# haiciyang/LaDiffCodec

Measured on AMD Instinct MI355X. Metric: audio-sec decoded / wall-sec, 16kHz 3kbps 50-step DDPM, higher is better.
Workload: dtype bf16; 1 GPU; LaDiffCodec 3 kbps, diff_dims=256, enc_ratios 8 4, 50-step DDPM, batch=32x2.4 s utterances per GPU; global_batch=32, latent_len=1200, denoise_steps=50, rccl_ranks=1, batches_in_flight=1, parallelism=dp1 (utterance-sharded, no data-path collective)

## Files before the change

### include/ladiffcodec.h

```cpp
#ifndef LADIFFCODEC_H_
#define LADIFFCODEC_H_

#include <stdint.h>

#ifdef __cplusplus
extern "C" {
#endif

#define LDC_OK 0
#define LDC_E_INVALID -1
#define LDC_E_STATE -2
#define LDC_E_MISSING -3
#define LDC_E_HIP -4
#define LDC_E_NOMEM -5

#define LDC_F32 0
#define LDC_BF16 1
#define LDC_BF16_W8 2

#define LDC_MODEL_MAIN 0
#define LDC_MODEL_COND 1

#define LDC_MAX_RATIOS 8

// ... 120 lines not shown
                             float* eps_out, void* stream);
int ldc_denoise_windows(ldc_ctx* ctx, float* img_inout, const float* cond, const float* noise, int n_steps, int Ltot, int Ftot, int Lw,
                        int overlap, void* stream);
int ldc_ddim_sample_windows(ldc_ctx* ctx, float* img_inout, const float* cond, const float* noise, int t_start, int n_steps, float eta,
                            int Ltot, int Ftot, int Lw, int overlap, void* stream);
int ldc_decode_windows(ldc_ctx* ctx, const float* wav, int T, int n_steps, const float* noise, int Lw, int overlap, float* wav_out,
                       float* latents_out, float* cond_out, int64_t* codes_out, void* stream);
int ldc_decode_ddim_windows(ldc_ctx* ctx, const float* wav, int T, int t_start, int n_steps, float eta, const float* noise, int Lw,
                            int overlap, float* wav_out, float* latents_out, float* cond_out, int64_t* codes_out, void* stream);
int ldc_dpm_sample_windows(ldc_ctx* ctx, float* img_inout, const float* cond, int t_start, int n_steps, int Ltot, int Ftot, int Lw,
                           int overlap, void* stream);
int ldc_decode_dpm_windows(ldc_ctx* ctx, const float* wav, int T, int t_start, int n_steps, int Lw, int overlap, float* wav_out,
                           float* latents_out, float* cond_out, int64_t* codes_out, void* stream);
int ldc_decode_codes_windows(ldc_ctx* ctx, const int64_t* codes, const uint8_t* packed, int64_t packed_stride, int bits, int n_q, int Ftot,
                             int t_start, int n_steps, float eta, const float* noise, int Lw, int overlap, float* wav_out,
                             float* latents_out, float* cond_out, void* stream);
int ldc_decode_codes_dpm_windows(ldc_ctx* ctx, const int64_t* codes, const uint8_t* packed, int64_t packed_stride, int bits, int n_q,
                                 int Ftot, int t_start, int n_steps, int Lw, int overlap, float* wav_out, float* latents_out,
                                 float* cond_out, void* stream);
int ldc_window_group_layout(int R, const int* Ltot , int Lw, int overlap, int up, int* w0_out , int* starts_out ,
                            float* weights_out );
int ldc_unet_forward_windows_group(ldc_ctx* ctx, const float* x, int t, const float* cond, int R, const int* Ltot ,
                                   const int* Ftot , int Lw, int overlap, float* eps_out, void* stream);
int ldc_sample_windows_group(ldc_ctx* ctx, float* img_inout, const float* cond, int sampler, int t_start, int n_steps, float eta,
                             const float* noise, const uint64_t* seeds , int R, const int* Ltot ,
                             const int* Ftot , int Lw, int overlap, void* stream);
int ldc_decode_windows_group(ldc_ctx* ctx, const float* wav, int R, const int* T , int sampler, int t_start, int n_steps, float eta,
                             const float* noise, const uint64_t* seeds , int Lw, int overlap, float* wav_out,
                             float* latents_out, float* cond_out, int64_t* codes_out, void* stream);

int ldc_decode_codes(ldc_ctx* ctx, const int64_t* codes, const uint8_t* packed, int64_t packed_stride, int bits,
                     int n_q, int B, int F, int n_steps, const float* noise, int per_item,
                     float* wav_out, float* latents_out, float* cond_out, void* stream);
int ldc_decode_codes_ddim(ldc_ctx* ctx, const int64_t* codes, const uint8_t* packed, int64_t packed_stride, int bits,
                          int n_q, int B, int F, int t_start, int n_steps, float eta, const float* noise, int per_item,
                          float* wav_out, float* latents_out, float* cond_out, void* stream);
int ldc_decode_codes_ragged(ldc_ctx* ctx, const int64_t* codes, const uint8_t* packed, int64_t packed_stride, int bits, int n_q,
                            int B, int Fmax, const int32_t* frames_host, int t_start, int n_steps, float eta, const float* noise,
                            float* wav_out, float* latents_out, float* cond_out, void* stream);

int ldc_dpm_schedule(const float* sqrt_recip, const float* sqrt_recipm1, int timesteps, int t_start, int n_steps, int* t_out,
                     float* coef_out);
int ldc_dpm_sample(ldc_ctx* ctx, float* img_inout, const float* cond, int t_start, int n_steps, int B, int L, int F, void* stream);
int ldc_decode_dpm(ldc_ctx* ctx, const float* wav, int B, int T, int t_start, int n_steps, int per_item, float* wav_out,
                   float* latents_out, float* cond_out, int64_t* codes_out, void* stream);
int ldc_decode_codes_dpm(ldc_ctx* ctx, const int64_t* codes, const uint8_t* packed, int64_t packed_stride, int bits, int n_q, int B,
                         int F, int t_start, int n_steps, int per_item, float* wav_out, float* latents_out, float* cond_out,
                         void* stream);
int ldc_decode_ragged_dpm(ldc_ctx* ctx, const float* wav, const int32_t* lengths_host, int B, int Tmax, int t_start, int n_steps,
                          float* wav_out, float* latents_out, float* cond_out, int64_t* codes_out, void* stream);

int64_t ldc_packed_bytes(int n_q, int F, int bits);
int ldc_pack_codes(ldc_ctx* ctx, const int64_t* codes, int n_q, int B, int F, int bits, uint8_t* out, int64_t out_stride, void* stream);
int ldc_unpack_codes(ldc_ctx* ctx, const uint8_t* in, int64_t in_stride, int n_q, int B, int F, int bits, int64_t* codes_out,
                     void* stream);
int ldc_ac_build_cdf(ldc_ctx* ctx, const float* pdf, int rows, int card, int total_range_bits, float roundoff, int min_range,
                     int32_t* cdf_out, void* stream);
int ldc_ac_encode(ldc_ctx* ctx, const int32_t* symbols, const int32_t* cdf, int B, int S, int card, int n_static, int total_range_bits,
                  uint8_t* out, int64_t out_stride, int64_t* nbytes_out, void* stream);
int ldc_ac_decode(ldc_ctx* ctx, const uint8_t* in, int64_t in_stride, const int64_t* nbytes, const int32_t* cdf, int B, int S, int card,
                  int n_static, int total_range_bits, int32_t* symbols_out, int32_t* status_out, void* stream);
int ldc_ac_encode_ragged(ldc_ctx* ctx, const int32_t* symbols, const int32_t* n_sym, const int32_t* cdf, int B, int S, int card,
                         int n_static, int total_range_bits, uint8_t* out, int64_t out_stride, int64_t* nbytes_out, void* stream);
int ldc_ac_decode_ragged(ldc_ctx* ctx, const uint8_t* in, int64_t in_stride, const int64_t* nbytes, const int32_t* n_sym,
                         const int32_t* cdf, int B, int S, int card, int n_static, int total_range_bits, int32_t* symbols_out,
                         int32_t* status_out, void* stream);

int64_t ldc_resample_out_len(int64_t T, int orig_freq, int new_freq);
int ldc_resample(ldc_ctx* ctx, const float* wav, int C, int64_t T, int orig_freq, int new_freq, float* out, void* stream);

int ldc_train_q_sample(ldc_ctx* ctx, const float* x_start, const int64_t* t, const float* noise, int B, int C, int L, float* x_t,
                       void* stream);
int ldc_train_num_timesteps(ldc_ctx* ctx);
int ldc_train_predict_x_start(ldc_ctx* ctx, const float* x_t, const float* eps, const int64_t* t, int B, int C, int L, float* x0_out,
                              void* stream);
int ldc_train_neg_sdsdr(ldc_ctx* ctx, const float* est, const float* tgt, int B, int64_t n_per_item, float clip_min, float* per_item_out,
                        void* stream);

int ldc_train_l1_loss(ldc_ctx* ctx, const float* model_out, const float* target, const int64_t* t, int B, int C, int L, float* loss_out,
                      float* grad_out, void* stream);
int64_t ldc_train_block_ws_floats(int B, int Cin, int Cout, int L, int groups);
int ldc_train_block_forward(ldc_ctx* ctx, const float* x, const float* w, const float* bias, const float* gamma, const float* beta,
                            const float* scale_shift, int B, int Cin, int Cout, int L, int groups, float* y, float* ws, void* stream);
int ldc_train_block_backward(ldc_ctx* ctx, const float* dy, const float* x, const float* gamma, const float* beta,
                             const float* scale_shift, int B, int Cin, int Cout, int L, int groups, float* ws, float* dx, float* dw,
                             float* db, float* dgamma, float* dbeta, float* dscale_shift, void* stream);

int ldc_train_layernorm_forward(ldc_ctx* ctx, const float* x, const float* g, int B, int C, int L, float* y, float* stats, void* stream);
int ldc_train_layernorm_backward(ldc_ctx* ctx, const float* dy, const float* x, const float* g, const float* stats, int B, int C, int L,
                                 float* dx, float* dg, void* stream);

int ldc_train_pointwise_forward(ldc_ctx* ctx, const float* x, const float* w, const float* bias, int B, int Cin, int Cout, int L, int pre_silu,
                                float* y, void* stream);
int ldc_train_pointwise_backward(ldc_ctx* ctx, const float* dy, const float* x, const float* w, int B, int Cin, int Cout, int L, int pre_silu,
                                 float* dx, float* dw, float* db, void* stream);

int64_t ldc_train_linattn_ws_floats(int B, int heads, int dim_head, int N);
int ldc_train_linattn_forward(ldc_ctx* ctx, const float* qkv, int B, int heads, int dim_head, int N, float* out, float* ws, void* stream);
int ldc_train_linattn_backward(ldc_ctx* ctx, const float* dout, const float* qkv, int B, int heads, int dim_head, int N, float* ws, float* dqkv,
                               void* stream);

int ldc_train_conv_forward(ldc_ctx* ctx, const float* x, const float* w, const float* bias, int B, int Cin, int Cout, int Lin, int K, int stride,
                           int pad, float* y, void* stream);
int ldc_train_conv_backward(ldc_ctx* ctx, const float* dy, const float* x, const float* w, int B, int Cin, int Cout, int Lin, int K, int stride,
                            int pad, float* dx, float* dw, float* db, void* stream);
int ldc_train_join(ldc_ctx* ctx, void* stream);
int ldc_train_side_stream(ldc_ctx* ctx, void** stream_out);
int ldc_train_upsample2(ldc_ctx* ctx, const float* in, int64_t rows, int L, int backward, float* out, void* stream);
int ldc_train_activation(ldc_ctx* ctx, const float* x, const float* dy, int64_t n, int kind, float* out, void* stream);
int64_t ldc_train_attn_ws_floats(int B, int heads, int N);
int ldc_train_attn_forward(ldc_ctx* ctx, const float* qkv, int B, int heads, int dim_head, int N, float* out, float* ws, void* stream);
int ldc_train_attn_backward(ldc_ctx* ctx, const float* dout, const float* qkv, int B, int heads, int dim_head, int N, float* ws, float* dqkv,
                            void* stream);

int ldc_train_convtr_forward(ldc_ctx* ctx, const float* x, const float* w, const float* bias, int B, int Cin, int Cout, int L, int ratio, float* y,
                             void* stream);
int ldc_train_convtr_backward(ldc_ctx* ctx, const float* dy, const float* x, const float* w, int B, int Cin, int Cout, int L, int ratio, float* dx,
                              float* dw, float* db, void* stream);
int ldc_train_maxscale(ldc_ctx* ctx, const float* x, const float* dy, int B, int64_t n_per_item, float* out, void* stream);

int ldc_train_adam_step(ldc_ctx* ctx, float* param, const float* grad, float* exp_avg, float* exp_avg_sq, int64_t n, int step, float lr,
                        float beta1, float beta2, float eps, void* stream);
int ldc_train_adam_step_dev(ldc_ctx* ctx, float* param, const float* grad, float* exp_avg, float* exp_avg_sq, int64_t n, int32_t* step_dev,
                            float lr, float beta1, float beta2, float eps, void* stream);

int ldc_sconv1d(ldc_ctx* ctx, const float* x, int B, int Cin, int L, const float* w_host, const float* b_host,
                int Cout, int k, int stride, int dilation, int causal, int pre_elu, float* y, void* stream);
int ldc_sconvtr1d(ldc_ctx* ctx, const float* x, int B, int Cin, int L, const float* w_host, const float* b_host,
                  int Cout, int k, int stride, int causal, float* y, void* stream);
int ldc_slstm(ldc_ctx* ctx, const float* x, int B, int H, int T, const float* const* weights_host, int layers,
              float* y, void* stream);

int ldc_unet_debug_tap(ldc_ctx* ctx, const char* name, float* out, int64_t capacity_elems, void* stream);
int ldc_unet_step_cost(ldc_ctx* ctx, int B, int L, double* flops, double* bytes);
int ldc_profile_enable(ldc_ctx* ctx, int on);
int ldc_xcc_census(ldc_ctx* ctx, const uint32_t* mask, int n_words, int wgs, int* hist16);

int ldc_debug_attn_core(ldc_ctx* ctx, int kind, const float* qkv, int B, int L, const float* w_out, const float* b_out,
                        const float* gain, const float* resid, int C, float* out, void* stream);
int ldc_debug_attention_block(ldc_ctx* ctx, const char* name, const float* x, int B, int L, float* out, void* stream);
int ldc_debug_resnet_block(ldc_ctx* ctx, const char* name, const float* x1, const float* x2, int B, int L, int t, const int32_t* lens,
                           int shift, const int32_t* t_items, int with_attention, float* out, float* mid, float* stats, float* attn_out,
                           float* pre, int* info, void* stream);

int ldc_debug_sea_conv(ldc_ctx* ctx, const float* x, int B, int Cin, int L, const float* w_host, const float* b_host, int Cout, int k,
                       int stride, int dilation, int causal, int transposed, int pre_elu, const float* residual, float* y, int* route,
                       void* stream);
int ldc_debug_sea_op(ldc_ctx* ctx, int which, int decoder, int index, const float* x, int B, int L, float* out, int64_t capacity_elems,
                     int* info, void* stream);

int ldc_debug_raise_failure(ldc_ctx* ctx, int code);
long long ldc_debug_sync_count(void);
long long ldc_debug_lean_launches(int kind);

int ldc_host_stats(ldc_ctx* ctx, int reset, double* graph_launch_ms, double* lookahead_wait_ms, int64_t* graph_launches);
int ldc_graph_schedule(int n_steps, int parts, int strided, int graph_steps_option, int* K_out, int* n_big_out, int* n_single_out);
int ldc_stream_info(ldc_ctx* ctx, int* good, int* candidates, double* one_spin_ms, double* all_spin_ms, int* parts);
int ldc_clock_sample(ldc_ctx* ctx, uint64_t* out2, void* stream);

int ldc_timeline_enable(ldc_ctx* ctx, int on);
int ldc_timeline_read(ldc_ctx* ctx, int part, int n, uint64_t* ticks);
int ldc_kstamps_enable(ldc_ctx* ctx, int on);
int ldc_kstamps_reset(ldc_ctx* ctx);
int ldc_kstamps_read(ldc_ctx* ctx, int idx, int n_steps, int* n_ops, uint64_t* ticks, char* infos, int info_cap, int* classes);
int ldc_gn_microbench(ldc_ctx* ctx, int dtype, int B, int L, int C, int with_residual, int iters, double* ms_per_launch);
int ldc_conv_microbench(ldc_ctx* ctx, int dtype, int B, int L, int cin1, int cin2, int cout, int k, int stride, int ups,
                        int iters, double* ms_per_launch);
int ldc_conv_compare(ldc_ctx* ctx, int dtype, int B, int L, int cin1, int cin2, int cout, int k, int stride, int ups, int tile_cfg,
                     int with_gn, int with_colmax, int with_residual, double* max_abs_diff, double* max_abs_ref, double* max_rel_stat);
int ldc_ln_fold_compare(ldc_ctx* ctx, int dtype, int rows, int C, int n_out, double dc, double* max_abs_diff2, double* max_abs_ref);
int ldc_conv_compare_fp8(ldc_ctx* ctx, int B, int L, int cin1, int cin2, int cout, int k, int stride, int ups, int with_gn, int with_colmax,
                         double* max_abs_diff, double* max_abs_ref, double* max_rel_stat);
int ldc_profile_read(ldc_ctx* ctx, double* conv_ms_total, int64_t* conv_launches, double* conv_flops_total);
enum {
  LDC_CLASS_OTHER = 0,
  LDC_CLASS_CONV = 1,
  LDC_CLASS_GN_APPLY = 2,
  LDC_CLASS_LAYERNORM = 3,
  LDC_CLASS_LINATTN = 4,
  LDC_CLASS_ATTN_FULL = 5,
  LDC_CLASS_ELEMENTWISE = 6,
  LDC_N_CLASSES = 7
};
int ldc_profile_read_classes(ldc_ctx* ctx, int n, double* ms, int64_t* launches, double* flops, double* bytes);

#ifdef __cplusplus
}
#endif
#endif
```

### ladiffcodec_amd/csrc/ldc_api.cpp

```cpp
#include "ldc_internal.h"

long long g_device_syncs = 0;

static thread_local char g_err[1024] = "";
int fail(int code, const char* fmt, ...) {
  va_list ap;
  va_start(ap, fmt);
  vsnprintf(g_err, sizeof(g_err), fmt, ap);
  va_end(ap);
  return code;
}

extern "C" const char* ldc_last_error(void) { return g_err; }
extern "C" const char* ldc_version(void) { return "ladiffcodec-amd 0.1 (gfx950)"; }



static std::vector<float> fold_weight_norm(const HostTensor& g, const HostTensor& v) {
  const size_t n0 = (size_t)v.shape[0], inner = v.numel() / n0;
  std::vector<float> w(v.numel());
  for (size_t i = 0; i < n0; ++i) {
    double s = 0;
    for (size_t j = 0; j < inner; ++j) s += (double)v.data[i * inner + j] * v.data[i * inner + j];
    const float nrm = (float)sqrt(s);
// ... 499 lines not shown
    const int r = c->cfg.upsampling_ratios[i];
    const std::string p = P + ".upsampling_layers." + std::to_string(i) + ".convtr.convtr";
    HostTensor* w = wr.get(p + ".weight", {u.cond_channels, u.cond_channels, 2 * r});
    HostTensor* b = wr.get(p + ".bias", {u.cond_channels});
    u.up_ratios.push_back(r);
    if (!w || !b) continue;
    ConvLayer ly;
    const int padding_total = r, right = padding_total / 2, left = padding_total - right;
    LDCCHK(make_convtr(c, DT_F32, u.cond_channels, u.cond_channels, r, left, ACT_NONE, w->data.data(), b->data.data(), &ly));
    u.upsamplers.push_back(ly);
  }
  static const char* names[13] = {"betas", "alphas_cumprod", "alphas_cumprod_prev", "sqrt_alphas_cumprod",
                                  "sqrt_one_minus_alphas_cumprod", "log_one_minus_alphas_cumprod",
                                  "sqrt_recip_alphas_cumprod", "sqrt_recipm1_alphas_cumprod", "posterior_variance",
                                  "posterior_log_variance_clipped", "posterior_mean_coef1", "posterior_mean_coef2",
                                  "p2_loss_weight"};
  std::map<std::string, float*> dev;
  for (const char* n : names) {
    HostTensor* t = wr.get(std::string("diffusion.") + n, {u.timesteps});
    if (!t) continue;
    float* d = nullptr;
    LDCCHK(c->wmem.upload(&d, t->data));
    dev[n] = d;
    if (std::string(n) == "alphas_cumprod") c->alphas_cumprod = t->data;
    if (std::string(n) == "sqrt_recip_alphas_cumprod") c->sqrt_recip_ac = t->data;
    if (std::string(n) == "sqrt_recipm1_alphas_cumprod") c->sqrt_recipm1_ac = t->data;
  }
  c->sched.sqrt_recip_alphas_cumprod = dev["sqrt_recip_alphas_cumprod"];
  c->sched.sqrt_recipm1_alphas_cumprod = dev["sqrt_recipm1_alphas_cumprod"];
  c->sched.posterior_mean_coef1 = dev["posterior_mean_coef1"];
  c->sched.posterior_mean_coef2 = dev["posterior_mean_coef2"];
  c->sched.posterior_log_variance_clipped = dev["posterior_log_variance_clipped"];
  c->sqrt_alphas_cumprod = dev["sqrt_alphas_cumprod"];
  c->sqrt_one_minus_alphas_cumprod = dev["sqrt_one_minus_alphas_cumprod"];
  c->p2_loss_weight = dev["p2_loss_weight"];
  if (wr.missing.empty()) LDCCHK(build_time_table(c, wr));
  *missing += wr.missing;
  return LDC_OK;
}

static int build_time_table(ldc_ctx* c, WeightReader& wr) {
  UnetW& u = c->unet;
  const int T = u.timesteps, dim = u.dim, td = u.time_dim;
  const std::string P = "diff_model";
  HostTensor* w1 = wr.get(P + ".time_mlp.1.weight", {td, dim});
  HostTensor* b1 = wr.get(P + ".time_mlp.1.bias", {td});
  HostTensor* w2 = wr.get(P + ".time_mlp.3.weight", {td, td});
  HostTensor* b2 = wr.get(P + ".time_mlp.3.bias", {td});
  if (!w1 || !b1 || !w2 || !b2) return LDC_OK;
  const int half = dim / 2;
  std::vector<float> emb((size_t)T * dim);
  const float lg = logf(10000.0f) / (float)(half - 1);
  for (int t = 0; t < T; ++t)
    for (int k = 0; k < half; ++k) {
      const float f = expf((float)k * -lg);
      const float a = (float)t * f;
      emb[(size_t)t * dim + k] = sinf(a);
      emb[(size_t)t * dim + half + k] = cosf(a);
    }
  DevMem tmp;
  float *d_emb = nullptr, *d_h1 = nullptr, *d_h2 = nullptr;
  LDCCHK(tmp.upload(&d_emb, emb));
  void* p = nullptr;
  LDCCHK(tmp.alloc(&p, (size_t)T * td * 4)); d_h1 = (float*)p;
  LDCCHK(tmp.alloc(&p, (size_t)T * td * 4)); d_h2 = (float*)p;
  LDCCHK(c->wmem.alloc(&p, (size_t)T * u.ss_stride * 4));
  u.ss_table = (float*)p;
  LDCCHK(c->wmem.alloc(&p, (size_t)u.ss_stride * 4));
  u.cur_ss = (float*)p;
  hipStream_t s = c->own_stream;
  ConvLayer l1, l2;
  ConvSpec sp;
  sp.dt = DT_F32; sp.cin1 = dim; sp.cout = td; sp.k = 1; sp.post_act = ACT_GELU;
  LDCCHK(make_conv(c, sp, w1->data.data(), b1->data.data(), &l1));
  sp.cin1 = td; sp.post_act = ACT_SILU;
  LDCCHK(make_conv(c, sp, w2->data.data(), b2->data.data(), &l2));
  ConvCall cc;
  cc.B = 1; cc.L_in = T; cc.L_rows = T;
  cc.x1 = d_emb; cc.y = d_h1; cc.y_ld = td;
  HIPCHK(launch_conv(l1, cc, s));
  cc.x1 = d_h1; cc.y = d_h2;
  HIPCHK(launch_conv(l2, cc, s));
  std::vector<ResnetW*> blocks;
  for (auto& lv : u.downs) { blocks.push_back(&lv.b1); blocks.push_back(&lv.b2); }
  blocks.push_back(&u.mid1); blocks.push_back(&u.mid2);
  for (auto& lv : u.ups) { blocks.push_back(&lv.b1); blocks.push_back(&lv.b2); }
  blocks.push_back(&u.fin);
  std::vector<std::string> prefixes;
  for (size_t i = 0; i < u.downs.size(); ++i) { prefixes.push_back(P + ".downs." + std::to_string(i) + ".0"); prefixes.push_back(P + ".downs." + std::to_string(i) + ".1"); }
  prefixes.push_back(P + ".mid_block1"); prefixes.push_back(P + ".mid_block2");
  for (size_t i = 0; i < u.ups.size(); ++i) { prefixes.push_back(P + ".ups." + std::to_string(i) + ".0"); prefixes.push_back(P + ".ups." + std::to_string(i) + ".1"); }
  prefixes.push_back(P + ".final_res_block");
  for (size_t i = 0; i < blocks.size(); ++i) {
    ResnetW* r = blocks[i];
    HostTensor* wm = wr.get(prefixes[i] + ".mlp.1.weight", {2 * r->cout, td});
    HostTensor* bm = wr.get(prefixes[i] + ".mlp.1.bias", {2 * r->cout});
    if (!wm || !bm) continue;
    ConvLayer lm;
    ConvSpec sm;
    sm.dt = DT_F32; sm.cin1 = td; sm.cout = 2 * r->cout; sm.k = 1;
    LDCCHK(make_conv(c, sm, wm->data.data(), bm->data.data(), &lm));
    ConvCall cm;
    cm.B = 1; cm.L_in = T; cm.L_rows = T; cm.x1 = d_h2; cm.y = u.ss_table + r->ss_off; cm.y_ld = u.ss_stride;
    HIPCHK(launch_conv(lm, cm, s));
    u.weight_elems += (double)wm->numel();
  }
  HIPCHK(hipStreamSynchronize(s));
  return LDC_OK;
}

extern "C" int ldc_create(const ldc_config* cfg, int device, ldc_ctx** out) {
  if (!cfg || !out) return fail(LDC_E_INVALID, "null argument");
  if (cfg->compute_dtype != LDC_F32 && cfg->compute_dtype != LDC_BF16 && cfg->compute_dtype != LDC_BF16_W8)
    return fail(LDC_E_INVALID, "compute_dtype must be LDC_F32, LDC_BF16 or LDC_BF16_W8");
  if (cfg->n_enc_ratios < 1 || cfg->n_enc_ratios > LDC_MAX_RATIOS || cfg->n_upsampling_ratios < 0 ||
      cfg->n_upsampling_ratios > LDC_MAX_RATIOS)
    return fail(LDC_E_INVALID, "bad ratio counts");
  if (cfg->rep_dims != 128) return fail(LDC_E_INVALID, "rep_dims must be 128 (RVQ / UNet channel width of the reference checkpoints)");
  if (cfg->diff_dims % 32 || cfg->diff_dims <= 0) return fail(LDC_E_INVALID, "diff_dims must be a positive multiple of 32");
  if (cfg->n_filters % 32) return fail(LDC_E_INVALID, "n_filters must be a multiple of 32");
  int ndev = 0;
  HIPCHK(hipGetDeviceCount(&ndev));
  if (device < 0 || device >= ndev) return fail(LDC_E_INVALID, "device %d out of range (%d visible)", device, ndev);
  HIPCHK(hipSetDevice(device));
  hipDeviceProp_t prop;
  HIPCHK(hipGetDeviceProperties(&prop, device));
  if (strncmp(prop.gcnArchName, "gfx950", 6) != 0)
    return fail(LDC_E_INVALID, "this library is built for gfx950 (MI355X) only; device %d is %s", device, prop.gcnArchName);
  std::unique_ptr<ldc_ctx> c(new ldc_ctx());
  c->cfg = *cfg;
  c->device = device;
  c->num_cus = prop.multiProcessorCount;
  c->dt = cfg->compute_dtype == LDC_F32 ? DT_F32 : DT_BF16;
  c->w8 = cfg->compute_dtype == LDC_BF16_W8;
  HIPCHK(hipStreamCreateWithFlags(&c->own_stream, hipStreamNonBlocking));
  for (int k = 0; k < kMaxParts; ++k)
    for (int e = 0; e <= ldc_ctx::kLstmChunks; ++e) HIPCHK(hipEventCreateWithFlags(&c->lstm_ev[k][e], hipEventDisableTiming));
  if (const char* ex = getenv("LDC_TEST_EXTRA_STREAMS")) {
    for (int i = 0; i < atoi(ex); ++i) { hipStream_t dummy = nullptr; HIPCHK(hipStreamCreateWithFlags(&dummy, hipStreamNonBlocking)); }
  }
  HIPCHK(hipEventCreateWithFlags(&c->ev_fork, hipEventDisableTiming));
  for (auto& e : c->flow_ev) HIPCHK(hipEventCreateWithFlags(&e, hipEventDisableTiming));
  for (int k = 1; k < kMaxParts; ++k) {
    HIPCHK(hipStreamCreateWithFlags(&c->aux_stream[k], hipStreamNonBlocking));
    HIPCHK(hipEventCreateWithFlags(&c->ev_join[k], hipEventDisableTiming));
  }
  for (int k = 0; k < kMaxParts; ++k) {
    HIPCHK(hipStreamCreateWithFlags(&c->side_stream[k], hipStreamNonBlocking));
    HIPCHK(hipEventCreateWithFlags(&c->ev_side_fork[k], hipEventDisableTiming));
    HIPCHK(hipEventCreateWithFlags(&c->ev_side_join[k], hipEventDisableTiming));
  }
  c->xcd_resident[0] = lstm_xcd_resident(256);
  c->xcd_resident[1] = lstm_xcd_resident(512);
  c->coop_resident[0] = lstm_coop_resident(256) ? 1 : 0;
  c->coop_resident[1] = lstm_coop_resident(512) ? 1 : 0;
  c->plan_bytes_cap = (size_t)48 << 30;
  c->plan_count_cap = 24;
  if (const char* mp = getenv("LDC_AUX_FROM_SIDE")) {
    c->calib = 0;
    for (int k = 1; k < kMaxParts && mp[k - 1]; ++k)
      if (mp[k - 1] >= '0' && mp[k - 1] < '0' + kMaxParts) std::swap(c->aux_stream[k], c->side_stream[mp[k - 1] - '0']);
  }
  if (const char* ov = getenv("LDC_OPTIONS")) {
    std::string all(ov);
    size_t pos = 0;
    while (pos < all.size()) {
      size_t end = all.find_first_of(",; ", pos);
      if (end == std::string::npos) end = all.size();
      const std::string kv = all.substr(pos, end - pos);
      pos = end + 1;
      if (kv.empty()) continue;
      const size_t eq = kv.find('=');
      const std::string name = kv.substr(0, eq);
      const int value = eq == std::string::npos ? 1 : atoi(kv.c_str() + eq + 1);
      std::unique_ptr<ldc_ctx>& cc = c;
      const int rc = ldc_set_option(cc.get(), name.c_str(), value);
      if (rc != LDC_OK) return fail(LDC_E_INVALID, "LDC_OPTIONS: %s", ldc_last_error());
    }
  }
  switch (cfg->final_activation) {
    case LDC_ACT_NONE: c->enc_final_act = ACT_NONE; break;
    case LDC_ACT_TANH: c->enc_final_act = ACT_TANH; break;
    case LDC_ACT_SIGMOID: c->enc_final_act = ACT_SIGMOID; break;
    case LDC_ACT_ELU: c->enc_final_act = ACT_ELU; break;
    case LDC_ACT_SILU: c->enc_final_act = ACT_SILU; break;
    case LDC_ACT_GELU: c->enc_final_act = ACT_GELU; break;
    case LDC_ACT_RELU: c->enc_final_act = ACT_RELU; break;
    default: return fail(LDC_E_INVALID, "final_activation code %d is not one of LDC_ACT_*", cfg->final_activation);
  }
  {
    void* hp = nullptr;
    HIPCHK(hipHostMalloc(&hp, 64, hipHostMallocMapped));
    memset(hp, 0, 64);
    c->dev_flag_host = (unsigned*)hp;
    void* dp = nullptr;
    HIPCHK(hipHostGetDevicePointer(&dp, hp, 0));
    c->dev_flag_dev = (unsigned*)dp;
  }
  void* p = nullptr;
  HIPCHK(hipMalloc(&p, 4 * sizeof(int)));
  c->step_state = (int*)p;
  *out = c.release();
  return LDC_OK;
}

void free_plan_resources(Plan* pl) {
  for (hipEvent_t e : pl->marker_events) (void)hipEventDestroy(e);
  if (pl->arena_base) (void)hipFree(pl->arena_base);
  if (pl->x0_prev) (void)hipFree(pl->x0_prev);
  if (pl->item_keys) (void)hipFree(pl->item_keys);
  if (pl->win_base) (void)hipFree(pl->win_base);
}

void release_plan(ldc_ctx* c, size_t idx) {
  Plan* pl = c->plans[idx].get();
  for (int k = 0; k < c->last_halves.n; ++k)
    if (c->last_halves.p[k] == pl) c->last_halves = Halves();
  free_plan_resources(pl);
  c->plan_bytes -= pl->arena_bytes;
  c->plans.erase(c->plans.begin() + idx);
}

void drop_plans(ldc_ctx* c) {
  (void)counted_device_sync();
  drop_step_graphs(c, [](const StepGraph&) { return true; });
  for (auto& pl : c->plans) free_plan_resources(pl.get());
  c->plans.clear();
  c->plan_bytes = 0;
  c->last_halves = Halves();
}

extern "C" int ldc_destroy(ldc_ctx* c) {
  if (!c) return LDC_OK;
  (void)hipSetDevice(c->device);
  (void)counted_device_sync();
  drop_plans(c);
  if (c->scratch) (void)hipFree(c->scratch);
  if (c->outnorm_ws) (void)hipFree(c->outnorm_ws);
  if (c->state_buf) (void)hipFree(c->state_buf);
  if (c->ddim_table) (void)hipFree(c->ddim_table);
  if (c->dpm_table) (void)hipFree(c->dpm_table);
  if (c->step_state) (void)hipFree(c->step_state);
  if (c->dev_flag_host) (void)hipHostFree(c->dev_flag_host);
  if (c->tl_buf) (void)hipFree(c->tl_buf);
  for (auto& e : c->prof_events) { (void)hipEventDestroy(e.first); (void)hipEventDestroy(e.second); }
  if (c->ev_fork) (void)hipEventDestroy(c->ev_fork);
  for (int k = 0; k < kMaxParts; ++k) {
    for (int e = 0; e <= ldc_ctx::kLstmChunks; ++e)
      if (c->lstm_ev[k][e]) (void)hipEventDestroy(c->lstm_ev[k][e]);
  }
  for (auto& e : c->flow_ev) if (e) (void)hipEventDestroy(e);
  for (int k = 1; k < kMaxParts; ++k) {
    if (c->ev_join[k]) (void)hipEventDestroy(c->ev_join[k]);
    if (c->aux_stream[k]) (void)hipStreamDestroy(c->aux_stream[k]);
  }
  for (int k = 0; k < kMaxParts; ++k) {
    if (c->ev_side_fork[k]) (void)hipEventDestroy(c->ev_side_fork[k]);
    if (c->ev_side_join[k]) (void)hipEventDestroy(c->ev_side_join[k]);
    if (c->side_stream[k]) (void)hipStreamDestroy(c->side_stream[k]);
  }
  if (c->own_stream) (void)hipStreamDestroy(c->own_stream);
  delete c;
  return LDC_OK;
}

extern "C" void ldc_quantize_e4m3(const float* in, int64_t n, uint8_t* out_codes, float* out_values) {
  for (int64_t i = 0; i < n; ++i) {
    const uint8_t q = host_f32_to_e4m3(in[i]);
    if (out_codes) out_codes[i] = q;
    if (out_values) out_values[i] = host_e4m3_to_f32(q);
  }
}

struct OptRef { int* p; bool replan; int lo, hi; };
static bool find_option(ldc_ctx* c, const std::string& n, OptRef* r) {
#define LDC_OPT(NAME, FIELD, REPLAN, LO, HI) if (n == NAME) { r->p = &(FIELD); r->replan = REPLAN; r->lo = LO; r->hi = HI; return true; }
  LDC_OPT("split", c->split_batch, true, 1, kMaxParts)
  LDC_OPT("part_graphs", c->part_graphs, false, 0, 2)
  LDC_OPT("graph_steps", c->graph_steps, false, 0, 1000)
  LDC_OPT("flow_depth", c->flow_depth, false, 0, (int)ldc_ctx::kFlowRing - 1)
  LDC_OPT("split_ends", c->split_ends, false, 0, 1)
  LDC_OPT("ends_join", c->ends_join, false, 0, 1)
  LDC_OPT("split_init", c->split_init, true, 0, 1)
  LDC_OPT("side_streams", c->side_streams, true, 0, 1)
  LDC_OPT("serial_parts", c->serial_parts, false, 0, 1)
  LDC_OPT("stream_calib", c->calib, false, 0, 1)
  LDC_OPT("merge_advance", c->merge_advance, true, 0, 1)
  LDC_OPT("fuse_gn_stats", c->fuse_gn_stats, true, 0, 1)
  LDC_OPT("fuse_gn_epi", c->fuse_gn_epi, true, 0, 1)
  LDC_OPT("gn_epi_min_l", c->gn_epi_min_l, true, 0, 1 << 30)
  LDC_OPT("gn_epi_max_tiles", c->gn_epi_max_tiles, true, 0, 1 << 30)
  LDC_OPT("fold_res", c->fold_res, true, 0, 1)
  LDC_OPT("fold_ln", c->fold_ln, true, 0, 1)
  LDC_OPT("fuse_kmax", c->fuse_kmax, true, 0, 1)
  LDC_OPT("fuse_ln", c->fuse_ln, true, 0, 1)
  LDC_OPT("fuse_attn_tail", c->fuse_attn_tail, true, 0, 1)
  LDC_OPT("fold_ctx", c->fold_ctx, true, 0, 1)
  LDC_OPT("conv_lean", c->tune.lean, true, 0, 1)
  LDC_OPT("lean_all", c->tune.lean_all, true, 0, 1)
  LDC_OPT("ring3_tiles", c->tune.ring3_tiles, true, 0, 1 << 30)
  LDC_OPT("ring3_wgs", c->tune.ring3_wgs, true, 1, 3)
  LDC_OPT("ring3_window", c->tune.ring3_window, true, 0, 1)
  LDC_OPT("ring3_window_tiles", c->tune.ring3_window_tiles, true, 0, 1 << 30)
  LDC_OPT("conv_generic", c->tune.force_generic, true, 0, 1)
  LDC_OPT("conv_small_tiles", c->tune.small_max, true, 0, 1 << 30)
  LDC_OPT("conv_splitk", c->tune.splitk, true, 0, 4)
  LDC_OPT("sk_tiles", c->tune.sk_tiles, true, 0, 1 << 30)
  LDC_OPT("sk_u2", c->tune.sk_u2, true, 0, 1 << 30)
  LDC_OPT("sk_u3", c->tune.sk_u3, true, 0, 1 << 30)
  LDC_OPT("conv_mfast", c->tune.m_fastest, true, 0, 2)
  LDC_OPT("conv_debug", c->tune.debug, true, 0, 255)
  LDC_OPT("conv_tile", c->tune.force_tile, true, -1, 1)
  LDC_OPT("conv_xcd_order", c->tune.xcd_order, true, 0, 8)
  LDC_OPT("gn_nap", c->tune.gn_nap, true, 0, 4096)
  LDC_OPT("gn_nap0", c->tune.gn_nap0, true, 0, 4096)
  LDC_OPT("lstm_stream", c->lstm_stream_only, false, 0, 1)
  LDC_OPT("lstm_xcd", c->lstm_xcd, false, 0, 1)
  LDC_OPT("lstm_pipe", c->lstm_pipe, false, 0, 1)
  LDC_OPT("coop_launch", c->coop_launch, false, 0, 1)
  LDC_OPT("sea_splitk", c->sea_splitk, false, 0, 1)
  LDC_OPT("rvq_tiled", c->rvq_tiled, false, 0, 1)
  LDC_OPT("train_bf16", g_train_bf16, false, 0, 1)
  LDC_OPT("train_fp32_mfma", g_train_fp32_mfma, false, 0, 1)
  LDC_OPT("train_valu", g_train_valu, false, 0, 1)
  LDC_OPT("train_dw_side", g_train_dw_side, false, 0, 1)
#undef LDC_OPT
  return false;
}

extern "C" int ldc_set_option(ldc_ctx* c, const char* name, int value) {
  if (!c || !name) return fail(LDC_E_INVALID, "null context or option name");
  const std::string n(name);
  if (n == "fp8_act") {
    if (c->finalized) return fail(LDC_E_STATE, "fp8_act must be set before ldc_finalize_weights");
    c->fp8_act = value ? 1 : 0;
    return LDC_OK;
  }
  if (n == "plan_cache_gb") { c->plan_bytes_cap = (size_t)std::max(1, value) << 30; return LDC_OK; }
  if (n == "plan_cache_n") { c->plan_count_cap = std::max(2 * kMaxParts, value); return LDC_OK; }
  OptRef r;
  if (!find_option(c, n, &r)) return fail(LDC_E_INVALID, "unknown option '%s' (tools/README.md lists the options)", name);
  if (value < r.lo || value > r.hi) return fail(LDC_E_INVALID, "option %s must be in %d..%d", name, r.lo, r.hi);
  if (n == "side_streams" && value && c->split_batch != 1) return fail(LDC_E_INVALID, "side streams need a single chain (split 1)");
  if (value == *r.p) return LDC_OK;
  if (r.replan && c->live_pools > 0)
    return fail(LDC_E_STATE, "option %s rebuilds every plan, and %d decode pool(s) keep their items' state in theirs: destroy the pools first", name, c->live_pools);
  if (r.replan && !c->plans.empty()) { HIPCHK(hipSetDevice(c->device)); drop_plans(c); }
  *r.p = value;
  if (n == "split" && value != 1) c->side_streams = 0;
  return LDC_OK;
}

extern "C" long long ldc_debug_sync_count(void) { return g_device_syncs; }

extern "C" int ldc_debug_raise_failure(ldc_ctx* c, int code) {
  if (!c || !c->dev_flag_host || (code != 1 && code != 2 && code != (int)kDevFailCtxRange)) return fail(LDC_E_INVALID, "bad arguments");
  *reinterpret_cast<volatile unsigned*>(c->dev_flag_host) = (unsigned)code;
  return LDC_OK;
}

extern "C" int ldc_reseed(ldc_ctx* c, uint64_t seed) {
  if (!c) return fail(LDC_E_INVALID, "null ctx");
  c->cfg.noise_seed = seed;
  c->noise_epoch = 0;
  return LDC_OK;
}

extern "C" int ldc_set_weight(ldc_ctx* c, int which, const char* key, const float* data, const int64_t* shape, int ndim) {
  if (!c || !key || !data || (ndim > 0 && !shape)) return fail(LDC_E_INVALID, "null argument");
  if (which != LDC_MODEL_MAIN && which != LDC_MODEL_COND) return fail(LDC_E_INVALID, "which must be LDC_MODEL_MAIN or LDC_MODEL_COND");
  if (c->finalized) return fail(LDC_E_STATE, "weights already finalized");
  HostTensor t;
  t.shape.assign(shape, shape + ndim);
  t.data.assign(data, data + t.numel());
  c->raw[which][key] = std::move(t);
  return LDC_OK;
}

extern "C" int ldc_finalize_weights(ldc_ctx* c, int strict) {
  if (!c) return fail(LDC_E_INVALID, "null ctx");
  if (c->finalized) return fail(LDC_E_STATE, "already finalized");
  HIPCHK(hipSetDevice(c->device));
  std::string missing;
  std::vector<int> main_ratios(c->cfg.enc_ratios, c->cfg.enc_ratios + c->cfg.n_enc_ratios);
  LDCCHK(build_codec(c, LDC_MODEL_MAIN, main_ratios, 0, &missing));
  LDCCHK(build_unet(c, &missing));
  if (c->cfg.has_cond_model) {
    const int frame_rate_ceil = 50;
    const int n_q = (int)floor(1000.0 * c->cfg.cond_bandwidth / (frame_rate_ceil * 10));
    LDCCHK(build_codec(c, LDC_MODEL_COND, {8, 5, 4, 2}, n_q, &missing));
  }
  if (!missing.empty()) return fail(LDC_E_MISSING, "missing or mis-shaped keys in state_dict: %s", missing.c_str());
  if (strict) {
    std::string unexpected;
    for (int w = 0; w < 2; ++w)
      for (auto& kv : c->raw[w])
        if (!kv.second.used) {
          const std::string& k = kv.first;
          std::string alias;
          if (k.rfind("diffusion.model.", 0) == 0) alias = "diff_model." + k.substr(16);
          else if (k.rfind("diff_model.", 0) == 0) alias = "diffusion.model." + k.substr(11);
          auto it = alias.empty() ? c->raw[w].end() : c->raw[w].find(alias);
          if (it != c->raw[w].end() && it->second.used && it->second.shape == kv.second.shape) continue;
          if (unexpected.size() < 600) unexpected += k + " ";
        }
    if (!unexpected.empty()) return fail(LDC_E_MISSING, "unexpected keys in state_dict: %s", unexpected.c_str());
  }
  c->raw[0].clear();
  c->raw[1].clear();
  c->finalized = true;
  return LDC_OK;
}

int ensure_scratch(ldc_ctx* c, size_t bytes, hipStream_t s) {
  if (bytes <= c->scratch_cap) return LDC_OK;
  HIPCHK(hipStreamSynchronize(s));
  HIPCHK(counted_device_sync());
  if (c->scratch) HIPCHK(hipFree(c->scratch));
  c->scratch = nullptr;
  c->scratch_cap = 0;
  void* p = nullptr;
  const size_t want = bytes + bytes / 4;
  hipError_t e = hipMalloc(&p, want);
  if (e != hipSuccess) return fail(LDC_E_NOMEM, "hipMalloc(%zu) for scratch failed: %s", want, hipGetErrorString(e));
  c->scratch = (char*)p;
  c->scratch_cap = want;
  return LDC_OK;
}

int conv_out_len(const ConvLayer& ly, int L) {
  const int eff_k = (ly.taps - 1) * ly.dil + 1;
  const int padding_total = eff_k - ly.stride;
  const double n_frames = (double)(L - eff_k + padding_total) / ly.stride + 1.0;
  return (int)ceil(n_frames);
}


static int stream_conv_state(SeaRun& R, int rows, int ch, StreamConvState** out) {
  *out = nullptr;
  if (!R.st || rows <= 0) return LDC_OK;
  if (R.st->conv_at >= R.st->convs.size() || R.st->convs[R.st->conv_at].rows != rows || R.st->convs[R.st->conv_at].ch != ch)
    return fail(LDC_E_STATE, "stream state does not match the layer table (conv %zu: %d rows x %d channels)", R.st->conv_at, rows, ch);
  *out = &R.st->convs[R.st->conv_at++];
  return LDC_OK;
}

static int sea_conv_stream(SeaRun& R, const ConvLayer& ly, StreamConvState& cs, const void* x, const void* residual, int L_in, void** y, int* L_out, int cout) {
  if (!ly.tr_stride && L_in % ly.stride) return fail(LDC_E_INVALID, "stream chunk of %d rows is not a multiple of the layer's stride %d", L_in, ly.stride);
  ConvLayer lv = ly;
  lv.pad_left = 0;
  ConvCall cc;
  cc.B = R.B; cc.L_in = L_in + cs.rows; cc.x1 = x; cc.residual = residual; cc.tune = &R.c->tune; cc.route_out = R.route;
  cc.ctx = cs.buf[R.st->parity]; cc.ctx_fresh = R.st->fresh_dev; cc.ctx_rows = cs.rows; cc.ctx_zero = ly.tr_stride ? 1 : 0;
  if (ly.tr_stride) {
    cc.L_rows = L_in;
    cc.L_final = L_in * ly.tr_stride;
    *L_out = cc.L_final;
    cc.y_ld = ly.tr_cout;
  } else {
    cc.L_rows = L_in / ly.stride;
    *L_out = cc.L_rows;
    cc.y_ld = cout;
  }
  *y = R.ar->alloc((size_t)R.B * (*L_out) * cc.y_ld * 4);
  cc.y = *y;
  if (R.c->sea_splitk) {
    const long long fl = conv_generic_splitk_floats(lv, cc);
    if (fl > 0) {
      cc.sk_part = (float*)R.ar->alloc((size_t)fl * 4);
      cc.sk_part_cap = fl;
      cc.generic_split = 1;
    }
  }
  if (R.dry) {
    ConvCall chk = cc;
    chk.check_only = 1; chk.route_out = nullptr;
    if (launch_conv(lv, chk, R.s) != hipSuccess)
      return fail(LDC_E_INVALID, "stream chunk of %d rows x B = %d items: the LDS window of a layer (%d context rows per item, stride %d) does not fit; "
                                 "use longer chunks or fewer items per session", L_in, R.B, cs.rows, ly.stride);
  } else {
    HIPCHK(launch_conv(lv, cc, R.s));
    HIPCHK(launch_stream_ctx_update((const float*)x, cs.buf[R.st->parity], cs.buf[R.st->parity ^ 1], R.st->fresh_dev, R.B, L_in, cs.rows, cs.ch, cc.ctx_zero, R.s));
  }
  return LDC_OK;
}

int sea_conv(SeaRun& R, const ConvLayer& ly, const void* x, const void* residual, int L_in, void** y, int* L_out, int cout) {
  StreamConvState* cs = nullptr;
  LDCCHK(stream_conv_state(R, ly.tr_stride ? 1 : ly.pad_left, ly.cin1, &cs));
  if (cs) return sea_conv_stream(R, ly, *cs, x, residual, L_in, y, L_out, cout);
  ConvCall cc;
  cc.B = R.B; cc.L_in = L_in; cc.x1 = x; cc.residual = residual; cc.tune = &R.c->tune; cc.route_out = R.route;
  if (ly.tr_stride) {
    cc.L_rows = L_in + 1;
    cc.L_final = L_in * ly.tr_stride;
    *L_out = cc.L_final;
    cc.y_ld = ly.tr_cout;
  } else {
    cc.L_rows = conv_out_len(ly, L_in);
    *L_out = cc.L_rows;
    cc.y_ld = cout;
  }
  *y = R.ar->alloc((size_t)R.B * (*L_out) * cc.y_ld * 4);
  cc.y = *y;
  if (R.c->sea_splitk) {
    const long long fl = conv_generic_splitk_floats(ly, cc);
    if (fl > 0) {
      cc.sk_part = (float*)R.ar->alloc((size_t)fl * 4);
      cc.sk_part_cap = fl;
      cc.generic_split = 1;
    }
  }
  if (!R.dry) HIPCHK(launch_conv(ly, cc, R.s));
  return LDC_OK;
}

int run_seanet(SeaRun& R, const std::vector<SeaOp>& ops, const void* x_in, int L, void** out, int* L_out, int* C_out) {
  const void* x = x_in;
  int C = 0;
  for (const SeaOp& op : ops) {
    void* y = nullptr;
    int Ln = L;
    switch (op.kind) {
      case SeaOp::CONV_CIN1: {
        if (L <= op.k - 1) return fail(LDC_E_INVALID, "input no longer than the first conv's reflect padding is not supported (L=%d pad=%d)", L, op.k - 1);
        y = R.ar->alloc((size_t)R.B * L * op.cout * 4);
        StreamConvState* cs = nullptr;
        LDCCHK(stream_conv_state(R, op.k - 1, 1, &cs));
        if (!R.dry && cs) {
          HIPCHK(launch_conv_cin1(DT_F32, (const float*)x, y, op.w1, op.b1, R.B, L, op.cout, op.k, R.s, nullptr, cs->buf[R.st->parity], R.st->fresh_dev));
          HIPCHK(launch_stream_ctx_update((const float*)x, cs->buf[R.st->parity], cs->buf[R.st->parity ^ 1], R.st->fresh_dev, R.B, L, cs->rows, 1, 0, R.s));
        } else if (!R.dry) HIPCHK(launch_conv_cin1(DT_F32, (const float*)x, y, op.w1, op.b1, R.B, L, op.cout, op.k, R.s));
        C = op.cout;
        break;
      }
      case SeaOp::CONV:
      case SeaOp::CONVTR:
        LDCCHK(sea_conv(R, op.conv, x, nullptr, L, &y, &Ln, op.cout));
        C = op.cout;
        break;
      case SeaOp::RES: {
        void *sc = nullptr, *h = nullptr;
        int l1 = L, l2 = L, l3 = L;
        LDCCHK(sea_conv(R, op.shortcut, x, nullptr, L, &sc, &l1, op.cout));
        LDCCHK(sea_conv(R, op.conv, x, nullptr, L, &h, &l2, op.hidden));
        LDCCHK(sea_conv(R, op.conv2, h, sc, l2, &y, &l3, op.cout));
        Ln = l3;
        C = op.cout;
        break;
      }
      case SeaOp::LSTM: {
        const int H = op.cout;
        const void* in = x;
        const bool pipe = !R.st && R.c->lstm_pipe && R.side >= 0 && R.side < 2 && R.c->aux_stream[2 + R.side] && op.lstm.size() == 2 && lstm_seq_supported(H) && !op.lstm[0].w_rm && !op.lstm[1].w_rm &&
                          L >= 64 * ldc_ctx::kLstmChunks;
        if (pipe) {
          constexpr int NCH = ldc_ctx::kLstmChunks;
          void* pre0 = R.ar->alloc((size_t)R.B * L * 4 * H * 4);
          void* o0 = R.ar->alloc((size_t)R.B * L * H * 4);
          void* pre1 = R.ar->alloc((size_t)R.B * L * 4 * H * 4);
          void* o1 = R.ar->alloc((size_t)R.B * L * H * 4);
          float* st0 = (float*)R.ar->alloc((size_t)R.B * 2 * H * 4);
          float* st1 = (float*)R.ar->alloc((size_t)R.B * 2 * H * 4);
          if (!R.dry) {
            hipStream_t s2 = R.c->aux_stream[2 + R.side];
            hipEvent_t* ev = R.c->lstm_ev[R.side];
            ConvCall cc;
            cc.B = R.B; cc.L_in = L; cc.L_rows = L; cc.x1 = in; cc.y = pre0; cc.y_ld = 4 * H; cc.tune = &R.c->tune;
            HIPCHK(launch_conv(op.lstm[0].in_proj, cc, R.s));
            for (int k = 0; k < NCH; ++k) {
              const int t0 = (int)((long long)L * k / NCH), t1 = (int)((long long)L * (k + 1) / NCH);
              LstmSeq q0;
              q0.t0 = t0; q0.t1 = t1; q0.pre_bs = L; q0.pre_ts = 1; q0.out_bs = 1; q0.out_ts = R.B; q0.state = st0;
              HIPCHK(launch_lstm_seq(DT_F32, pre0, op.lstm[0].w_hh, o0, nullptr, R.B, H, q0, R.s));
              HIPCHK(hipEventRecord(ev[k], R.s));
              HIPCHK(hipStreamWaitEvent(s2, ev[k], 0));
              ConvCall c1;
              c1.B = 1; c1.L_in = (t1 - t0) * R.B; c1.L_rows = c1.L_in; c1.tune = &R.c->tune; c1.y_ld = 4 * H;
              c1.x1 = (const char*)o0 + (size_t)t0 * R.B * H * 4;
              c1.y = (char*)pre1 + (size_t)t0 * R.B * 4 * H * 4;
              HIPCHK(launch_conv(op.lstm[1].in_proj, c1, s2));
              LstmSeq q1;
              q1.t0 = t0; q1.t1 = t1; q1.pre_bs = 1; q1.pre_ts = R.B; q1.out_bs = L; q1.out_ts = 1; q1.skip_bs = L; q1.skip_ts = 1; q1.state = st1;
              HIPCHK(launch_lstm_seq(DT_F32, pre1, op.lstm[1].w_hh, o1, x, R.B, H, q1, s2));
            }
            HIPCHK(hipEventRecord(ev[NCH], s2));
            HIPCHK(hipStreamWaitEvent(R.s, ev[NCH], 0));
          }
          y = o1;
          C = H;
          break;
        }
        for (size_t n = 0; n < op.lstm.size(); ++n) {
          void* pre = R.ar->alloc((size_t)R.B * L * 4 * H * 4);
          void* o = R.ar->alloc((size_t)R.B * L * H * 4);
          const bool coop = op.lstm[n].w_rm && !R.c->lstm_stream_only && R.c->coop_resident[H == 512 ? 1 : 0];
          void* lws = coop ? R.ar->alloc(lstm_coop_ws_bytes(H)) : nullptr;
          LstmCarry carry;
          if (R.st) {
            if (R.st->lstm_at >= R.st->lstm.size()) return fail(LDC_E_STATE, "stream state does not match the layer table (LSTM layer %zu)", R.st->lstm_at);
            carry.state = R.st->lstm[R.st->lstm_at++];
            carry.fresh = R.st->fresh_dev;
          }
          if (!R.dry) {
            ConvCall cc;
            cc.B = R.B; cc.L_in = L; cc.L_rows = L; cc.x1 = in; cc.y = pre; cc.y_ld = 4 * H; cc.tune = &R.c->tune;
            HIPCHK(launch_conv(op.lstm[n].in_proj, cc, R.s));
            const bool lastl = n + 1 == op.lstm.size();
            hipError_t le = hipErrorCooperativeLaunchTooLarge;
            if (coop) le = launch_lstm_coop(DT_F32, pre, op.lstm[n].w_rm, o, lastl ? x : nullptr, R.B, L, H, lws, R.c->dev_flag_dev, (R.c->lstm_xcd && R.c->xcd_resident[H == 512 ? 1 : 0] >= 2 * R.teams) ? 2 : R.c->coop_launch, R.s, carry);
            if (le == hipErrorCooperativeLaunchTooLarge) {
              (void)hipGetLastError();
              le = launch_lstm_layer(DT_F32, pre, op.lstm[n].w_hh, o, lastl ? x : nullptr, R.B, L, H, R.s, carry);
            }
            HIPCHK(le);
          }
          in = o;
          y = o;
        }
        C = H;
        break;
      }
    }
    x = y;
    L = Ln;
  }
  *out = const_cast<void*>(x);
  *L_out = L;
  *C_out = C;
  return LDC_OK;
}


int check_ready(ldc_ctx* c, int which, bool need_cond_codec) {
  if (!c) return fail(LDC_E_INVALID, "null ctx");
  if (!c->finalized) return fail(LDC_E_STATE, "ldc_finalize_weights has not been called");
  if (which != LDC_MODEL_MAIN && which != LDC_MODEL_COND) return fail(LDC_E_INVALID, "bad model selector");
  if ((which == LDC_MODEL_COND || need_cond_codec) && !c->codec[LDC_MODEL_COND].present)
    return fail(LDC_E_STATE, "no cond model configured (has_cond_model = 0)");
  hipError_t e = hipSetDevice(c->device);
  if (e != hipSuccess) return fail(LDC_E_HIP, "hipSetDevice failed: %s", hipGetErrorString(e));
  return check_dev_flag(c);
}

extern "C" int ldc_seanet_encode(ldc_ctx* c, int which, const float* wav, int B, int T, float* z_out, void* stream) {
  LDCCHK(check_ready(c, which));
  if (!wav || !z_out || B <= 0 || T <= 0) return fail(LDC_E_INVALID, "bad arguments");
  hipStream_t s = pick_stream(c, stream);
  const Codec& cd = c->codec[which];
  LDCCHK(with_scratch(c, s, [&](Arena& ar, bool dry) -> int {
    SeaRun R{c, &ar, s, dry, B};
    void* z = nullptr;
    int L = 0, C = 0;
    LDCCHK(run_seanet(R, cd.enc, wav, T, &z, &L, &C));
    if (!dry) HIPCHK(launch_from_cl(DT_F32, z, z_out, B, C, L, nullptr, 0, 0.f, s));
    return LDC_OK;
  }));
  return finish_stream(c, stream);
}

extern "C" int ldc_seanet_decode(ldc_ctx* c, int which, const float* z, int B, int L, float* wav_out, void* stream) {
  LDCCHK(check_ready(c, which));
  if (!z || !wav_out || B <= 0 || L <= 0) return fail(LDC_E_INVALID, "bad arguments");
  hipStream_t s = pick_stream(c, stream);
  const Codec& cd = c->codec[which];
  const int D = c->cfg.rep_dims;
  LDCCHK(with_scratch(c, s, [&](Arena& ar, bool dry) -> int {
    SeaRun R{c, &ar, s, dry, B};
    R.side = 0;
    void* zc = ar.alloc((size_t)B * L * D * 4);
    if (!dry) HIPCHK(launch_to_cl(DT_F32, z, zc, B, D, L, nullptr, 0, 0.f, s));
    void* y = nullptr;
    int Lo = 0, C = 0;
    LDCCHK(run_seanet(R, cd.dec, zc, L, &y, &Lo, &C));
    if (!dry) HIPCHK(hipMemcpyAsync(wav_out, y, (size_t)B * Lo * 4, hipMemcpyDeviceToDevice, s));
    return LDC_OK;
  }));
  return finish_stream(c, stream);
}

int rvq_rows(ldc_ctx* c, const float* z_rows, int rows, int n_q, int64_t* codes, float* q_rows, Arena& ar, bool dry,
                    hipStream_t s) {
  const Codec& cd = c->codec[LDC_MODEL_COND];
  int64_t* cw = codes;
  if (!cw) cw = (int64_t*)ar.alloc((size_t)n_q * rows * sizeof(int64_t));
  if (!dry) HIPCHK(launch_rvq(z_rows, rows, c->cfg.rep_dims, cd.codebooks, cd.cb_sqnorm, cd.bins, n_q, cw, q_rows, s, c->rvq_tiled));
  return LDC_OK;
}

int n_q_for_bandwidth(ldc_ctx* c, float bandwidth) {
  const Codec& cd = c->codec[LDC_MODEL_COND];
  const double bw = bandwidth > 0 ? bandwidth : c->cfg.cond_bandwidth;
  const double bw_per_q = log2((double)cd.bins) * (16000.0 / cd.hop) / 1000.0;
  int n_q = cd.n_q_layers;
  if (bw > 0) n_q = (int)std::max(1.0, floor(bw / bw_per_q));
  return std::min(n_q, cd.n_q_layers);
}

extern "C" int ldc_rvq_encode(ldc_ctx* c, const float* z, int B, int F, int n_q, int64_t* codes_out, float* quantized_out,
                              void* stream) {
  LDCCHK(check_ready(c, LDC_MODEL_COND));
  const Codec& cd = c->codec[LDC_MODEL_COND];
  if (!z || !quantized_out || B <= 0 || F <= 0 || n_q < 1 || n_q > cd.n_q_layers)
    return fail(LDC_E_INVALID, "bad arguments (n_q must be in [1,%d])", cd.n_q_layers);
  hipStream_t s = pick_stream(c, stream);
  const int D = c->cfg.rep_dims;
  LDCCHK(with_scratch(c, s, [&](Arena& ar, bool dry) -> int {
    float* zr = (float*)ar.alloc((size_t)B * F * D * 4);
    float* qr = (float*)ar.alloc((size_t)B * F * D * 4);
    if (!dry) HIPCHK(launch_to_cl(DT_F32, z, zr, B, D, F, nullptr, 0, 0.f, s));
    LDCCHK(rvq_rows(c, zr, B * F, n_q, codes_out, qr, ar, dry, s));
    if (!dry) HIPCHK(launch_from_cl(DT_F32, qr, quantized_out, B, D, F, nullptr, 0, 0.f, s));
    return LDC_OK;
  }));
  return finish_stream(c, stream);
}

extern "C" int ldc_rvq_decode(ldc_ctx* c, const int64_t* codes, int B, int F, int n_q, float* quantized_out, void* stream) {
  LDCCHK(check_ready(c, LDC_MODEL_COND));
  const Codec& cd = c->codec[LDC_MODEL_COND];
  if (!codes || !quantized_out || B <= 0 || F <= 0 || n_q < 1 || n_q > cd.n_q_layers) return fail(LDC_E_INVALID, "bad arguments");
  hipStream_t s = pick_stream(c, stream);
  const int D = c->cfg.rep_dims;
  LDCCHK(with_scratch(c, s, [&](Arena& ar, bool dry) -> int {
    float* qr = (float*)ar.alloc((size_t)B * F * D * 4);
    if (!dry) {
      HIPCHK(launch_rvq_dequant(codes, nullptr, 0, 0, n_q, B, 0, B, F, cd.codebooks, cd.bins, D, qr, c->dev_flag_dev, s));
      HIPCHK(launch_from_cl(DT_F32, qr, quantized_out, B, D, F, nullptr, 0, 0.f, s));
    }
    return LDC_OK;
  }));
  return finish_stream(c, stream);
}

static int get_cond_rows(ldc_ctx* c, const float* wav, int B, int T, float bandwidth, Arena& ar, bool dry, hipStream_t s,
                         float** q_rows, int* F_out, int64_t* codes_out, int teams = 1) {
  const Codec& cd = c->codec[LDC_MODEL_COND];
  SeaRun R{c, &ar, s, dry, B};
  R.teams = teams;
  void* z = nullptr;
  int F = 0, C = 0;
  LDCCHK(run_seanet(R, cd.enc, wav, T, &z, &F, &C));
  float* qr = (float*)ar.alloc((size_t)B * F * C * 4);
  LDCCHK(rvq_rows(c, (const float*)z, B * F, n_q_for_bandwidth(c, bandwidth), codes_out, qr, ar, dry, s));
  *q_rows = qr;
  *F_out = F;
  return LDC_OK;
}

extern "C" int ldc_get_cond(ldc_ctx* c, const float* wav, int B, int T, float bandwidth, float* cond_out, int64_t* codes_out,
                            void* stream) {
  LDCCHK(check_ready(c, LDC_MODEL_COND));
  if (!wav || !cond_out || B <= 0 || T <= 0) return fail(LDC_E_INVALID, "bad arguments");
  hipStream_t s = pick_stream(c, stream);
  LDCCHK(with_scratch(c, s, [&](Arena& ar, bool dry) -> int {
    float* qr = nullptr;
    int F = 0;
    LDCCHK(get_cond_rows(c, wav, B, T, bandwidth, ar, dry, s, &qr, &F, codes_out));
    if (!dry) HIPCHK(launch_from_cl(DT_F32, qr, cond_out, B, c->cfg.rep_dims, F, nullptr, 0, 0.f, s));
    return LDC_OK;
  }));
  return finish_stream(c, stream);
}

static int upsample_rows(ldc_ctx* c, const void* rows_in, int B, int F, Arena& ar, bool dry, hipStream_t s, void** out,
                         int* L_out, const int* flens = nullptr) {
  const UnetW& u = c->unet;
  const void* x = rows_in;
  int L = F;
  for (const ConvLayer& ly : u.upsamplers) {
    ConvCall cc;
    cc.B = B; cc.L_in = L; cc.L_rows = L + 1; cc.L_final = L * ly.tr_stride; cc.y_ld = ly.tr_cout; cc.x1 = x; cc.tune = &c->tune;
    void* y = ar.alloc((size_t)B * cc.L_final * ly.tr_cout * 4);
    cc.y = y;
    if (!dry) HIPCHK(launch_conv(ly, cc, s));
    if (!dry && flens) HIPCHK(launch_mask_rows(DT_F32, y, B, F, cc.L_final / F * ly.tr_cout, flens, 0, s));
    x = y;
    L = cc.L_final;
  }
  *out = const_cast<void*>(x);
  *L_out = L;
  return LDC_OK;
}

int upsample_factor(const ldc_ctx* c) {
  int f = 1;
  for (int r : c->unet.up_ratios) f *= r;
  return f;
}

extern "C" int ldc_cond_upsample(ldc_ctx* c, const float* cond, int B, int F, int normalise, float* img_out, void* stream) {
  LDCCHK(check_ready(c, LDC_MODEL_MAIN));
  if (!cond || !img_out || B <= 0 || F <= 0 || normalise < 0 || normalise > 2) return fail(LDC_E_INVALID, "bad arguments");
  hipStream_t s = pick_stream(c, stream);
  const int C = c->unet.cond_channels;
  LDCCHK(with_scratch(c, s, [&](Arena& ar, bool dry) -> int {
    void* rows = ar.alloc((size_t)B * F * C * 4);
    float* mx = (float*)ar.alloc((size_t)B * 4);
    if (!dry) HIPCHK(launch_to_cl(DT_F32, cond, rows, B, C, F, nullptr, 0, 0.f, s));
    void* up = nullptr;
    int L = 0;
    LDCCHK(upsample_rows(c, rows, B, F, ar, dry, s, &up, &L));
    if (!dry) {
      if (normalise) {
        HIPCHK(hipMemsetAsync(mx, 0, (size_t)B * 4, s));
        HIPCHK(launch_maxabs(DT_F32, up, B, (int64_t)L * C, normalise == 2, mx, s));
        HIPCHK(launch_from_cl(DT_F32, up, img_out, B, C, L, mx, normalise == 2, 1e-8f, s));
      } else {
        HIPCHK(launch_from_cl(DT_F32, up, img_out, B, C, L, nullptr, 0, 0.f, s));
      }
    }
    return LDC_OK;
  }));
  return finish_stream(c, stream);
}

int calibrate_part_streams(ldc_ctx* c, hipStream_t s) {
  if (!c->calib || (c->calibrated && c->calib_stream == s)) return LDC_OK;
  hipStreamCaptureStatus cs = hipStreamCaptureStatusNone;
  if (hipStreamIsCapturing(s, &cs) != hipSuccess || cs != hipStreamCaptureStatusNone) { (void)hipGetLastError(); return LDC_OK; }
  std::vector<hipStream_t*> cand;
  for (int k = 1; k < kMaxParts; ++k) cand.push_back(&c->aux_stream[k]);
  for (int k = 0; k < kMaxParts; ++k) cand.push_back(&c->side_stream[k]);
  for (const auto& e : c->calib_cache)
    if (e.s == s && e.order.size() == cand.size()) {
      for (size_t i = 0; i < cand.size(); ++i) *cand[i] = e.order[i];
      c->calib_good = e.good; c->calib_cand = e.cand; c->calib_one_ms = e.one_ms; c->calib_all_ms = e.all_ms;
      c->calib_stream = s; c->calibrated = true;
      return LDC_OK;
    }
  std::vector<hipStream_t> chosen{s};
  auto timed = [&](const std::vector<hipStream_t>& set, double* ms) -> int {
    double best = 1e30;
    for (int rep = 0; rep < 4; ++rep) {
      for (hipStream_t q : set) HIPCHK(hipStreamSynchronize(q));
      const auto t0 = std::chrono::steady_clock::now();
      for (hipStream_t q : set) HIPCHK(launch_spin_us(150, q));
      for (hipStream_t q : set) HIPCHK(hipStreamSynchronize(q));
      best = std::min(best, std::chrono::duration<double, std::milli>(std::chrono::steady_clock::now() - t0).count());
    }
    *ms = best;
    return LDC_OK;
  };
  double base = 0;
  LDCCHK(timed(chosen, &base));
  LDCCHK(timed(chosen, &base));
  std::vector<hipStream_t> good, rest;
  for (hipStream_t* p : cand) {
    if ((int)good.size() >= kMaxParts - 1) { rest.push_back(*p); continue; }
    std::vector<hipStream_t> set = chosen;
    set.push_back(*p);
    double ms = 0;
    LDCCHK(timed(set, &ms));
    if (ms < base + 0.09) { good.push_back(*p); chosen.push_back(*p); }
    else rest.push_back(*p);
  }
  if (getenv("LDC_VERBOSE")) fprintf(stderr, "[ldc] part streams: %zu of %zu candidates overlap with the caller's stream and each other (one spin: %.3f ms)\n", good.size(), cand.size(), base);
  std::vector<hipStream_t> order = good;
  order.insert(order.end(), rest.begin(), rest.end());
  for (size_t i = 0; i < cand.size(); ++i) *cand[i] = order[i];
  double all_ms = base;
  if (!good.empty()) LDCCHK(timed(chosen, &all_ms));
  c->calib_good = (int)good.size(); c->calib_cand = (int)cand.size(); c->calib_one_ms = base; c->calib_all_ms = all_ms;
  if (c->calib_cache.size() >= 8) c->calib_cache.erase(c->calib_cache.begin());
  c->calib_cache.push_back({s, order, c->calib_good, c->calib_cand, base, all_ms});
  c->calib_stream = s;
  c->calibrated = true;
  return LDC_OK;
}

int get_halves(ldc_ctx* c, int B, int L, int F, hipStream_t s, Halves* h, bool ragged, bool items, int pool_id) {
  *h = Halves();
  c->call_tick = c->use_tick;
  h->n = std::max(1, std::min(c->split_batch, B));
  if (h->n >= 2) LDCCHK(calibrate_part_streams(c, s));
  for (int k = 0; k < h->n; ++k) {
    const int lo = (int)((long long)B * k / h->n), hi = (int)((long long)B * (k + 1) / h->n);
    h->b0[k] = lo;
    LDCCHK(get_plan(c, hi - lo, L, F, k, s, &h->p[k], ragged, items, pool_id));
  }
  c->last_halves = *h;
  return LDC_OK;
}

int load_cond(ldc_ctx* c, const Halves& h, const float* cond, hipStream_t s) {
  for (int k = 0; k < h.n; ++k) {
    Plan* pl = h.p[k];
    const float* src = cond + (size_t)h.b0[k] * c->unet.cond_channels * pl->F;
    HIPCHK(launch_to_cl(DT_F32, src, pl->cond_in_cl, pl->B, c->unet.cond_channels, pl->F, nullptr, 0, 0.f, s));
    LDCCHK(run_ops(c, pl, false, s));
  }
  return LDC_OK;
}

int load_x(ldc_ctx* c, const Halves& h, const float* x, hipStream_t s) {
  for (int k = 0; k < h.n; ++k) {
    Plan* pl = h.p[k];
    HIPCHK(launch_to_cl(c->dt, x + (size_t)h.b0[k] * c->unet.channels * pl->L, pl->x_cl, pl->B, c->unet.channels, pl->L, nullptr,
                        0, 0.f, s));
  }
  return LDC_OK;
}

int check_unet_args(ldc_ctx* c, int B, int L, int F) {
  if (B <= 0 || L <= 0 || F <= 0) return fail(LDC_E_INVALID, "bad sizes");
  if (F * upsample_factor(c) != L) return fail(LDC_E_INVALID, "L (%d) must equal F (%d) x prod(upsampling_ratios) (%d)", L, F, upsample_factor(c));
  return LDC_OK;
}

extern "C" int ldc_unet_forward(ldc_ctx* c, const float* x, int t, const float* cond, int B, int L, int F, float* eps_out,
                                void* stream) {
// ... 43 lines not shown
    std::vector<int> fr(pl->B);
    for (int b = 0; b < pl->B; ++b) fr[b] = lat[h.b0[k] + b] / up;
    HIPCHK(launch_lens_write(pl->lens, lat.data() + h.b0[k], pl->B, s));
    HIPCHK(launch_lens_write(pl->flens, fr.data(), pl->B, s));
  }
  return LDC_OK;
}

extern "C" int ldc_unet_forward_ragged(ldc_ctx* c, const float* x, int t, const float* cond, const int32_t* latent_lens_host, int B, int Lmax,
                                       int Fmax, float* eps_out, void* stream) {
  LDCCHK(check_ready(c, LDC_MODEL_MAIN));
  if (!x || !cond || !eps_out) return fail(LDC_E_INVALID, "null tensor");
  if (t < 0 || t >= c->unet.timesteps) return fail(LDC_E_INVALID, "t out of range");
  LDCCHK(check_unet_args(c, B, Lmax, Fmax));
  LDCCHK(check_ragged_lengths(latent_lens_host, B, Lmax, ragged_latent_quantum(c), "latent frames"));
  if (c->w8) return fail(LDC_E_INVALID, "ragged batches are not available on the fp8 engine (its fused forms have no length-aware variant): use dtype bf16 or f32");
  hipStream_t s = pick_stream(c, stream);
  Halves h;
  LDCCHK(get_halves(c, B, Lmax, Fmax, s, &h, true));
  LDCCHK(write_plan_lens(c, h, std::vector<int>(latent_lens_host, latent_lens_host + B), s));
  LDCCHK(load_cond(c, h, cond, s));
  LDCCHK(load_x(c, h, x, s));
  for (int k = 0; k < h.n; ++k) {
    Plan* pl = h.p[k];
    HIPCHK(launch_mask_rows(c->dt, pl->x_cl, pl->B, Lmax, c->unet.channels, pl->lens, 0, s));
    HIPCHK(launch_step_set(pl->step_state, t, 0, c->cur_key, s));
    HIPCHK(launch_step_begin(c->unet.ss_table, c->unet.ss_stride, pl->step_state, pl->cur_ss, nullptr, s, pl->zero_ptr, pl->zero_bytes));
    LDCCHK(run_ops(c, pl, true, s));
    HIPCHK(launch_mask_rows(c->dt, pl->eps_cl, pl->B, Lmax, c->unet.channels, pl->lens, 0, s));
    HIPCHK(launch_from_cl(c->dt, pl->eps_cl, eps_out + (size_t)h.b0[k] * c->unet.channels * Lmax, pl->B, c->unet.channels, Lmax, nullptr,
                          0, 0.f, s));
  }
  return finish_stream(c, stream);
}

static int ensure_outnorm(ldc_ctx* c, int B) {
  const size_t need = output_normalise_ws_bytes(B);
  if (need <= c->outnorm_ws_bytes) return LDC_OK;
  HIPCHK(counted_device_sync());
  if (c->outnorm_ws) HIPCHK(hipFree(c->outnorm_ws));
  c->outnorm_ws = nullptr;
  HIPCHK(hipMalloc(&c->outnorm_ws, need * 2));
  c->outnorm_ws_bytes = need * 2;
  return LDC_OK;
}

extern "C" int ldc_output_normalise(ldc_ctx* c, float* wav, int B, int T, int per_item, void* stream) {
  if (!c) return fail(LDC_E_INVALID, "null ctx");
  if (!wav || B <= 0 || T <= 0) return fail(LDC_E_INVALID, "bad arguments");
  HIPCHK(hipSetDevice(c->device));
  LDCCHK(ensure_outnorm(c, B));
  hipStream_t s = pick_stream(c, stream);
  HIPCHK(launch_output_normalise(wav, B, T, per_item ? 1 : 0, c->outnorm_ws, s));
  return finish_stream(c, stream);
}

struct FrontSrc {
  const float* wav = nullptr;
  const int64_t* codes = nullptr;
  const uint8_t* packed = nullptr;
  int64_t packed_stride = 0;
  int bits = 0, n_q = 0;
};

static int ragged_cond_rows(ldc_ctx* c, const float* wav, int B, int b0, int Bk, int T, const int32_t* lens, const int* flens_dev,
                            float bandwidth, Arena& ar, bool dry, hipStream_t sk, float** q_rows, int* F_out, int64_t* codes_out,
                            int teams) {
  const Codec& cc = c->codec[LDC_MODEL_COND];
  const int F = T / cc.hop, D = c->cfg.rep_dims, n_q = n_q_for_bandwidth(c, bandwidth);
  if (codes_out && (b0 != 0 || Bk != B)) return fail(LDC_E_INVALID, "internal: the codes of a ragged batch are written for the whole batch");
  float* qr = nullptr;
  int Fq = 0;
  LDCCHK(get_cond_rows(c, wav + (size_t)b0 * T, Bk, T, bandwidth, ar, dry, sk, &qr, &Fq, codes_out, teams));
  if (!dry && Fq != F) return fail(LDC_E_INVALID, "internal: encoder produced %d frames, expected %d", Fq, F);
  const int short_max = cc.enc.empty() ? 0 : cc.enc.back().k - 1;
  for (int b = b0; b < b0 + Bk; ++b) {
    const int Fb = lens[b] / cc.hop;
    if (Fb > short_max) continue;
    float* q1 = nullptr;
    int F1 = 0;
    int64_t* codes1 = codes_out ? (int64_t*)ar.alloc((size_t)n_q * Fb * 8) : nullptr;
    LDCCHK(get_cond_rows(c, wav + (size_t)b * T, 1, lens[b], bandwidth, ar, dry, sk, &q1, &F1, codes1, teams));
    if (dry) continue;
    HIPCHK(hipMemcpyAsync(qr + (size_t)(b - b0) * F * D, q1, (size_t)F1 * D * 4, hipMemcpyDeviceToDevice, sk));
    if (codes_out)
      HIPCHK(hipMemcpy2DAsync(codes_out + (size_t)b * F, (size_t)B * F * 8, codes1, (size_t)F1 * 8, (size_t)F1 * 8, n_q, hipMemcpyDeviceToDevice, sk));
  }
  if (!dry) {
    if (codes_out) HIPCHK(launch_mask_codes(codes_out, n_q, Bk, F, flens_dev + b0, sk));
    HIPCHK(launch_mask_rows(DT_F32, qr, Bk, F, D, flens_dev + b0, 0, sk));
  }
  *q_rows = qr;
  *F_out = F;
  return LDC_OK;
}

static int decode_body(ldc_ctx* c, const FrontSrc& src, int B, int T, int n_steps, int sampler, bool draws, const float* noise, int per_item,
                       float* wav_out, float* latents_out, float* cond_out, int64_t* codes_out, void* stream, const int32_t* rag = nullptr,
                       const uint64_t* seeds = nullptr) {
  const Codec& cc = c->codec[LDC_MODEL_COND];
  const Codec& mc = c->codec[LDC_MODEL_MAIN];
  if (T % cc.hop || T % mc.hop) return fail(LDC_E_INVALID, "T must be a multiple of %d and %d (sample.py:87 trims to 640)", cc.hop, mc.hop);
  const int F = T / cc.hop, L = T / mc.hop, D = c->cfg.rep_dims;
  LDCCHK(check_unet_args(c, B, L, F));
  LDCCHK(ensure_outnorm(c, B));
  hipStream_t s = pick_stream(c, stream);
  if (sampler == SAMPLER_DDIM) LDCCHK(ddim_upload(c, s));
  if (sampler == SAMPLER_DPM) LDCCHK(dpm_upload(c, s));
  Halves h;
  LDCCHK(get_halves(c, B, L, F, s, &h, rag != nullptr));
  if (sampler == SAMPLER_DPM) LDCCHK(ensure_history(c, h));
  std::vector<int> rag_lat, rag_fr;
  if (rag) {
    for (int b = 0; b < B; ++b) { rag_lat.push_back(rag[b] / mc.hop); rag_fr.push_back(rag[b] / cc.hop); }
    LDCCHK(write_plan_lens(c, h, rag_lat, s));
  }
  if (seeds) LDCCHK(write_item_keys(c, h, seeds, s));
  const bool split_ends = c->split_ends && per_item && !codes_out && h.n >= 2 && parts_parallel(c, h);
  LDCCHK(with_scratch(c, s, [&](Arena& ar, bool dry) -> int {
    float* x = latents_out ? latents_out : (float*)ar.alloc((size_t)B * D * L * 4);
    float* mx = (float*)ar.alloc((size_t)B * 4);
    int *lens_all = nullptr, *flens_all = nullptr;
    const float* wav_in = src.wav;
    if (rag) {
      lens_all = (int*)ar.alloc((size_t)B * 4);
      flens_all = (int*)ar.alloc((size_t)B * 4);
      float* wm = src.wav ? (float*)ar.alloc((size_t)B * T * 4) : nullptr;
      if (!dry) {
        HIPCHK(launch_lens_write(lens_all, rag_lat.data(), B, s));
        HIPCHK(launch_lens_write(flens_all, rag_fr.data(), B, s));
        if (wm) {
          HIPCHK(hipMemcpyAsync(wm, src.wav, (size_t)B * T * 4, hipMemcpyDeviceToDevice, s));
          HIPCHK(launch_mask_rows(DT_F32, wm, B, L, mc.hop, lens_all, 0, s));
        }
      }
      wav_in = wm;
    }
    if (!dry && split_ends) LDCCHK(fork_parts(c, h, s));
    const int n_front = split_ends ? h.n : 1;
    bool parts_open = !dry && split_ends;
    auto bail = [&](int rc) -> int {
      if (parts_open) (void)join_parts(c, h, s);
      parts_open = false;
      return rc;
    };
    auto front_end = [&]() -> int {
    for (int k = 0; k < n_front; ++k) {
      hipStream_t sk = (split_ends && k > 0) ? c->aux_stream[k] : s;
      const int b0 = split_ends ? h.b0[k] : 0, Bk = split_ends ? h.p[k]->B : B;
      float* qr = nullptr;
      int Fq = 0;
      if (src.wav) {
        if (rag) LDCCHK(ragged_cond_rows(c, wav_in, B, b0, Bk, T, rag, flens_all, 0.f, ar, dry, sk, &qr, &Fq, codes_out, n_front));
        else LDCCHK(get_cond_rows(c, wav_in + (size_t)b0 * T, Bk, T, 0.f, ar, dry, sk, &qr, &Fq, codes_out, n_front));
      } else {
        qr = (float*)ar.alloc((size_t)Bk * F * D * 4);
        Fq = F;
        if (!dry)
          HIPCHK(launch_rvq_dequant(src.codes, src.packed, src.packed_stride, src.bits, src.n_q, B, b0, Bk, F, cc.codebooks, cc.bins, D, qr,
                                    c->dev_flag_dev, sk, rag ? flens_all + b0 : nullptr));
      }
      if (!dry && Fq != F) return fail(LDC_E_INVALID, "internal: encoder produced %d frames, expected %d", Fq, F);
      void* up = nullptr;
      int Lu = 0;
      LDCCHK(upsample_rows(c, qr, Bk, F, ar, dry, sk, &up, &Lu, rag ? flens_all + b0 : nullptr));
      if (dry) continue;
      if (cond_out) HIPCHK(launch_from_cl(DT_F32, qr, cond_out + (size_t)b0 * D * F, Bk, D, F, nullptr, 0, 0.f, sk));
      HIPCHK(hipMemsetAsync(mx + b0, 0, (size_t)Bk * 4, sk));
      HIPCHK(launch_maxabs(DT_F32, up, Bk, (int64_t)L * D, per_item ? 1 : 0, mx + b0, sk));
      HIPCHK(launch_from_cl(DT_F32, up, x + (size_t)b0 * D * L, Bk, D, L, mx + b0, per_item ? 1 : 0, 1e-8f, sk));
      for (int kk = 0; kk < h.n; ++kk) {
        if (split_ends && kk != k) continue;
        Plan* pl = h.p[kk];
        HIPCHK(hipMemcpyAsync(pl->cond_in_cl, qr + (size_t)(h.b0[kk] - b0) * F * D, (size_t)pl->B * F * D * 4, hipMemcpyDeviceToDevice, sk));
        LDCCHK(run_ops(c, pl, false, sk));
        HIPCHK(launch_to_cl(c->dt, x + (size_t)h.b0[kk] * c->unet.channels * pl->L, pl->x_cl, pl->B, c->unet.channels, pl->L, nullptr, 0, 0.f, sk));
      }
    }
    return LDC_OK;
    };
    { const int fr = front_end(); if (fr != LDC_OK) return bail(fr); }
    if (!dry) {
      if (split_ends && c->ends_join) { parts_open = false; LDCCHK(join_parts(c, h, s)); }
      if (!seeds) next_noise_key(c, noise == nullptr && draws);
      bool forked = false;
      StepSampler sm;
      sm.kind = sampler;
      sm.item_seeds = seeds != nullptr;
      sm.ddim = sampler == SAMPLER_DDIM ? c->ddim_table : nullptr;
      sm.dpm = sampler == SAMPLER_DPM ? c->dpm_table : nullptr;
      const int dr = denoise_loop(c, h, B, x, noise, n_steps, s, (split_ends && !c->ends_join) ? &forked : nullptr, sm);
      if (dr != LDC_OK) return bail(dr);
      if (split_ends && !forked) { parts_open = false; LDCCHK(fork_parts(c, h, s)); }
      parts_open = split_ends;
    }
    int Lo_all = T;
    auto back_end = [&]() -> int {
    for (int k = 0; k < n_front; ++k) {
      hipStream_t sk = (split_ends && k > 0) ? c->aux_stream[k] : s;
      const int b0 = split_ends ? h.b0[k] : 0, Bk = split_ends ? h.p[k]->B : B;
      SeaRun R{c, &ar, sk, dry, Bk};
      R.side = h.n <= 2 ? k : -1;
      R.teams = h.n;
      void* zc = ar.alloc((size_t)Bk * L * D * 4);
      if (!dry) HIPCHK(launch_to_cl(DT_F32, x + (size_t)b0 * D * L, zc, Bk, D, L, nullptr, 0, 0.f, sk));
      void* y = nullptr;
      int Lo = 0, Cd = 0;
      LDCCHK(run_seanet(R, mc.dec, zc, L, &y, &Lo, &Cd));
      if (!dry) HIPCHK(hipMemcpyAsync(wav_out + (size_t)b0 * Lo, y, (size_t)Bk * Lo * 4, hipMemcpyDeviceToDevice, sk));
      Lo_all = Lo;
    }
    return LDC_OK;
    };
    { const int br = back_end(); if (br != LDC_OK) return bail(br); }
    if (!dry) {
      if (split_ends) { parts_open = false; LDCCHK(join_parts(c, h, s)); }
      if (rag && Lo_all != T) return fail(LDC_E_INVALID, "internal: decoder produced %d samples, expected %d", Lo_all, T);
      HIPCHK(launch_output_normalise(wav_out, B, Lo_all, per_item ? 1 : 0, c->outnorm_ws, s, lens_all, mc.hop));
    }
    return LDC_OK;
  }));
  return finish_stream(c, stream);
}

extern "C" int ldc_decode(ldc_ctx* c, const float* wav, int B, int T, int n_steps, const float* noise, int per_item,
                          float* wav_out, float* latents_out, float* cond_out, int64_t* codes_out, void* stream) {
  LDCCHK(check_ready(c, LDC_MODEL_MAIN, true));
  if (!wav || !wav_out || B <= 0 || T <= 0) return fail(LDC_E_INVALID, "bad arguments");
  if (n_steps < 1 || n_steps > c->unet.timesteps) return fail(LDC_E_INVALID, "n_steps must be in [1,%d]", c->unet.timesteps);
  FrontSrc src;
  src.wav = wav;
  return decode_body(c, src, B, T, n_steps, SAMPLER_DDPM, true, noise, per_item, wav_out, latents_out, cond_out, codes_out, stream);
}

extern "C" int ldc_decode_ddim(ldc_ctx* c, const float* wav, int B, int T, int t_start, int n_steps, float eta, const float* noise,
                               int per_item, float* wav_out, float* latents_out, float* cond_out, int64_t* codes_out, void* stream) {
  LDCCHK(check_ready(c, LDC_MODEL_MAIN, true));
  if (!wav || !wav_out || B <= 0 || T <= 0) return fail(LDC_E_INVALID, "bad arguments");
  bool draws = false;
  LDCCHK(ddim_schedule(c, t_start, n_steps, eta, &draws));
  FrontSrc src;
  src.wav = wav;
  return decode_body(c, src, B, T, n_steps, SAMPLER_DDIM, draws, noise, per_item, wav_out, latents_out, cond_out, codes_out, stream);
}

static int decode_ragged_impl(ldc_ctx* c, const float* wav, const int32_t* lengths_host, int B, int Tmax, int t_start, int n_steps, float eta,
                              const float* noise, const uint64_t* seeds, float* wav_out, float* latents_out, float* cond_out, int64_t* codes_out,
                              void* stream) {
  LDCCHK(check_ready(c, LDC_MODEL_MAIN, true));
  if (!wav || !wav_out || B <= 0 || Tmax <= 0) return fail(LDC_E_INVALID, "bad arguments");
  if (t_start < 0) return fail(LDC_E_INVALID, "t_start must be >= 0 (0: DDPM halfway sampling)");
  const long long quantum = lcm_ll(c->codec[LDC_MODEL_COND].hop, (long long)c->codec[LDC_MODEL_MAIN].hop << unet_halvings(c));
  LDCCHK(check_ragged_lengths(lengths_host, B, Tmax, quantum, "samples"));
  if (c->w8) return fail(LDC_E_INVALID, "ragged batches are not available on the fp8 engine (its fused forms have no length-aware variant): use dtype bf16 or f32");
  bool draws = true;
  if (t_start > 0) LDCCHK(ddim_schedule(c, t_start, n_steps, eta, &draws));
  else if (n_steps < 1 || n_steps > c->unet.timesteps) return fail(LDC_E_INVALID, "n_steps must be in [1,%d]", c->unet.timesteps);
  FrontSrc src;
  src.wav = wav;
  return decode_body(c, src, B, Tmax, n_steps, t_start > 0 ? SAMPLER_DDIM : SAMPLER_DDPM, draws, noise, 1, wav_out, latents_out, cond_out, codes_out,
                     stream, lengths_host, seeds);
}
extern "C" int ldc_decode_ragged(ldc_ctx* c, const float* wav, const int32_t* lengths_host, int B, int Tmax, int t_start, int n_steps, float eta,
                                 const float* noise, float* wav_out, float* latents_out, float* cond_out, int64_t* codes_out, void* stream) {
  return decode_ragged_impl(c, wav, lengths_host, B, Tmax, t_start, n_steps, eta, noise, nullptr, wav_out, latents_out, cond_out, codes_out, stream);
}

extern "C" int ldc_get_cond_ragged(ldc_ctx* c, const float* wav, const int32_t* lengths_host, int B, int Tmax, float bandwidth, float* cond_out,
                                   int64_t* codes_out, void* stream) {
  LDCCHK(check_ready(c, LDC_MODEL_COND));
  if (!wav || !cond_out || B <= 0 || Tmax <= 0) return fail(LDC_E_INVALID, "bad arguments");
  const Codec& cc = c->codec[LDC_MODEL_COND];
  LDCCHK(check_ragged_lengths(lengths_host, B, Tmax, cc.hop, "samples"));
  hipStream_t s = pick_stream(c, stream);
  const int F = Tmax / cc.hop, D = c->cfg.rep_dims;
  std::vector<int> fr(B);
  for (int b = 0; b < B; ++b) fr[b] = lengths_host[b] / cc.hop;
  LDCCHK(with_scratch(c, s, [&](Arena& ar, bool dry) -> int {
    int* flens = (int*)ar.alloc((size_t)B * 4);
    float* wm = (float*)ar.alloc((size_t)B * Tmax * 4);
    if (!dry) {
      HIPCHK(launch_lens_write(flens, fr.data(), B, s));
      HIPCHK(hipMemcpyAsync(wm, wav, (size_t)B * Tmax * 4, hipMemcpyDeviceToDevice, s));
      HIPCHK(launch_mask_rows(DT_F32, wm, B, F, cc.hop, flens, 0, s));
    }
    float* qr = nullptr;
    int Fq = 0;
    LDCCHK(ragged_cond_rows(c, wm, B, 0, B, Tmax, lengths_host, flens, bandwidth, ar, dry, s, &qr, &Fq, codes_out, 1));
    if (!dry) HIPCHK(launch_from_cl(DT_F32, qr, cond_out, B, D, F, nullptr, 0, 0.f, s));
    return LDC_OK;
  }));
  return finish_stream(c, stream);
}

static int codes_args(const int64_t* codes, const uint8_t* packed, int64_t packed_stride, int bits, int n_q, int B, int F,
                      const float* wav_out) {
  if ((codes == nullptr) == (packed == nullptr)) return fail(LDC_E_INVALID, "exactly one of codes / packed must be given");
  if (!wav_out || B <= 0 || F <= 0) return fail(LDC_E_INVALID, "bad arguments");
  if (n_q < 1) return fail(LDC_E_INVALID, "n_q must be >= 1");
  if (packed && (bits < 1 || bits > 16)) return fail(LDC_E_INVALID, "bits must be in [1,16]");
  if (packed && packed_stride < ldc_packed_bytes(n_q, F, bits))
    return fail(LDC_E_INVALID, "packed_stride %lld < %lld packed bytes per item", (long long)packed_stride, (long long)ldc_packed_bytes(n_q, F, bits));
  return LDC_OK;
}

static int codes_src(ldc_ctx* c, const int64_t* codes, const uint8_t* packed, int64_t packed_stride, int bits, int n_q, int F, FrontSrc* src,
                     int* T) {
// ... 593 lines not shown
```

### ladiffcodec_amd/csrc/ldc_internal.h

```cpp
#pragma once
#include "../../include/ladiffcodec.h"

#include <hip/hip_runtime.h>
#include <math.h>
#include <stdarg.h>
#include <stdio.h>
#include <string.h>

#include <algorithm>
#include <chrono>
#include <functional>
#include <map>
#include <memory>
#include <set>
#include <string>
#include <vector>

#include "ldc_kernels.h"
#include "ldc_windows.h"
#include "plan_passes.h"
static_assert(kGnSumFloats == ldc::kGnPad, "plan_passes.h sizes the GroupNorm sums by the kernels' padding");

extern long long g_device_syncs;
inline hipError_t counted_device_sync() {
// ... 72 lines not shown
struct Codec {
  std::vector<int> ratios;
  int hop = 1;
  std::vector<SeaOp> enc, dec;
  int n_q_layers = 0, bins = 1024;
  float* codebooks = nullptr;
  float* cb_sqnorm = nullptr;
  bool present = false;
};

struct ResnetW {
  ConvLayer c1r;
  ConvLayer c1, c2, res;
  ConvLayer c2_f8;
  bool has_res = false;
  float *g1 = nullptr, *b1 = nullptr, *g2 = nullptr, *b2 = nullptr;
  int cin1 = 0, cin2 = 0, cout = 0;
  int ss_off = 0;
};
struct LinAttnW {
  float* norm_g = nullptr;
  ConvLayer qkv, out;
  ConvLayer qkv_f8;
  ConvLayer qkv_ln;
  ConvLayer qkv_ctx;
  float* out_g = nullptr;
  int dim = 0;
};
struct LevelW {
  ResnetW b1, b2;
  LinAttnW attn;
  ConvLayer resample;
  int kind = 0;
  int cin = 0, cout = 0;
};
struct UnetW {
  int dim = 0, time_dim = 0, groups = 8, heads = 4, dim_head = 32, channels = 128, cond_channels = 128;
  std::vector<int> dims;
  ConvLayer init, final_conv;
  ConvLayer init_c, init_x;
  ConvLayer final_conv_f8;
  std::vector<LevelW> downs, ups;
  ResnetW mid1, mid2, fin;
  LinAttnW mid_attn;
  std::vector<ConvLayer> upsamplers;
  std::vector<int> up_ratios;
  float* ss_table = nullptr;
  float* cur_ss = nullptr;
  int ss_stride = 0;
  int timesteps = 1000;
  double weight_elems = 0;
};

struct Plan {
  int B = 0, L = 0, F = 0, slot = 0;
  bool ragged = false;
  int* lens = nullptr;
  int* flens = nullptr;
  bool items = false;
  ItemState* item_state = nullptr;
  int pool_id = 0;
  void* init_pc = nullptr;
  uint64_t last_use = 0;
  long long sk_floats = 0;
  long long sk_need_max = 0;
  unsigned long long* kst = nullptr;
  size_t part_bytes = 0;
  size_t part_need = 0;
  void* arena_base = nullptr;
  size_t arena_bytes = 0;
  void* zero_ptr = nullptr;
  size_t zero_bytes = 0;
  void* x_cl = nullptr;
  void* cond_in_cl = nullptr;
  void* cond_cl = nullptr;
  void* eps_cl = nullptr;
  float* maxabs = nullptr;
  int* step_state = nullptr;
  float* cur_ss = nullptr;
  float* x0_prev = nullptr;
  uint64_t* item_keys = nullptr;
  int win_Ltot = 0, win_O = 0, win_id = 0;
  void* win_base = nullptr;
  float* win_x = nullptr;
  WinGroup win_group;
  WinGroupTables wg{};
  WinGroupRec* wg_rec = nullptr;
  std::vector<std::function<hipError_t(hipStream_t)>> cond_ops;
  struct StepOp {
    std::function<hipError_t(hipStream_t)> fn;
    int where;
    int cls;
    double flops, bytes;
    std::string info;
  };
  std::vector<StepOp> step;
  std::vector<hipEvent_t> marker_events;
  struct Tap { void* p; int C; int L; };
  std::map<std::string, Tap> taps;
  double flops = 0, act_bytes = 0, conv_bytes = 0;
  std::vector<std::pair<void*, size_t>> zero_once;
  void reset_build() {
    cond_ops.clear(); step.clear(); taps.clear(); zero_once.clear();
    flops = 0; act_bytes = 0; conv_bytes = 0; sk_need_max = 0; part_need = 0;
  }
};

static constexpr int kMaxParts = 4;
static_assert(kMaxParts == kWinMaxParts, "ldc_windows.h sizes the windows cap by the number of batch parts");
struct Halves {
  int n = 0;
  Plan* p[kMaxParts] = {nullptr, nullptr, nullptr, nullptr};
  int b0[kMaxParts] = {0, 0, 0, 0};
};

static constexpr int kKstOps = 256;

enum { SAMPLER_DDPM = 0, SAMPLER_DDIM = 1, SAMPLER_DPM = 2 };
struct StepSampler {
  int kind = SAMPLER_DDPM;
  const DdimStep* ddim = nullptr;
  bool item_seeds = false;
  const DpmStep* dpm = nullptr;
};

#include "step_graphs.h"

struct ldc_ctx {
  ldc_config cfg;
  int device = 0;
  int dt = DT_F32;
  bool w8 = false;
  bool finalized = false;
  std::map<std::string, HostTensor> raw[2];
  DevMem wmem;
  Codec codec[2];
  UnetW unet;
  StepTables sched{};
  const float* sqrt_alphas_cumprod = nullptr;
  const float* sqrt_one_minus_alphas_cumprod = nullptr;
  const float* p2_loss_weight = nullptr;
  std::vector<float> alphas_cumprod;
  DdimStep* ddim_table = nullptr;
  std::vector<DdimStep> ddim_host;
  std::vector<float> sqrt_recip_ac, sqrt_recipm1_ac;
  DpmStep* dpm_table = nullptr;
  std::vector<DpmStep> dpm_host;
  int* step_state = nullptr;
  std::vector<std::unique_ptr<Plan>> plans;
  std::vector<StepGraph> graphs;
  Halves last_halves;
  hipStream_t aux_stream[kMaxParts] = {nullptr, nullptr, nullptr, nullptr};
  hipEvent_t ev_fork = nullptr, ev_join[kMaxParts] = {nullptr, nullptr, nullptr, nullptr};
  static constexpr int kLstmChunks = 4;
  hipEvent_t lstm_ev[kMaxParts][kLstmChunks + 1] = {};
  hipStream_t calib_stream = nullptr; bool calibrated = false;
  int calib_good = -1, calib_cand = 0; double calib_one_ms = 0, calib_all_ms = 0;
  struct CalibOrder { hipStream_t s; std::vector<hipStream_t> order; int good, cand; double one_ms, all_ms; };
  std::vector<CalibOrder> calib_cache;
  int calib = 1;
  int ends_join = 0;
  int lstm_pipe = 0;
  int split_batch = 2;
  int merge_advance = 1;
  int rvq_tiled = 1;
  int sea_splitk = 1;
  int split_init = 1;
  int split_ends = 1;
  int fp8_act = 1;
  int part_graphs = 1;
  double host_graph_ms = 0, host_wait_ms = 0;
  long long host_graph_launches = 0;
  hipStream_t side_stream[kMaxParts] = {nullptr, nullptr, nullptr, nullptr};
  hipEvent_t ev_side_fork[kMaxParts] = {nullptr, nullptr, nullptr, nullptr}, ev_side_join[kMaxParts] = {nullptr, nullptr, nullptr, nullptr};
  int side_streams = 0;
  int fuse_kmax = 1;
  int fuse_ln = 1;
  int coop_launch = 0;
  int lstm_xcd = 1;
  int num_cus = 256;
  int xcd_resident[2] = {0, 0};
  int coop_resident[2] = {0, 0};
  int fuse_attn_tail = 1;
  int fold_ctx = 1;
  static constexpr int kFlowRing = 32;
  hipEvent_t flow_ev[kFlowRing] = {};
  unsigned long long flow_n = 0;
  int flow_depth = 8;
  int fuse_gn_stats = 1;
  int gn_epi_max_tiles = 1300;
  int gn_epi_min_l = 0;
  int fold_ln = 1;
  int fold_res = 1;
  int fuse_gn_epi = 1;
  ConvTune tune;
  int lstm_stream_only = 0;
  int serial_parts = 0;
  int graph_steps = 0;
  uint64_t use_tick = 0, call_tick = 0;
  size_t plan_bytes = 0, plan_bytes_cap = (size_t)48 << 30;
  int plan_count_cap = 24;
  int live_pools = 0, next_pool_id = 1;
  int next_win_id = 1;
  uint64_t noise_epoch = 0, cur_key = 0;
  unsigned* dev_flag_host = nullptr;
  unsigned* dev_flag_dev = nullptr;
  int enc_final_act = ACT_NONE;
  unsigned long long* tl_buf = nullptr;
  bool timeline = false;
  bool kstamps = false;
  char* scratch = nullptr;
  size_t scratch_cap = 0;
  void* outnorm_ws = nullptr;
  size_t outnorm_ws_bytes = 0;
  float* state_buf = nullptr;
  size_t state_bytes = 0;
  hipStream_t own_stream = nullptr;
  bool profile = false;
  double prof_ms = 0, prof_flops = 0;
  int64_t prof_launches = 0;
  std::vector<std::pair<hipEvent_t, hipEvent_t>> prof_events;
  std::vector<double> prof_event_flops;
  std::vector<int> prof_event_class;
  std::vector<double> prof_event_bytes;
  std::vector<std::string> prof_event_info;
  double cls_ms[LDC_N_CLASSES] = {}, cls_flops[LDC_N_CLASSES] = {}, cls_bytes[LDC_N_CLASSES] = {};
  int64_t cls_launches[LDC_N_CLASSES] = {};
};

inline hipStream_t pick_stream(ldc_ctx* c, void* s) { return s ? reinterpret_cast<hipStream_t>(s) : c->own_stream; }
inline int check_dev_flag(ldc_ctx* c) {
  const unsigned v = c->dev_flag_host ? *reinterpret_cast<volatile unsigned*>(c->dev_flag_host) : 0u;
  if (v) {
    *reinterpret_cast<volatile unsigned*>(c->dev_flag_host) = 0u;
    if (v == LDC_DEV_BAD_CODE) {
      const uint64_t w = *reinterpret_cast<volatile uint64_t*>(c->dev_flag_host + 2);
      return fail(LDC_E_INVALID, "[bad_code] an RVQ code is outside [0, %d) (e.g. codebook %d, item %d, frame %d); the rows of such "
                                 "codes are NaN", c->codec[LDC_MODEL_COND].bins, (int)(w >> 56), (int)((w >> 32) & 0xffffff), (int)(uint32_t)w);
    }
    if (v == 2)
      return fail(LDC_E_HIP, "device-side failure [gn_wait]: the in-launch GroupNorm exchange of a fused conv timed out (its tiles were "
                             "not all resident in time: is the GPU shared with another process?); the outputs of that call are NaN; "
                             "ldc_set_option(ctx, \"fuse_gn_epi\", 0) restores the separate conv + gn_apply launches");
    if (v == kDevFailCtxRange)
      return fail(LDC_E_HIP, "device-side failure [ctx_range]: the LinearAttention context folded into to_qkv met k values outside the range "
                             "its unshifted exponentials are valid for (a column whose sum of exp(k) is below 2^-100 or reaches 1e26: a k of 60 or more); the "
                             "outputs of that call are wrong; ldc_set_option(ctx, \"fold_ctx\", 0) restores the column maximum and the "
                             "context launch, which shift by it");
    c->lstm_xcd = 0;
    return fail(LDC_E_HIP, "device-side failure [coop_lstm]: cooperative LSTM: the hidden-state exchange timed out (its workgroups were "
                           "not co-resident: is the GPU shared with another process?); the outputs of that call are NaN; "
                           "ldc_set_option(ctx, \"lstm_stream\", 1) selects the streamed LSTM kernel");
  }
  return LDC_OK;
}
inline int finish_stream(ldc_ctx* c, void* s) {
  if (!s) {
    HIPCHK(hipStreamSynchronize(c->own_stream));
    return check_dev_flag(c);
  }
  return LDC_OK;
}
inline uint64_t next_noise_key(ldc_ctx* c, bool draws) {
  c->cur_key = c->cfg.noise_seed ^ (c->noise_epoch * 0x9E3779B97F4A7C15ull);
  if (draws) ++c->noise_epoch;
  return c->cur_key;
}

struct WeightReader {
  ldc_ctx* c;
  int which;
  std::string missing;
  HostTensor* get(const std::string& key, std::initializer_list<int64_t> shape) {
    auto& m = c->raw[which];
    auto it = m.find(key);
    if (it == m.end() && key.rfind("diff_model.", 0) == 0) it = m.find("diffusion.model." + key.substr(11));
    if (it == m.end()) {
      if (missing.size() < 600) missing += key + " ";
      return nullptr;
    }
    HostTensor& t = it->second;
    if (t.shape != std::vector<int64_t>(shape)) {
      if (missing.size() < 600) missing += key + "(shape) ";
      return nullptr;
    }
    t.used = true;
    return &t;
  }
};

struct ConvSpec {
  int dt = DT_F32;
  int cin1 = 0, cin2 = 0, cout = 0, k = 1, stride = 1, dil = 1, pad_left = 0, ups = 0, pad_mode = PAD_ZERO;
  int pre_act = ACT_NONE, post_act = ACT_NONE;
  int no_w8 = 0;
  int act8 = 0;
};

struct StreamConvState { int rows = 0, ch = 0; float* buf[2] = {nullptr, nullptr}; };
struct ldc_stream {
  ldc_ctx* ctx = nullptr;
  int which = 0, side = 0, B = 0, hop = 1, min_first = 0;
  std::vector<StreamConvState> convs;
  std::vector<float*> lstm;
  int* fresh_dev = nullptr;
  std::vector<int> fresh_host;
  int parity = 0;
  size_t conv_at = 0, lstm_at = 0;
  hipStream_t last_stream = nullptr;
  bool touched = false;
  bool poisoned = false;
  DevMem mem;
};

// ... 75 lines not shown
```

### ladiffcodec_amd/csrc/ldc_kernels.h

```cpp
#pragma once
#include <hip/hip_runtime.h>
#include <stdint.h>

#include "ldc_windows.h"

namespace ldc {

enum { DT_F32 = 0, DT_BF16 = 1, DT_FP8 = 2 };
enum { ACT_NONE = 0, ACT_SILU = 1, ACT_ELU = 2, ACT_TANH = 3, ACT_GELU = 4, ACT_SIGMOID = 5, ACT_RELU = 6 };
enum { PAD_ZERO = 0, PAD_REFLECT = 1 };
static constexpr int kGnPad = 16;

inline size_t dt_size(int dt) { return dt == DT_F32 ? 4 : (dt == DT_FP8 ? 1 : 2); }

struct ConvLayer {
  int dt = DT_F32;
  int cin1 = 0, cin2 = 0;
  int n = 0;
  int n_pad = 0;
  int bn = 128;
  int taps = 1, stride = 1, dil = 1, pad_left = 0, ups = 0, pad_mode = PAD_ZERO;
  int pre_act = ACT_NONE, post_act = ACT_NONE;
  int tr_stride = 0, tr_cout = 0, tr_trim_left = 0;
  void* w = nullptr;
// ... 79 lines not shown
uint8_t host_f32_to_e4m3(float f);
float host_e4m3_to_f32(uint8_t v);
void pack_convtr_weights(const ConvLayer& ly, const float* w_iok, int cin, int cout, int stride, void* dst_host);
int conv_pick_bn(int n);

hipError_t launch_gn_stats(int dt, const void* x, int B, int L, int C, int groups, float* stats, hipStream_t s, const int* lens = nullptr,
                           int shift = 0);
hipError_t launch_gn_apply(int dt, const void* x, void* y, const void* residual, int B, int L, int C, int groups,
                           const float* stats, const float* gamma, const float* beta, const float* ss_table,
                           int ss_stride, const int* t_ptr, int act, hipStream_t s, void* y_ln = nullptr, const float* ln_g = nullptr, int out8 = 0,
                           const int* lens = nullptr, int shift = 0,
                           int t_stride = 0, int t_rows = 0);
bool gn_apply_ln_fusable(int C);
hipError_t launch_ln_rows(int dt, const void* x, void* y, const void* residual, const float* g, int rows, int C,
                          hipStream_t s, int out8 = 0, const int* lens = nullptr, int shift = 0, int L = 0);
hipError_t launch_mask_rows(int dt, void* x, int B, int L, int C, const int* lens, int shift, hipStream_t s);
hipError_t launch_act(int dt, const void* x, void* y, int64_t n, int act, hipStream_t s, int out8 = 0);

hipError_t launch_linattn(int dt, const void* qkv, void* out, float* ctx_ws, int B, int L, int heads, int dim_head,
                          bool kmax_fused, hipStream_t s, const int* lens = nullptr, int shift = 0, bool ws_zeroed = false);
size_t linattn_ws_floats_per_item(int heads, int dim_head);
bool linattn_tail_supported(int dt, int heads, int dim_head, int C);
hipError_t launch_linattn_ctx(int dt, const void* qkv, float* ctx_ws, int B, int L, int heads, int dim_head, hipStream_t s);
hipError_t launch_linattn_tail(int dt, const void* qkv, const float* ctx_ws, const void* wo_packed, int n_pad, const float* bias, const float* gain,
                               const void* resid, void* out, int B, int L, int heads, int dim_head, int C, unsigned* fail_flag, hipStream_t s);
hipError_t launch_linattn_kmax(int dt, const void* qkv, float* ctx_ws, int B, int L, int heads, int dim_head, hipStream_t s,
                               const int* lens = nullptr, int shift = 0);
constexpr float kLinattnKClamp = 60.0f;
constexpr float kLinattnKsumMin = 7.888609052210118e-31f;
constexpr float kLinattnKsumMax = 1.0e26f;
constexpr unsigned kDevFailCtxRange = 4u;
hipError_t launch_attn_full(int dt, const void* qkv, void* out, int B, int L, int heads, int dim_head, hipStream_t s, const int* lens = nullptr,
                            int shift = 0);

hipError_t launch_to_cl(int dt, const float* x_bcl, void* y_blc, int B, int C, int L, const float* maxabs,
                        int maxabs_per_item, float eps, hipStream_t s);
hipError_t launch_from_cl(int dt, const void* x_blc, float* y_bcl, int B, int C, int L, const float* maxabs,
                          int maxabs_per_item, float eps, hipStream_t s);
hipError_t launch_maxabs(int dt, const void* x, int B, int64_t n_per_item, int per_item, float* maxabs,
                         hipStream_t s);
struct StepTables {
  const float* sqrt_recip_alphas_cumprod;
  const float* sqrt_recipm1_alphas_cumprod;
  const float* posterior_mean_coef1;
  const float* posterior_mean_coef2;
  const float* posterior_log_variance_clipped;
};
hipError_t launch_random_fill(float* x, int64_t n, int uniform, uint64_t seed, unsigned step, hipStream_t s);
hipError_t launch_axpby(float* x, const float* y, float a, float b, int64_t n, hipStream_t s);
hipError_t launch_p_sample_update(int dt, float* x, const void* eps_cl, const float* noise, int64_t noise_step_stride,
                                  void* x_cl, int B, int C, int L, StepTables tb, const int* st,
                                  uint64_t elem_base, hipStream_t s, const int* lens = nullptr,
                                  const uint64_t* item_keys = nullptr);
hipError_t launch_item_keys_write(uint64_t* dst, const uint64_t* keys_host, int n, hipStream_t s);
struct DdimStep;
struct ItemState {
  int t;
  int j;
  unsigned key_lo, key_hi;
  int remaining;
  int len;
  int active;
  int pad_;
  const float* noise;
  const DdimStep* sched;
};
constexpr int kItemStateInts = (int)(sizeof(ItemState) / sizeof(int));
hipError_t launch_items_write(ItemState* dst, const ItemState* src_host, int n, int* lens, int* flens, int up, hipStream_t s);
hipError_t launch_step_begin_items(ItemState* items, int B, int* st, void* zero, size_t zero_bytes, int advance, hipStream_t s);
hipError_t launch_p_sample_update_items(int dt, float* x, int64_t x_item_stride, const void* eps_cl, void* x_cl, int B, int C, int Lmax,
                                        StepTables tb, const ItemState* items, int T, hipStream_t s);
struct DdimStep {
  int t;
  int last;
  float sqrt_an;
  float c;
  float sigma;
  float pad_[3];
};
hipError_t launch_ddim_table_write(DdimStep* dst, const DdimStep* src_host, int n, hipStream_t s);
hipError_t launch_ddim_update(int dt, float* x, const void* eps_cl, const float* noise, int64_t noise_step_stride,
                              void* x_cl, int B, int C, int L, StepTables tb, const DdimStep* sched, const int* st,
                              uint64_t elem_base, hipStream_t s, const int* lens = nullptr, const uint64_t* item_keys = nullptr);
struct DpmStep {
  int t;
  int last;
  int has_prev;
  float a;
  float b0;
  float b1;
  float pad_[2];
};
hipError_t launch_dpm_table_write(DpmStep* dst, const DpmStep* src_host, int n, hipStream_t s);
hipError_t launch_dpm_update(int dt, float* x, const void* eps_cl, float* x0_prev, void* x_cl, int B, int C, int L, StepTables tb,
                             const DpmStep* sched, const int* st, hipStream_t s, const int* lens = nullptr);
struct WinGroupTables {
  const WinGroupTile* tile;
  const WinGroupRec* rec;
  const int* cover;
  const float* weight;
  const int* start;
  const int* wrec;
  int n_tiles, R, Lw;
};
enum { WIN_BLEND = 0, WIN_DDPM = 1, WIN_DDIM = 2, WIN_DPM = 3 };
hipError_t launch_windows_group_update(int dt, int kind, float* x, const void* eps_cl, const float* noise, int64_t noise_step_stride, void* x_cl,
                                       float* ebar, int C, WinGroupTables gt, StepTables tb, const DdimStep* sched, const int* st, hipStream_t s);
hipError_t launch_windows_group_dpm_update(int dt, float* x, const void* eps_cl, float* x0_prev, void* x_cl, int C, WinGroupTables gt, StepTables tb,
                                           const DpmStep* sched, const int* st, hipStream_t s);
hipError_t launch_windows_group_gather(int dt, const float* x, void* y, int W, int C, int Lw, WinGroupTables gt, int div, hipStream_t s);
hipError_t launch_windows_group_keys(WinGroupRec* rec, const uint64_t* keys_host, int R, hipStream_t s);
hipError_t launch_scale_by_maxabs(int dt, void* x, int B, int64_t n_per_item, const float* maxabs, int per_item,
                                  float eps, hipStream_t s);
hipError_t launch_resample(const float* wav, int C, int64_t T, const float* bank, int orig, int nnew, int width, int64_t target, float* out,
                           hipStream_t s);
hipError_t launch_scale_copy(int dt, const void* x, void* y, int B, int64_t n_per_item, const float* maxabs, float eps,
                             hipStream_t s);
hipError_t launch_step_advance(int* st, unsigned long long* tl, hipStream_t s);
hipError_t launch_step_begin(const float* table, int stride, int* st, float* cur, unsigned long long* tl, hipStream_t s,
                             void* zero = nullptr, size_t zero_bytes = 0, int advance = 0, const DdimStep* ddim = nullptr);
hipError_t launch_step_begin_sched(const float* table, int stride, int* st, float* cur, unsigned long long* tl, hipStream_t s, void* zero,
                                   size_t zero_bytes, int advance, const int* t_words, int t_stride_ints);
hipError_t launch_step_set(int* st, int t, int j, uint64_t noise_key, hipStream_t s);
hipError_t launch_clock_sample(unsigned long long* out2, hipStream_t s);
hipError_t launch_spin_us(unsigned us, hipStream_t s);
hipError_t launch_output_normalise(float* x, int B, int64_t n_per_item, int per_item, void* ws, hipStream_t s, const int* lens = nullptr,
                                   int lens_unit = 1);
hipError_t launch_lens_write(int* dst, const int* src_host, int n, hipStream_t s);
hipError_t launch_mask_codes(int64_t* codes, int n_q, int B, int F, const int* flens, hipStream_t s);
size_t output_normalise_ws_bytes(int B);

hipError_t launch_conv_cin1(int dt, const float* x, void* y, const float* w, const float* bias, int B, int L, int Cout,
                            int k, hipStream_t s, int* route_out = nullptr,
                            const float* ctx = nullptr, const int* fresh = nullptr);
hipError_t launch_stream_ctx_update(const float* x, const float* cur, float* nxt, const int* fresh, int B, int L, int P, int C, int zero_pad,
                                    hipStream_t s);
struct LstmSeq {
  int t0 = 0, t1 = 0;
  long long pre_bs = 0, pre_ts = 1, out_bs = 0, out_ts = 1, skip_bs = 0, skip_ts = 1;
  float* state = nullptr;
  const int* fresh = nullptr;
};
struct LstmCarry {
  float* state = nullptr;
  const int* fresh = nullptr;
};
bool lstm_seq_supported(int H);
hipError_t launch_lstm_seq(int dt, const void* pre, const float* w_hh, void* out, const void* skip, int B, int H, const LstmSeq& q,
                           hipStream_t s);
hipError_t launch_lstm_layer(int dt, const void* pre, const float* w_hh, void* out, const void* skip, int B, int T,
                             int H, hipStream_t s, LstmCarry carry = LstmCarry());
bool lstm_coop_eligible(int H);
size_t lstm_coop_ws_bytes(int H);
bool lstm_coop_resident(int H);
int conv_fused_gn_wgs_per_cu(int dt, bool w8);
int lstm_xcd_resident(int H);
hipError_t launch_lstm_coop(int dt, const void* pre, const float* w_rm, void* out, const void* skip, int B, int T, int H,
                            void* ws, unsigned* host_flag, int coop_launch, hipStream_t s, LstmCarry carry = LstmCarry());

hipError_t launch_rvq(const float* z_rows, int rows, int D, const float* codebooks, const float* cb_sqnorm, int bins,
                      int n_q, int64_t* codes, float* quantized_rows, hipStream_t s, int variant = 1);
constexpr unsigned LDC_DEV_BAD_CODE = 3u;
hipError_t launch_rvq_dequant(const int64_t* codes, const uint8_t* packed, int64_t packed_stride, int bits, int n_q, int B_total, int b0,
                              int Bk, int F, const float* codebooks, int bins, int D, float* quantized_rows, unsigned* flag, hipStream_t s,
                              const int* flens = nullptr);
hipError_t launch_sqnorm_rows(const float* x, int rows, int D, float* out, hipStream_t s);

hipError_t launch_q_sample(const float* x0, const float* noise, const int64_t* t, const float* sqrt_ac, const float* sqrt_1mac, int B,
                           int64_t n_per_item, float* out, int T, hipStream_t s);
hipError_t launch_predict_x_start(const float* x_t, const float* eps, const int64_t* t, const float* sqrt_recip_ac, const float* sqrt_recipm1_ac,
                                  int B, int64_t n_per_item, float* out, int T, hipStream_t s);
hipError_t launch_neg_sdsdr(const float* est, const float* tgt, int B, int64_t n_per_item, float clip_min, float* per_item, hipStream_t s);
size_t l1_loss_ws_bytes(int B);
hipError_t launch_l1_loss(const float* pred, const float* target, const int64_t* t, const float* p2w, int B, int64_t n_per_item,
                          float* loss, float* grad, void* ws, int T, hipStream_t s);
size_t train_block_ws_floats(int B, int Cin, int Cout, int L, int groups);
hipError_t launch_train_pw_forward(const float* x, const float* w, const float* bias, int B, int Cin, int Cout, int L, int pre_silu, float* y,
                                   hipStream_t s);
hipError_t launch_train_pw_backward(const float* dy, const float* x, const float* w, int B, int Cin, int Cout, int L, int pre_silu, float* dx,
                                    float* dw, float* db, hipStream_t s);
size_t train_linattn_ws_floats(int B, int H, int D, int N);
hipError_t launch_train_linattn_forward(const float* qkv, int B, int H, int D, int N, float* o, float* ws, hipStream_t s);
hipError_t launch_train_linattn_backward(const float* d_o, const float* qkv, int B, int H, int D, int N, float* ws, float* dqkv, hipStream_t s);
hipError_t launch_train_conv_forward(const float* x, const float* w, const float* bias, int B, int Cin, int Cout, int Lin, int K, int S, int P,
                                     float* y, hipStream_t s);
hipError_t launch_train_conv_backward(const float* dy, const float* x, const float* w, int B, int Cin, int Cout, int Lin, int K, int S, int P,
                                      float* dx, float* dw, float* db, hipStream_t s);
hipError_t launch_train_upsample2(const float* in, int64_t rows, int L, int backward, float* out, hipStream_t s);
hipError_t launch_train_act(const float* x, const float* dy, int64_t n, int kind, float* out, hipStream_t s);
size_t train_attn_ws_floats(int B, int H, int N);
hipError_t launch_train_attn_forward(const float* qkv, int B, int H, int D, int N, float* out, float* ws, hipStream_t s);
hipError_t launch_train_attn_backward(const float* d_o, const float* qkv, int B, int H, int D, int N, float* ws, float* dqkv, hipStream_t s);
hipError_t launch_train_convtr_forward(const float* x, const float* w, const float* bias, int B, int Cin, int Cout, int L, int r, float* y,
                                       hipStream_t s);
hipError_t launch_train_convtr_backward(const float* dy, const float* x, const float* w, int B, int Cin, int Cout, int L, int r, float* dx,
                                        float* dw, float* db, hipStream_t s);
hipError_t launch_train_maxscale(const float* x, const float* dy, int B, int64_t n_per_item, float* out, hipStream_t s);
extern int g_train_bf16;
extern int g_train_fp32_mfma;
hipError_t launch_mm3_forward(const float* x, const float* w, const float* bias, int B, int Cin, int Cout, int Lin, int Lout, int K, int S, int P,
                              float* y, hipStream_t s);
hipError_t launch_mm3_dx(const float* dy, const float* w, int B, int Cin, int Cout, int Lin, int Lout, int K, int S, int P, float* dx, hipStream_t s,
                         const float* bias = nullptr);
hipError_t launch_mm3_dw(const float* dy, const float* x, int B, int Cin, int Cout, int Lin, int Lout, int K, int S, int P, float* dw, hipStream_t s,
                         float* db = nullptr);
extern hipStream_t g_train_side_stream;
extern int g_train_dw_side;
hipStream_t train_side_stream();
hipError_t launch_train_join(hipStream_t s);
extern int g_train_valu;
hipError_t launch_adam(float* p, const float* g, float* m, float* v, int64_t n, int step, float lr, float b1, float b2, float eps, hipStream_t s);
hipError_t launch_adam_dev(float* p, const float* g, float* m, float* v, int64_t n, int* step_dev, float lr, float b1, float b2, float eps, hipStream_t s);
hipError_t launch_train_ln_forward(const float* x, const float* g, int B, int C, int L, float* y, float* stats, hipStream_t s);
hipError_t launch_train_ln_backward(const float* dy, const float* x, const float* g, const float* stats, int B, int C, int L, float* dx,
                                    float* dg, hipStream_t s);
hipError_t launch_train_block_forward(const float* x, const float* w, const float* bias, const float* gamma, const float* beta,
                                      const float* ss, int B, int Cin, int Cout, int L, int groups, float* y, float* ws, hipStream_t s);
hipError_t launch_train_block_backward(const float* dy, const float* x, const float* gamma, const float* beta, const float* ss, int B,
                                       int Cin, int Cout, int L, int groups, float* ws, float* dx, float* dw, float* db, float* dgamma,
                                       float* dbeta, float* dss, hipStream_t s);

hipError_t launch_pack_codes(const int64_t* codes, int n_q, int B, int F, int bits, uint8_t* out, int64_t out_stride, hipStream_t s);
hipError_t launch_unpack_codes(const uint8_t* in, int64_t in_stride, int n_q, int B, int F, int bits, int64_t* codes, hipStream_t s);
hipError_t launch_build_cdf(const float* pdf, int rows, int card, int total_range_bits, float roundoff, int min_range, int* cdf,
                            hipStream_t s);
hipError_t launch_ac_encode(const int* symbols, const int* cdf, int B, int S, int card, int mode, int period, int total_range_bits,
                            uint8_t* out, int64_t out_stride, int64_t cap, int64_t* nbytes, hipStream_t s, const int* n_sym = nullptr);
hipError_t launch_ac_decode(const uint8_t* in, int64_t in_stride, const int64_t* nbytes, const int* cdf, int B, int S, int card, int mode,
                            int period, int total_range_bits, int* symbols, int* status, hipStream_t s, const int* n_sym = nullptr);

}
```

### ladiffcodec_amd/csrc/seanet.hip

```cpp
#include <type_traits>
#include "ldc_kernels.h"
#include "ldc_math.h"

namespace ldc {

__device__ __forceinline__ float sbf2f(unsigned short h) { return __uint_as_float(((unsigned)h) << 16); }
__device__ __forceinline__ unsigned short sf2bf(float f) { return hw_bf16(f); }
template <typename T>
__device__ __forceinline__ float sld(const void* p, size_t i);
template <>
__device__ __forceinline__ float sld<float>(const void* p, size_t i) { return reinterpret_cast<const float*>(p)[i]; }
template <>
__device__ __forceinline__ float sld<__bf16>(const void* p, size_t i) {
  return sbf2f(reinterpret_cast<const unsigned short*>(p)[i]);
}
template <typename T>
__device__ __forceinline__ void sst(void* p, size_t i, float v);
template <>
__device__ __forceinline__ void sst<float>(void* p, size_t i, float v) { reinterpret_cast<float*>(p)[i] = v; }
template <>
__device__ __forceinline__ void sst<__bf16>(void* p, size_t i, float v) {
  reinterpret_cast<unsigned short*>(p)[i] = sf2bf(v);
}

// ... 106 lines not shown
hipError_t launch_stream_ctx_update(const float* x, const float* cur, float* nxt, const int* fresh, int B, int L, int P, int C, int zero_pad,
                                    hipStream_t s) {
  if (B <= 0 || L <= 0 || P <= 0 || C <= 0 || !fresh || cur == nxt) return hipErrorInvalidValue;
  const int V = C % 4 == 0 ? 4 : 1;
  const long n = (long)B * P * (C / V);
  const dim3 grid((unsigned)((n + 255) / 256));
  if (V == 4) hipLaunchKernelGGL(stream_ctx_update_kernel<4>, grid, dim3(256), 0, s, x, cur, nxt, fresh, B, L, P, C, zero_pad);
  else hipLaunchKernelGGL(stream_ctx_update_kernel<1>, grid, dim3(256), 0, s, x, cur, nxt, fresh, B, L, P, C, zero_pad);
  return hipGetLastError();
}

__device__ __forceinline__ float sigmoid_acc(float v) { return 1.0f / (1.0f + expf(-v)); }

template <typename T, int H>
__global__ __launch_bounds__(4 * H) void lstm_reg_kernel(const void* pre, const float* w_hh, void* out, const void* skip,
                                                         const LstmSeq q) {
  constexpr int KS = H / 4;
  constexpr int KP = KS + 4;
  __shared__ __attribute__((aligned(16))) float sh[4 * KP];
  __shared__ float sg[4 * H];
  const int b = blockIdx.x, tid = threadIdx.x;
  const int rg = tid >> 2, g = tid & 3;
  float w[4][KS];
#pragma unroll
  for (int q = 0; q < 4; ++q)
#pragma unroll
    for (int k = 0; k < KS; k += 4) {
      const float4 v = *reinterpret_cast<const float4*>(w_hh + (size_t)(rg * 4 + q) * H + g * KS + k);
      w[q][k] = v.x; w[q][k + 1] = v.y; w[q][k + 2] = v.z; w[q][k + 3] = v.w;
    }
  const int row = tid;
  const bool resume = q.state && (q.fresh ? !q.fresh[b] : q.t0 > 0);
  float c = (resume && row < H) ? q.state[(size_t)b * 2 * H + H + row] : 0.f;
  float h_last = (resume && row < H) ? q.state[(size_t)b * 2 * H + row] : 0.f;
  if (row < H) sh[row + 4 * (row / KS)] = h_last;
  float p_next[4] = {0.f, 0.f, 0.f, 0.f};
  const size_t pre0 = (size_t)b * q.pre_bs, out0 = (size_t)b * q.out_bs, skip0 = (size_t)b * q.skip_bs;
  if (row < H) {
#pragma unroll
    for (int gq = 0; gq < 4; ++gq) p_next[gq] = sld<T>(pre, (pre0 + (size_t)q.t0 * q.pre_ts) * (4 * H) + gq * H + row);
  }
  float sk_next = (skip && row < H) ? sld<T>(skip, (skip0 + (size_t)q.t0 * q.skip_ts) * H + row) : 0.f;
  __syncthreads();
  for (int t = q.t0; t < q.t1; ++t) {
    const float p_cur[4] = {p_next[0], p_next[1], p_next[2], p_next[3]};
    const float sk = sk_next;
    if (t + 1 < q.t1 && row < H) {
#pragma unroll
      for (int gq = 0; gq < 4; ++gq) p_next[gq] = sld<T>(pre, (pre0 + (size_t)(t + 1) * q.pre_ts) * (4 * H) + gq * H + row);
      if (skip) sk_next = sld<T>(skip, (skip0 + (size_t)(t + 1) * q.skip_ts) * H + row);
    }
    typedef float f32x2 __attribute__((ext_vector_type(2)));
    f32x2 a01[4], a23[4];
#pragma unroll
    for (int q = 0; q < 4; ++q) { a01[q] = f32x2{0.f, 0.f}; a23[q] = f32x2{0.f, 0.f}; }
#pragma unroll
    for (int k = 0; k < KS; k += 4) {
      const float4 hv = *reinterpret_cast<const float4*>(&sh[g * KP + k]);
      const f32x2 h01 = {hv.x, hv.y}, h23 = {hv.z, hv.w};
#pragma unroll
      for (int q = 0; q < 4; ++q) {
        const f32x2 w01 = {w[q][k], w[q][k + 1]}, w23 = {w[q][k + 2], w[q][k + 3]};
        a01[q] = __builtin_elementwise_fma(w01, h01, a01[q]);
        a23[q] = __builtin_elementwise_fma(w23, h23, a23[q]);
      }
    }
#pragma unroll
    for (int q = 0; q < 4; ++q) {
      float v = (a01[q][0] + a01[q][1]) + (a23[q][0] + a23[q][1]);
      v += __int_as_float(__builtin_amdgcn_update_dpp(0, __float_as_int(v), 0xB1, 0xf, 0xf, true));
      v += __int_as_float(__builtin_amdgcn_update_dpp(0, __float_as_int(v), 0x4E, 0xf, 0xf, true));
      if (g == q) sg[rg * 4 + q] = v;
    }
    __syncthreads();
    if (row < H) {
      const float ig = fast_sigmoid(sg[row] + p_cur[0]), fg = fast_sigmoid(sg[H + row] + p_cur[1]);
      const float gg = fast_tanh(sg[2 * H + row] + p_cur[2]), og = fast_sigmoid(sg[3 * H + row] + p_cur[3]);
      c = fg * c + ig * gg;
      const float h = og * fast_tanh(c);
      h_last = h;
      sh[row + 4 * (row / KS)] = h;
      const size_t o = (out0 + (size_t)t * q.out_ts) * H + row;
      sst<T>(out, o, h + sk);
    }
    __syncthreads();
  }
  if (q.state && row < H) {
    q.state[(size_t)b * 2 * H + row] = h_last;
    q.state[(size_t)b * 2 * H + H + row] = c;
  }
}

template <typename T>
__global__ __launch_bounds__(1024) void lstm_stream_kernel(const void* pre, const float* w_km, void* out, const void* skip,
                                                           int T_len, int H, const LstmCarry carry) {
  extern __shared__ __attribute__((aligned(16))) float sm[];
  float* sh = sm;
  float* sg = sm + H;
  const int b = blockIdx.x, tid = threadIdx.x;
  const int G = 4 * H;
  const float* st_in = (carry.state && !carry.fresh[b]) ? carry.state + (size_t)b * 2 * H : nullptr;
  for (int i = tid; i < H; i += 1024) sh[i] = st_in ? st_in[i] : 0.f;
  float c_state[4] = {0.f, 0.f, 0.f, 0.f};
  if (st_in) {
    int ci = 0;
    for (int j = tid; j < H; j += 1024, ++ci) c_state[ci] = st_in[H + j];
  }
  __syncthreads();
  for (int t = 0; t < T_len; ++t) {
    for (int row = tid; row < G; row += 1024) {
      float acc0 = 0.f, acc1 = 0.f;
      const float4* wp = reinterpret_cast<const float4*>(w_km) + row;
      for (int k4 = 0; k4 < H / 4; k4 += 2) {
        const float4 w0 = wp[(size_t)k4 * G];
        const float4 w1 = wp[(size_t)(k4 + 1) * G];
        const float4 h0 = *reinterpret_cast<const float4*>(&sh[4 * k4]);
        const float4 h1 = *reinterpret_cast<const float4*>(&sh[4 * k4 + 4]);
        acc0 += w0.x * h0.x + w0.y * h0.y + w0.z * h0.z + w0.w * h0.w;
        acc1 += w1.x * h1.x + w1.y * h1.y + w1.z * h1.z + w1.w * h1.w;
      }
      sg[row] = acc0 + acc1 + sld<T>(pre, ((size_t)b * T_len + t) * G + row);
    }
    __syncthreads();
    int ci = 0;
    for (int j = tid; j < H; j += 1024, ++ci) {
      const float ig = sigmoid_acc(sg[j]), fg = sigmoid_acc(sg[H + j]);
      const float gg = tanhf(sg[2 * H + j]), og = sigmoid_acc(sg[3 * H + j]);
      const float c = fg * c_state[ci] + ig * gg;
      c_state[ci] = c;
      const float h = og * tanhf(c);
      sh[j] = h;
      const size_t o = ((size_t)b * T_len + t) * H + j;
      sst<T>(out, o, skip ? h + sld<T>(skip, o) : h);
    }
    __syncthreads();
  }
  if (carry.state) {
    int ci = 0;
    for (int j = tid; j < H; j += 1024, ++ci) {
      carry.state[(size_t)b * 2 * H + j] = sh[j];
      carry.state[(size_t)b * 2 * H + H + j] = c_state[ci];
    }
  }
}

constexpr int LSTM_COOP_SHARDS = 8;
constexpr int LSTM_COOP_SHARD_STRIDE = 16;
size_t lstm_coop_ws_bytes(int H) { return (size_t)2 * 32 * H * sizeof(float) + 256 * sizeof(unsigned); }

using f32x4 = __attribute__((ext_vector_type(4))) float;

template <typename T, int H>
__global__ __launch_bounds__(256) void lstm_coop_kernel(const void* pre, const float* w_hh, void* out, const void* skip,
                                                        int B, int T_len, float* hbuf, unsigned* sync, unsigned* host_flag, const LstmCarry carry) {
  constexpr int KW = H / 4;
  constexpr int NI = KW / 16;
  __shared__ float part[4][2][16][16];
  __shared__ int s_dead;
  const int tid = threadIdx.x, lane = tid & 63, w = tid >> 6;
  const int j = blockIdx.x, nb = gridDim.x;
  const int n = lane & 15, q = lane >> 4;
  const int MT = (B + 15) / 16;
  f32x4 breg[NI];
  {
    const size_t row = (size_t)(n >> 2) * H + 4 * j + (n & 3);
#pragma unroll
    for (int jj = 0; jj < NI; ++jj) breg[jj] = *reinterpret_cast<const f32x4*>(w_hh + row * H + w * KW + 16 * jj + 4 * q);
  }
  if (tid == 0) s_dead = 0;
  const int ob = tid >> 2, ou = tid & 3;
  const bool owner = tid < 4 * B;
  float c_state = 0.f;
  float pnext[4] = {0.f, 0.f, 0.f, 0.f};
  float sknext = 0.f;
  if (owner) {
#pragma unroll
    for (int g = 0; g < 4; ++g) pnext[g] = sld<T>(pre, ((size_t)ob * T_len) * (4 * H) + g * H + 4 * j + ou);
    if (skip) sknext = sld<T>(skip, ((size_t)ob * T_len) * H + 4 * j + ou);
    if (carry.state && !carry.fresh[ob]) c_state = carry.state[(size_t)ob * 2 * H + H + 4 * j + ou];
  }
  float h_last = 0.f;
  __syncthreads();
  bool dead = false;
  int t = 0;
  for (; t < T_len; ++t) {
    f32x4 acc[2] = {{0.f, 0.f, 0.f, 0.f}, {0.f, 0.f, 0.f, 0.f}};
    if (t > 0) {
      if (w == 0) {
        const unsigned target = (unsigned)(t * (nb / LSTM_COOP_SHARDS));
        unsigned spins = 0;
        for (;;) {
          unsigned v = target;
          if (lane < LSTM_COOP_SHARDS) v = __hip_atomic_load(sync + lane * LSTM_COOP_SHARD_STRIDE, __ATOMIC_RELAXED, __HIP_MEMORY_SCOPE_AGENT);
          const unsigned flag = lane == 0 ? __hip_atomic_load(sync + 200, __ATOMIC_RELAXED, __HIP_MEMORY_SCOPE_AGENT) : 0u;
          if (__any(flag != 0u) || ++spins > 400000u) {
            if (lane == 0) { __hip_atomic_store(sync + 200, 1u, __ATOMIC_RELAXED, __HIP_MEMORY_SCOPE_AGENT); s_dead = 1; }
            break;
          }
          if (__all(v >= target)) break;
          __builtin_amdgcn_s_sleep(2);
        }
      }
      __syncthreads();
      if (s_dead) { dead = true; break; }
    }
    if (t > 0 || carry.state) {
      const float* hp = hbuf + (size_t)((t + 1) & 1) * 32 * H;
      f32x4 areg[2][NI];
#pragma unroll
      for (int mt = 0; mt < 2; ++mt) {
        if (mt < MT) {
          const int item = min(mt * 16 + n, B - 1);
#pragma unroll
          for (int jj = 0; jj < NI; ++jj) {
            const float* src = hp + (size_t)item * H + w * KW + 16 * jj + 4 * q;
            asm volatile("global_load_dwordx4 %0, %1, off sc0 sc1" : "=v"(areg[mt][jj]) : "v"(src) : "memory");
          }
        }
      }
      asm volatile("s_waitcnt vmcnt(0)" ::: "memory");
#pragma unroll
      for (int mt = 0; mt < 2; ++mt)
        if (mt < MT) {
#pragma unroll
          for (int jj = 0; jj < NI; ++jj) asm volatile("" : "+v"(areg[mt][jj]));
        }
#pragma unroll
      for (int jj = 0; jj < NI; ++jj) {
#pragma unroll
        for (int e = 0; e < 4; ++e) {
          acc[0] = __builtin_amdgcn_mfma_f32_16x16x4f32(areg[0][jj][e], breg[jj][e], acc[0], 0, 0, 0);
          if (MT > 1) acc[1] = __builtin_amdgcn_mfma_f32_16x16x4f32(areg[1][jj][e], breg[jj][e], acc[1], 0, 0, 0);
        }
      }
    }
#pragma unroll
    for (int mt = 0; mt < 2; ++mt)
#pragma unroll
      for (int r = 0; r < 4; ++r) part[w][mt][4 * q + r][n] = acc[mt][r];
    __syncthreads();
    if (owner) {
      float gates[4];
#pragma unroll
      for (int g = 0; g < 4; ++g) {
        const int col = g * 4 + ou;
        gates[g] = pnext[g] + ((part[0][ob >> 4][ob & 15][col] + part[1][ob >> 4][ob & 15][col]) +
                               (part[2][ob >> 4][ob & 15][col] + part[3][ob >> 4][ob & 15][col]));
      }
      const float ig = sigmoid_acc(gates[0]), fg = sigmoid_acc(gates[1]);
      const float gg = tanhf(gates[2]), og = sigmoid_acc(gates[3]);
      c_state = fg * c_state + ig * gg;
      const float h = og * tanhf(c_state);
      h_last = h;
      __hip_atomic_store(hbuf + (size_t)(t & 1) * 32 * H + (size_t)ob * H + 4 * j + ou, h, __ATOMIC_RELAXED, __HIP_MEMORY_SCOPE_AGENT);
      asm volatile("s_waitcnt vmcnt(0)" ::: "memory");
      const size_t o = ((size_t)ob * T_len + t) * H + 4 * j + ou;
      sst<T>(out, o, h + sknext);
      if (t + 1 < T_len) {
#pragma unroll
        for (int g = 0; g < 4; ++g) pnext[g] = sld<T>(pre, ((size_t)ob * T_len + t + 1) * (4 * H) + g * H + 4 * j + ou);
        if (skip) sknext = sld<T>(skip, o + H);
      }
    }
    __syncthreads();
    if (tid == 0 && t + 1 < T_len)
      __hip_atomic_fetch_add(sync + (j % LSTM_COOP_SHARDS) * LSTM_COOP_SHARD_STRIDE, 1u, __ATOMIC_RELAXED, __HIP_MEMORY_SCOPE_AGENT);
  }
  if (dead && owner) {
    for (int tt = t; tt < T_len; ++tt) sst<T>(out, ((size_t)ob * T_len + tt) * H + 4 * j + ou, __builtin_nanf(""));
  }
  if (carry.state && owner) {
    carry.state[(size_t)ob * 2 * H + 4 * j + ou] = dead ? __builtin_nanf("") : h_last;
    carry.state[(size_t)ob * 2 * H + H + 4 * j + ou] = dead ? __builtin_nanf("") : c_state;
  }
  if (dead && tid == 0 && host_flag) __hip_atomic_store(host_flag, 1u, __ATOMIC_RELAXED, __HIP_MEMORY_SCOPE_SYSTEM);
}

template <int G>
__device__ __forceinline__ float dpp_sum_group(float v) {
  auto dpp = [](float x, auto ctrl) {
    return __int_as_float(__builtin_amdgcn_update_dpp(0, __float_as_int(x), decltype(ctrl)::value, 0xf, 0xf, true));
  };
  v += dpp(v, std::integral_constant<int, 0xB1>());
  v += dpp(v, std::integral_constant<int, 0x4E>());
  v += dpp(v, std::integral_constant<int, 0x141>());
  if (G >= 16) v += dpp(v, std::integral_constant<int, 0x140>());
  if (G >= 32) v += __shfl_xor(v, 16);
  if (G >= 64) v += __shfl_xor(v, 32);
  return v;
}

template <typename T, int H>
__global__ __launch_bounds__(1024) void lstm_xcd_kernel(const void* pre, const float* w_hh, void* out, const void* skip,
                                                        int B, int T_len, float* hbuf, unsigned* sync, unsigned* host_flag, unsigned long long* dbg = nullptr,
                                                        const LstmCarry carry = LstmCarry()) {
  constexpr int NB = 16;
  constexpr int U = H / NB;
  constexpr int ROWS = 4 * U;
  constexpr int RPT = 2;
  constexpr int KSEG = 1024 / (ROWS / RPT);
  constexpr int KS = H / KSEG;
  constexpr int NV = KS / 4;
  constexpr int KPAD = KS >= 8 ? 4 : 0;
  __shared__ float sgate[2][ROWS];
  __shared__ __attribute__((aligned(16))) float sh[2][H + KPAD * KSEG];
  __shared__ int s_dead, s_rank;
  const int tid = threadIdx.x, lane = tid & 63, w = tid >> 6;
  const unsigned xcc = __builtin_amdgcn_s_getreg((20 << 0) | (0 << 6) | ((4 - 1) << 11)) & 7u;
  if (xcc != 0u) return;
  if (tid == 0) {
    s_rank = (int)__hip_atomic_fetch_add(sync + 202, 1u, __ATOMIC_RELAXED, __HIP_MEMORY_SCOPE_AGENT);
    s_dead = 0;
  }
  __syncthreads();
  const int j = s_rank;
  if (j >= NB) return;
  unsigned* flags = sync;
  const int rg = tid / KSEG, g = tid % KSEG;
  f32x4 wreg[RPT][NV];
#pragma unroll
  for (int q = 0; q < RPT; ++q) {
    const int r = rg * RPT + q;
    const size_t row = (size_t)(r / U) * H + (size_t)j * U + (r % U);
#pragma unroll
    for (int v = 0; v < NV; ++v) wreg[q][v] = *reinterpret_cast<const f32x4*>(w_hh + row * H + g * KS + 4 * v);
  }
  const int ob = tid / U, ou = tid % U;
  const bool owner = tid < U * B;
  float c_state = 0.f;
  float pnext[4] = {0.f, 0.f, 0.f, 0.f};
  float sknext = 0.f;
  if (owner) {
#pragma unroll
    for (int gg = 0; gg < 4; ++gg) pnext[gg] = sld<T>(pre, ((size_t)ob * T_len) * (4 * H) + gg * H + j * U + ou);
    if (skip) sknext = sld<T>(skip, ((size_t)ob * T_len) * H + j * U + ou);
    if (carry.state && !carry.fresh[ob]) c_state = carry.state[(size_t)ob * 2 * H + H + j * U + ou];
  }
  float h_last = 0.f;
  bool dead = false;
  int t = 0;
  for (; t < T_len; ++t) {
    float dot[2][RPT];
#pragma unroll
    for (int q = 0; q < RPT; ++q) dot[0][q] = dot[1][q] = 0.f;
    unsigned long long st0 = 0, st1 = 0, st2 = 0, st3 = 0, st4 = 0, st5 = 0;
    const bool rec = dbg && j == 3 && tid == 0 && t >= 16 && t < 48;
    if (rec) st0 = __builtin_amdgcn_s_memtime();
    if (t > 0 || carry.state) {
      if (t > 0 && w == 0) {
        const unsigned long long t0 = wall_clock64();
        for (unsigned spins = 0;; ++spins) {
          const bool ok = lane >= NB || __hip_atomic_load(flags + lane, __ATOMIC_RELAXED, __HIP_MEMORY_SCOPE_AGENT) >= (unsigned)t;
          if (__all(ok)) break;
          if ((spins & 255u) == 255u) {
            const unsigned flag = lane == 0 ? __hip_atomic_load(sync + 200, __ATOMIC_RELAXED, __HIP_MEMORY_SCOPE_AGENT) : 0u;
            if (__any(flag != 0u) || wall_clock64() - t0 > 20000000ull) {
              if (lane == 0) { __hip_atomic_store(sync + 200, 1u, __ATOMIC_RELAXED, __HIP_MEMORY_SCOPE_AGENT); s_dead = 1; }
              break;
            }
          }
        }
      }
      __syncthreads();
      if (rec) st1 = __builtin_amdgcn_s_memtime();
      if (s_dead) { dead = true; break; }
      const float* hp = hbuf + (size_t)((t + 1) & 1) * 32 * H;
      if (tid < B * (H / 4)) {
        const int b = tid / (H / 4), v = tid % (H / 4);
        f32x4 hv;
        asm volatile("global_load_dwordx4 %0, %1, off sc1\n\ts_waitcnt vmcnt(0)" : "=&v"(hv) : "v"(hp + (size_t)b * H + 4 * v) : "memory");
        *reinterpret_cast<f32x4*>(&sh[b][4 * v + KPAD * ((4 * v) / KS)]) = hv;
      }
      __syncthreads();
      if (rec) st2 = __builtin_amdgcn_s_memtime();
#pragma unroll
      for (int b = 0; b < 2; ++b)
        if (b < B) {
#pragma unroll
          for (int v = 0; v < NV; ++v) {
            const f32x4 hv = *reinterpret_cast<const f32x4*>(&sh[b][g * (KS + KPAD) + 4 * v]);
#pragma unroll
            for (int q = 0; q < RPT; ++q)
#pragma unroll
              for (int e = 0; e < 4; ++e) dot[b][q] = fmaf(hv[e], wreg[q][v][e], dot[b][q]);
          }
        }
#pragma unroll
      for (int b = 0; b < 2; ++b)
        if (b < B) {
#pragma unroll
          for (int q = 0; q < RPT; ++q) dot[b][q] = dpp_sum_group<KSEG>(dot[b][q]);
        }
    }
    if (g == 0) {
#pragma unroll
      for (int q = 0; q < RPT; ++q) {
        sgate[0][rg * RPT + q] = dot[0][q];
        sgate[1][rg * RPT + q] = dot[1][q];
      }
    }
    __syncthreads();
    if (rec) st3 = __builtin_amdgcn_s_memtime();
    if (owner) {
      float gates[4];
#pragma unroll
      for (int gg = 0; gg < 4; ++gg) gates[gg] = pnext[gg] + sgate[ob][gg * U + ou];
      const float ig = sigmoid_acc(gates[0]), fg = sigmoid_acc(gates[1]);
      const float gv = tanhf(gates[2]), og = sigmoid_acc(gates[3]);
      c_state = fg * c_state + ig * gv;
      const float h = og * tanhf(c_state);
      h_last = h;
      asm volatile("global_store_dword %0, %1, off" ::"v"(hbuf + (size_t)(t & 1) * 32 * H + (size_t)ob * H + j * U + ou), "v"(h) : "memory");
      asm volatile("s_waitcnt vmcnt(0)" ::: "memory");
      if (rec) st4 = __builtin_amdgcn_s_memtime();
      const size_t o = ((size_t)ob * T_len + t) * H + j * U + ou;
      sst<T>(out, o, h + sknext);
      if (t + 1 < T_len) {
#pragma unroll
        for (int gg = 0; gg < 4; ++gg) pnext[gg] = sld<T>(pre, ((size_t)ob * T_len + t + 1) * (4 * H) + gg * H + j * U + ou);
        if (skip) sknext = sld<T>(skip, o + H);
      }
    }
    __syncthreads();
    if (tid == 0 && t + 1 < T_len) {
      asm volatile("global_store_dword %0, %1, off" ::"v"(flags + j), "v"((unsigned)(t + 1)) : "memory");
    }
    if (rec) { st5 = __builtin_amdgcn_s_memtime(); unsigned long long* o = dbg + (size_t)(t - 16) * 6; o[0] = st0; o[1] = st1; o[2] = st2; o[3] = st3; o[4] = st4; o[5] = st5; }
  }
  if (dead && owner) {
    for (int tt = t; tt < T_len; ++tt) sst<T>(out, ((size_t)ob * T_len + tt) * H + j * U + ou, __builtin_nanf(""));
  }
  if (carry.state && owner) {
    carry.state[(size_t)ob * 2 * H + j * U + ou] = dead ? __builtin_nanf("") : h_last;
    carry.state[(size_t)ob * 2 * H + H + j * U + ou] = dead ? __builtin_nanf("") : c_state;
  }
  if (dead && tid == 0 && host_flag) __hip_atomic_store(host_flag, 1u, __ATOMIC_RELAXED, __HIP_MEMORY_SCOPE_SYSTEM);
}

__global__ __launch_bounds__(256) void lstm_state_publish_kernel(const LstmCarry carry, float* hdst, int nb, int H) {
  const int idx = blockIdx.x * 256 + threadIdx.x;
  if (idx >= nb * H) return;
  const int b = idx / H, u = idx - b * H;
  hdst[(size_t)b * H + u] = carry.fresh[b] ? 0.f : carry.state[(size_t)b * 2 * H + u];
}

template <typename T>
static hipError_t lstm_coop_launch(const void* pre, const float* w_rm, void* out, const void* skip, int B, int T_len, int H,
                                   void* ws, unsigned* host_flag, int coop_launch, hipStream_t s, const LstmCarry carry_all) {
  float* hbuf = reinterpret_cast<float*>(ws);
  unsigned* sync = reinterpret_cast<unsigned*>(hbuf + (size_t)2 * 32 * H);
  const size_t esz = sizeof(T);
  for (int b0 = 0; b0 < B; b0 += 32) {
    const int nb = std::min(32, B - b0);
    hipError_t e = hipMemsetAsync(sync, 0, 256 * sizeof(unsigned), s);
    if (e != hipSuccess) return e;
    const char* p = reinterpret_cast<const char*>(pre) + (size_t)b0 * T_len * 4 * H * esz;
    char* o = reinterpret_cast<char*>(out) + (size_t)b0 * T_len * H * esz;
    const char* k = skip ? reinterpret_cast<const char*>(skip) + (size_t)b0 * T_len * H * esz : nullptr;
    const void* pp = p; void* oo = o; const void* kk = k; int nbv = nb, tl = T_len;
    LstmCarry carry;
    if (carry_all.state) {
      carry.state = carry_all.state + (size_t)b0 * 2 * H;
      carry.fresh = carry_all.fresh + b0;
      hipLaunchKernelGGL(lstm_state_publish_kernel, dim3((nb * H + 255) / 256), dim3(256), 0, s, carry, hbuf + (size_t)32 * H, nb, H);
      if ((e = hipGetLastError()) != hipSuccess) return e;
    }
    void* args[] = {&pp, &w_rm, &oo, &kk, &nbv, &tl, &hbuf, &sync, &host_flag, &carry};
    const void* fn = H == 512 ? reinterpret_cast<const void*>(lstm_coop_kernel<T, 512>) : reinterpret_cast<const void*>(lstm_coop_kernel<T, 256>);
    if (coop_launch == 2 && nb <= 2) {
      const void* fx = H == 512 ? reinterpret_cast<const void*>(lstm_xcd_kernel<T, 512>) : reinterpret_cast<const void*>(lstm_xcd_kernel<T, 256>);
      static unsigned long long* dbg = nullptr;
      static int dbg_n = 0;
      if (getenv("LDC_LSTM_STAMPS") && !dbg) (void)hipMalloc((void**)&dbg, 32 * 6 * 8);
      void* args2[] = {&pp, &w_rm, &oo, &kk, &nbv, &tl, &hbuf, &sync, &host_flag, &dbg, &carry};
      e = hipLaunchKernel(fx, dim3(8 * 16), dim3(1024), args2, 0, s);
      if (dbg && ++dbg_n == 20) {
        (void)hipStreamSynchronize(s);
        unsigned long long hb[32 * 6];
        (void)hipMemcpy(hb, dbg, sizeof(hb), hipMemcpyDeviceToHost);
        double acc[6] = {0};
        for (int i = 1; i < 32; ++i) {
          acc[0] += (double)(hb[i * 6 + 1] - hb[i * 6 + 0]); acc[1] += (double)(hb[i * 6 + 2] - hb[i * 6 + 1]); acc[2] += (double)(hb[i * 6 + 3] - hb[i * 6 + 2]);
          acc[3] += (double)(hb[i * 6 + 4] - hb[i * 6 + 3]); acc[4] += (double)(hb[i * 6 + 5] - hb[i * 6 + 4]); acc[5] += (double)(hb[i * 6 + 0] - hb[(i - 1) * 6 + 0]);
        }
        fprintf(stderr, "[lstm_xcd] cycles per step: poll %.0f | h load %.0f | dot+reduce %.0f | gates+h store %.0f | rest+flag %.0f | step %.0f\n", acc[0] / 31, acc[1] / 31,
                acc[2] / 31, acc[3] / 31, acc[4] / 31, acc[5] / 31);
      }
    } else if (coop_launch == 1) e = hipLaunchCooperativeKernel(fn, dim3(H / 4), dim3(256), args, 0, s);
    else e = hipLaunchKernel(fn, dim3(H / 4), dim3(256), args, 0, s);
    if (e != hipSuccess) return e;
  }
  return hipSuccess;
}

bool lstm_coop_eligible(int H) { return H == 256 || H == 512; }
int lstm_xcd_resident(int H) {
  if (!lstm_coop_eligible(H)) return 0;
  const void* fn = H == 512 ? reinterpret_cast<const void*>(lstm_xcd_kernel<float, 512>) : reinterpret_cast<const void*>(lstm_xcd_kernel<float, 256>);
  int per_cu = 0, cus = 0, dev = 0;
  if (hipGetDevice(&dev) != hipSuccess || hipDeviceGetAttribute(&cus, hipDeviceAttributeMultiprocessorCount, dev) != hipSuccess ||
      hipOccupancyMaxActiveBlocksPerMultiprocessor(&per_cu, fn, 1024, 0) != hipSuccess) {
    (void)hipGetLastError();
    return 0;
  }
  if (cus % 8 != 0 || per_cu < 1) return 0;
  return per_cu * (cus / 8) / 16;
}

bool lstm_coop_resident(int H) {
  if (!lstm_coop_eligible(H)) return false;
  const void* fn = H == 512 ? reinterpret_cast<const void*>(lstm_coop_kernel<float, 512>) : reinterpret_cast<const void*>(lstm_coop_kernel<float, 256>);
  int dev = 0, per_cu = 0, cus = 0;
  if (hipGetDevice(&dev) != hipSuccess || hipDeviceGetAttribute(&cus, hipDeviceAttributeMultiprocessorCount, dev) != hipSuccess ||
      hipOccupancyMaxActiveBlocksPerMultiprocessor(&per_cu, fn, 256, 0) != hipSuccess) {
    (void)hipGetLastError();
    return false;
  }
  return (long long)std::max(0, per_cu - 1) * cus >= H / 4 || (long long)per_cu * cus >= 2 * (H / 4);
}

hipError_t launch_lstm_coop(int dt, const void* pre, const float* w_rm, void* out, const void* skip, int B, int T, int H,
                            void* ws, unsigned* host_flag, int coop_launch, hipStream_t s, LstmCarry carry) {
  if (!lstm_coop_eligible(H) || (carry.state && !carry.fresh)) return hipErrorInvalidValue;
  return dt == DT_F32 ? lstm_coop_launch<float>(pre, w_rm, out, skip, B, T, H, ws, host_flag, coop_launch, s, carry)
                      : lstm_coop_launch<__bf16>(pre, w_rm, out, skip, B, T, H, ws, host_flag, coop_launch, s, carry);
}

bool lstm_seq_supported(int H) { return H == 64 || H == 128; }

hipError_t launch_lstm_seq(int dt, const void* pre, const float* w_hh, void* out, const void* skip, int B, int H, const LstmSeq& q,
                           hipStream_t s) {
  if (!lstm_seq_supported(H) || q.t1 <= q.t0) return hipErrorInvalidValue;
  if (H == 64) {
    if (dt == DT_F32) hipLaunchKernelGGL((lstm_reg_kernel<float, 64>), dim3(B), dim3(256), 0, s, pre, w_hh, out, skip, q);
    else hipLaunchKernelGGL((lstm_reg_kernel<__bf16, 64>), dim3(B), dim3(256), 0, s, pre, w_hh, out, skip, q);
  } else {
    if (dt == DT_F32) hipLaunchKernelGGL((lstm_reg_kernel<float, 128>), dim3(B), dim3(512), 0, s, pre, w_hh, out, skip, q);
    else hipLaunchKernelGGL((lstm_reg_kernel<__bf16, 128>), dim3(B), dim3(512), 0, s, pre, w_hh, out, skip, q);
  }
  return hipGetLastError();
}

hipError_t launch_lstm_layer(int dt, const void* pre, const float* w_hh, void* out, const void* skip, int B, int T,
                             int H, hipStream_t s, LstmCarry carry) {
  if (H % 8 || H > 4096 || (carry.state && !carry.fresh)) return hipErrorInvalidValue;
  if (H == 64 || H == 128) {
    LstmSeq q;
    q.t0 = 0; q.t1 = T; q.pre_bs = q.out_bs = q.skip_bs = T; q.pre_ts = q.out_ts = q.skip_ts = 1; q.state = carry.state; q.fresh = carry.fresh;
    return launch_lstm_seq(dt, pre, w_hh, out, skip, B, H, q, s);
  } else {
    const size_t lds = (size_t)5 * H * sizeof(float);
    if (dt == DT_F32) hipLaunchKernelGGL(lstm_stream_kernel<float>, dim3(B), dim3(1024), lds, s, pre, w_hh, out, skip, T, H, carry);
    else hipLaunchKernelGGL(lstm_stream_kernel<__bf16>, dim3(B), dim3(1024), lds, s, pre, w_hh, out, skip, T, H, carry);
  }
  return hipGetLastError();
}

}
```

### ladiffcodec_amd/lib.py

```python
from __future__ import annotations

import ctypes as C
import os
import subprocess
from typing import Optional

_HERE = os.path.dirname(os.path.abspath(__file__))
LIB_PATH = os.path.join(_HERE, "libladiffcodec.so")
CSRC = os.path.join(_HERE, "csrc")

LDC_F32, LDC_BF16, LDC_BF16_W8 = 0, 1, 2
DTYPES = {"f32": LDC_F32, "bf16": LDC_BF16, "fp8": LDC_BF16_W8}
MODEL_MAIN, MODEL_COND = 0, 1
MAX_RATIOS = 8
STREAM_ENCODER, STREAM_DECODER = 0, 1

EXPORTS = [
    "ldc_last_error", "ldc_version", "ldc_create", "ldc_destroy", "ldc_reseed", "ldc_set_option", "ldc_quantize_e4m3", "ldc_set_weight", "ldc_finalize_weights",
    "ldc_seanet_encode", "ldc_seanet_decode", "ldc_rvq_encode", "ldc_rvq_decode", "ldc_get_cond",
    "ldc_cond_upsample", "ldc_unet_forward", "ldc_p_sample", "ldc_denoise", "ldc_p_sample_loop", "ldc_infilling", "ldc_output_normalise", "ldc_decode", "ldc_ddim_times", "ldc_ddim_sample", "ldc_decode_ddim", "ldc_decode_codes", "ldc_decode_codes_ddim",
    "ldc_dpm_schedule", "ldc_dpm_sample", "ldc_decode_dpm", "ldc_decode_codes_dpm", "ldc_decode_ragged_dpm",
    "ldc_window_layout", "ldc_window_layout_n", "ldc_window_parts", "ldc_unet_forward_windows", "ldc_denoise_windows", "ldc_ddim_sample_windows", "ldc_decode_windows", "ldc_decode_ddim_windows",
    "ldc_dpm_sample_windows", "ldc_decode_dpm_windows", "ldc_decode_codes_windows", "ldc_decode_codes_dpm_windows",
    "ldc_window_group_layout", "ldc_unet_forward_windows_group", "ldc_sample_windows_group", "ldc_decode_windows_group",
    "ldc_decode_ragged", "ldc_unet_forward_ragged", "ldc_get_cond_ragged", "ldc_decode_codes_ragged", "ldc_ac_encode_ragged", "ldc_ac_decode_ragged",
    "ldc_sample_seeded", "ldc_decode_seeded", "ldc_decode_codes_seeded",
    "ldc_unet_forward_items", "ldc_pool_create", "ldc_pool_destroy", "ldc_pool_admit", "ldc_pool_admit_ddim", "ldc_pool_step", "ldc_pool_remaining", "ldc_pool_take", "ldc_pool_peek", "ldc_pool_evict",
    "ldc_stream_min_first", "ldc_stream_create", "ldc_stream_reset", "ldc_stream_destroy", "ldc_seanet_encode_stream", "ldc_seanet_decode_stream", "ldc_get_cond_stream",
    "ldc_sconv1d", "ldc_sconvtr1d", "ldc_slstm", "ldc_unet_debug_tap", "ldc_unet_step_cost", "ldc_profile_enable",
    "ldc_profile_read", "ldc_profile_read_classes", "ldc_conv_microbench", "ldc_conv_compare", "ldc_conv_compare_fp8", "ldc_ln_fold_compare", "ldc_gn_microbench", "ldc_host_stats", "ldc_graph_schedule", "ldc_stream_info", "ldc_clock_sample", "ldc_debug_raise_failure", "ldc_debug_attn_core", "ldc_debug_attention_block", "ldc_debug_resnet_block", "ldc_debug_sea_conv", "ldc_debug_sea_op", "ldc_debug_sync_count", "ldc_debug_lean_launches", "ldc_xcc_census", "ldc_timeline_enable", "ldc_timeline_read", "ldc_kstamps_enable", "ldc_kstamps_reset", "ldc_kstamps_read", "ldc_packed_bytes", "ldc_pack_codes", "ldc_unpack_codes",
    "ldc_ac_build_cdf", "ldc_ac_encode", "ldc_ac_decode", "ldc_train_q_sample", "ldc_train_num_timesteps", "ldc_train_predict_x_start", "ldc_train_neg_sdsdr", "ldc_train_l1_loss", "ldc_train_block_ws_floats",
    "ldc_train_block_forward", "ldc_train_block_backward", "ldc_train_layernorm_forward", "ldc_train_layernorm_backward", "ldc_train_adam_step", "ldc_train_adam_step_dev", "ldc_train_pointwise_forward", "ldc_train_pointwise_backward", "ldc_train_linattn_ws_floats", "ldc_train_linattn_forward", "ldc_train_linattn_backward", "ldc_train_conv_forward", "ldc_train_conv_backward", "ldc_train_join", "ldc_train_side_stream", "ldc_train_upsample2", "ldc_train_activation", "ldc_train_attn_ws_floats", "ldc_train_attn_forward", "ldc_train_attn_backward", "ldc_train_convtr_forward", "ldc_train_convtr_backward", "ldc_train_maxscale", "ldc_resample_out_len", "ldc_resample",
]


class LdcConfig(C.Structure):
    _fields_ = [
        ("compute_dtype", C.c_int32), ("rep_dims", C.c_int32), ("n_filters", C.c_int32),
        ("n_residual_layers", C.c_int32), ("lstm", C.c_int32), ("n_enc_ratios", C.c_int32),
        ("enc_ratios", C.c_int32 * MAX_RATIOS), ("diff_dims", C.c_int32), ("n_upsampling_ratios", C.c_int32),
        ("upsampling_ratios", C.c_int32 * MAX_RATIOS), ("unet_scale_cond", C.c_int32), ("unet_scale_x", C.c_int32),
        ("has_cond_model", C.c_int32), ("cond_bandwidth", C.c_float), ("max_batch", C.c_int32),
        ("max_latent_len", C.c_int32), ("noise_seed", C.c_uint64), ("final_activation", C.c_int32),
        ("reserved_", C.c_int32),
    ]


FINAL_ACTIVATIONS = {None: 0, "Identity": 0, "Tanh": 1, "Sigmoid": 2, "ELU": 3, "SiLU": 4, "GELU": 5, "ReLU": 6}


E_INVALID, E_STATE, E_MISSING, E_HIP, E_NOMEM = -1, -2, -3, -4, -5


class LdcError(RuntimeError):
    def __init__(self, code: int, msg: str):
        super().__init__(f"libladiffcodec error {code}: {msg}")
        self.code = code


_lib: Optional[C.CDLL] = None


def build(verbose: bool = False) -> str:
    r = subprocess.run(["make", "-C", CSRC, "-j8"], capture_output=True, text=True)
    if verbose or r.returncode != 0:
        print(r.stdout[-4000:])
        print(r.stderr[-8000:])
    if r.returncode != 0:
        raise RuntimeError("building libladiffcodec.so failed")
    return LIB_PATH


def load() -> C.CDLL:
    global _lib
    if _lib is not None:
        return _lib
    path = os.environ.get("LDC_LIB_PATH", LIB_PATH)
    if not os.path.exists(path):
        raise RuntimeError(f"{path} not found: run `python -c 'import __graft_entry__ as g; g.build()'` "
                           f"(or `make -C {CSRC}`). There is no CPU fallback.")
    lib = C.CDLL(path)
    vp, i32, i64p, fp = C.c_void_p, C.c_int, C.POINTER(C.c_int64), C.c_void_p
    lib.ldc_last_error.restype = C.c_char_p
    lib.ldc_version.restype = C.c_char_p
    lib.ldc_create.argtypes = [C.POINTER(LdcConfig), i32, C.POINTER(vp)]
    lib.ldc_destroy.argtypes = [vp]
    lib.ldc_reseed.argtypes = [vp, C.c_uint64]
    lib.ldc_quantize_e4m3.argtypes = [vp, C.c_int64, vp, vp]
    lib.ldc_set_weight.argtypes = [vp, i32, C.c_char_p, vp, i64p, i32]
    lib.ldc_finalize_weights.argtypes = [vp, i32]
    lib.ldc_seanet_encode.argtypes = [vp, i32, fp, i32, i32, fp, vp]
    lib.ldc_seanet_decode.argtypes = [vp, i32, fp, i32, i32, fp, vp]
    lib.ldc_rvq_encode.argtypes = [vp, fp, i32, i32, i32, vp, fp, vp]
    lib.ldc_rvq_decode.argtypes = [vp, vp, i32, i32, i32, fp, vp]
    lib.ldc_get_cond.argtypes = [vp, fp, i32, i32, C.c_float, fp, vp, vp]
    lib.ldc_cond_upsample.argtypes = [vp, fp, i32, i32, i32, fp, vp]
    lib.ldc_unet_forward.argtypes = [vp, fp, i32, fp, i32, i32, i32, fp, vp]
    lib.ldc_p_sample.argtypes = [vp, fp, i32, fp, fp, i32, i32, i32, vp]
    lib.ldc_denoise.argtypes = [vp, fp, fp, fp, i32, i32, i32, i32, vp]
    lib.ldc_p_sample_loop.argtypes = [vp, fp, fp, fp, i32, i32, i32, i32, vp]
    lib.ldc_infilling.argtypes = [vp, fp, fp, fp, i32, fp, C.c_float, i32, i32, i32, i32, vp]
    lib.ldc_output_normalise.argtypes = [vp, fp, i32, i32, i32, vp]
    lib.ldc_decode.argtypes = [vp, fp, i32, i32, i32, fp, i32, fp, fp, fp, vp, vp]
    lib.ldc_ddim_times.argtypes = [i32, i32, C.POINTER(C.c_int)]
    lib.ldc_graph_schedule.argtypes = [i32, i32, i32, i32, C.POINTER(C.c_int), C.POINTER(C.c_int), C.POINTER(C.c_int)]
    lib.ldc_ddim_sample.argtypes = [vp, fp, fp, fp, i32, i32, i32, C.c_float, i32, i32, i32, vp]
    lib.ldc_decode_ddim.argtypes = [vp, fp, i32, i32, i32, i32, C.c_float, fp, i32, fp, fp, fp, vp, vp]
    lib.ldc_decode_codes.argtypes = [vp, vp, vp, C.c_int64, i32, i32, i32, i32, i32, fp, i32, fp, fp, fp, vp]
    lib.ldc_decode_codes_ddim.argtypes = [vp, vp, vp, C.c_int64, i32, i32, i32, i32, i32, i32, C.c_float, fp, i32, fp, fp, fp, vp]
    lib.ldc_decode_ragged.argtypes = [vp, fp, C.POINTER(C.c_int32), i32, i32, i32, i32, C.c_float, fp, fp, fp, fp, vp, vp]
    lib.ldc_get_cond_ragged.argtypes = [vp, fp, C.POINTER(C.c_int32), i32, i32, C.c_float, fp, vp, vp]
    lib.ldc_decode_codes_ragged.argtypes = [vp, vp, vp, C.c_int64, i32, i32, i32, i32, C.POINTER(C.c_int32), i32, i32, C.c_float, fp, fp, fp, fp, vp]
    lib.ldc_dpm_schedule.argtypes = [fp, fp, i32, i32, i32, C.POINTER(C.c_int), C.POINTER(C.c_float)]
    lib.ldc_dpm_sample.argtypes = [vp, fp, fp, i32, i32, i32, i32, i32, vp]
    lib.ldc_decode_dpm.argtypes = [vp, fp, i32, i32, i32, i32, i32, fp, fp, fp, vp, vp]
    lib.ldc_decode_codes_dpm.argtypes = [vp, vp, vp, C.c_int64, i32, i32, i32, i32, i32, i32, i32, fp, fp, fp, vp]
    lib.ldc_decode_ragged_dpm.argtypes = [vp, fp, C.POINTER(C.c_int32), i32, i32, i32, i32, fp, fp, fp, vp, vp]
    lib.ldc_window_layout.argtypes = [i32, i32, i32, i32, C.POINTER(C.c_int), C.POINTER(C.c_float)]
    lib.ldc_window_layout_n.argtypes = [i32, i32, i32, i32, i32, C.POINTER(C.c_int), C.POINTER(C.c_float)]
    lib.ldc_window_parts.argtypes = [i32, i32, C.POINTER(C.c_int)]
    lib.ldc_unet_forward_windows.argtypes = [vp, fp, i32, fp, i32, i32, i32, i32, fp, vp]
    lib.ldc_denoise_windows.argtypes = [vp, fp, fp, fp, i32, i32, i32, i32, i32, vp]
    lib.ldc_ddim_sample_windows.argtypes = [vp, fp, fp, fp, i32, i32, C.c_float, i32, i32, i32, i32, vp]
    lib.ldc_decode_windows.argtypes = [vp, fp, i32, i32, fp, i32, i32, fp, fp, fp, vp, vp]
    lib.ldc_decode_ddim_windows.argtypes = [vp, fp, i32, i32, i32, C.c_float, fp, i32, i32, fp, fp, fp, vp, vp]
    lib.ldc_dpm_sample_windows.argtypes = [vp, fp, fp, i32, i32, i32, i32, i32, i32, vp]
    lib.ldc_decode_dpm_windows.argtypes = [vp, fp, i32, i32, i32, i32, i32, fp, fp, fp, vp, vp]
    lib.ldc_decode_codes_windows.argtypes = [vp, vp, vp, C.c_int64, i32, i32, i32, i32, i32, C.c_float, fp, i32, i32, fp, fp, fp, vp]
    lib.ldc_decode_codes_dpm_windows.argtypes = [vp, vp, vp, C.c_int64, i32, i32, i32, i32, i32, i32, i32, fp, fp, fp, vp]
    ip, u64p = C.POINTER(C.c_int), C.POINTER(C.c_uint64)
    lib.ldc_window_group_layout.argtypes = [i32, ip, i32, i32, i32, ip, ip, C.POINTER(C.c_float)]
    lib.ldc_unet_forward_windows_group.argtypes = [vp, fp, i32, fp, i32, ip, ip, i32, i32, fp, vp]
    lib.ldc_sample_windows_group.argtypes = [vp, fp, fp, i32, i32, i32, C.c_float, fp, u64p, i32, ip, ip, i32, i32, vp]
    lib.ldc_decode_windows_group.argtypes = [vp, fp, i32, ip, i32, i32, i32, C.c_float, fp, u64p, i32, i32, fp, fp, fp, vp, vp]
    lib.ldc_sample_seeded.argtypes = [vp, fp, fp, i32, i32, i32, C.c_float, u64p, i32, i32, i32, vp]
    lib.ldc_decode_seeded.argtypes = [vp, fp, C.POINTER(C.c_int32), i32, i32, i32, i32, i32, C.c_float, u64p, fp, fp, fp, vp, vp]
    lib.ldc_decode_codes_seeded.argtypes = [vp, vp, vp, C.c_int64, i32, i32, i32, i32, C.POINTER(C.c_int32), i32, i32, i32, C.c_float, u64p, fp, fp,
                                            fp, vp]
    lib.ldc_ac_encode_ragged.argtypes = [vp, vp, vp, vp, i32, i32, i32, i32, i32, vp, C.c_int64, vp, vp]
    lib.ldc_ac_decode_ragged.argtypes = [vp, vp, C.c_int64, vp, vp, vp, i32, i32, i32, i32, i32, vp, vp, vp]
    lib.ldc_unet_forward_ragged.argtypes = [vp, fp, i32, fp, C.POINTER(C.c_int32), i32, i32, i32, fp, vp]
    lib.ldc_unet_forward_items.argtypes = [vp, fp, C.POINTER(C.c_int32), fp, C.POINTER(C.c_int32), i32, i32, i32, fp, vp]
    lib.ldc_pool_create.argtypes = [vp, i32, i32, C.POINTER(vp)]
    lib.ldc_pool_destroy.argtypes = [vp]
    lib.ldc_pool_admit.argtypes = [vp, vp, i32, fp, fp, i32, i32, fp, C.c_uint64, vp]
    lib.ldc_pool_admit_ddim.argtypes = [vp, vp, i32, fp, fp, i32, i32, i32, C.c_float, fp, C.c_uint64, vp]
    lib.ldc_pool_step.argtypes = [vp, vp, i32, vp]
    lib.ldc_pool_remaining.argtypes = [vp, C.POINTER(C.c_int32)]
    lib.ldc_pool_take.argtypes = [vp, vp, i32, fp, vp]
    lib.ldc_pool_peek.argtypes = [vp, vp, i32, fp, vp]
    lib.ldc_pool_evict.argtypes = [vp, i32]
    lib.ldc_stream_min_first.argtypes = [C.POINTER(LdcConfig), i32, i32]
    lib.ldc_stream_create.argtypes = [vp, i32, i32, i32, C.POINTER(vp)]
    lib.ldc_stream_reset.argtypes = [vp, vp, vp]
    lib.ldc_stream_destroy.argtypes = [vp]
    lib.ldc_seanet_encode_stream.argtypes = [vp, vp, fp, i32, fp, vp]
    lib.ldc_seanet_decode_stream.argtypes = [vp, vp, fp, i32, fp, vp]
    lib.ldc_get_cond_stream.argtypes = [vp, vp, fp, i32, C.c_float, fp, vp, vp]
    lib.ldc_sconv1d.argtypes = [vp, fp, i32, i32, i32, vp, vp, i32, i32, i32, i32, i32, i32, fp, vp]
    lib.ldc_sconvtr1d.argtypes = [vp, fp, i32, i32, i32, vp, vp, i32, i32, i32, i32, fp, vp]
    lib.ldc_slstm.argtypes = [vp, fp, i32, i32, i32, C.POINTER(vp), i32, fp, vp]
    lib.ldc_unet_debug_tap.argtypes = [vp, C.c_char_p, fp, C.c_int64, vp]
    lib.ldc_unet_step_cost.argtypes = [vp, i32, i32, C.POINTER(C.c_double), C.POINTER(C.c_double)]
    lib.ldc_profile_enable.argtypes = [vp, i32]
    lib.ldc_profile_read.argtypes = [vp, C.POINTER(C.c_double), C.POINTER(C.c_int64), C.POINTER(C.c_double)]
    lib.ldc_profile_read_classes.argtypes = [vp, C.c_int, C.POINTER(C.c_double), C.POINTER(C.c_int64), C.POINTER(C.c_double), C.POINTER(C.c_double)]
    lib.ldc_set_option.argtypes = [vp, C.c_char_p, i32]
    lib.ldc_train_num_timesteps.argtypes = [vp]
    lib.ldc_train_predict_x_start.argtypes = [vp, vp, vp, vp, i32, i32, i32, vp, vp]
    lib.ldc_train_neg_sdsdr.argtypes = [vp, vp, vp, i32, C.c_int64, C.c_float, vp, vp]
    lib.ldc_host_stats.argtypes = [vp, i32, C.POINTER(C.c_double), C.POINTER(C.c_double), C.POINTER(C.c_int64)]
    lib.ldc_stream_info.argtypes = [vp, C.POINTER(C.c_int), C.POINTER(C.c_int), C.POINTER(C.c_double), C.POINTER(C.c_double), C.POINTER(C.c_int)]
    lib.ldc_clock_sample.argtypes = [vp, C.POINTER(C.c_uint64), vp]
    lib.ldc_xcc_census.argtypes = [vp, vp, i32, i32, vp]
    lib.ldc_conv_microbench.argtypes = [vp, i32, i32, i32, i32, i32, i32, i32, i32, i32, i32, C.POINTER(C.c_double)]
    lib.ldc_conv_compare.argtypes = [vp] + [i32] * 13 + [C.POINTER(C.c_double)] * 3
    lib.ldc_conv_compare_fp8.argtypes = [vp] + [i32] * 10 + [C.POINTER(C.c_double)] * 3
    lib.ldc_ln_fold_compare.argtypes = [vp, i32, i32, i32, i32, C.c_double, C.POINTER(C.c_double), C.POINTER(C.c_double)]
    lib.ldc_debug_attn_core.argtypes = [vp, i32, fp, i32, i32, vp, vp, vp, fp, i32, fp, vp]
    lib.ldc_debug_attention_block.argtypes = [vp, C.c_char_p, fp, i32, i32, fp, vp]
    lib.ldc_debug_resnet_block.argtypes = [vp, C.c_char_p, fp, fp, i32, i32, i32, C.POINTER(i32), i32, C.POINTER(i32), i32, fp, fp, vp, fp, fp, C.POINTER(i32), vp]
    lib.ldc_debug_sea_conv.argtypes = [vp, fp, i32, i32, i32, vp, vp, i32, i32, i32, i32, i32, i32, i32, fp, fp, C.POINTER(i32), vp]
    lib.ldc_debug_sea_op.argtypes = [vp, i32, i32, i32, fp, i32, i32, fp, C.c_int64, C.POINTER(i32), vp]
    lib.ldc_timeline_enable.argtypes = [vp, i32]
    lib.ldc_timeline_read.argtypes = [vp, i32, i32, C.POINTER(C.c_uint64)]
    lib.ldc_kstamps_enable.argtypes = [vp, i32]
    lib.ldc_kstamps_reset.argtypes = [vp]
    lib.ldc_kstamps_read.argtypes = [vp, i32, i32, C.POINTER(i32), C.POINTER(C.c_uint64), C.c_char_p, i32, C.POINTER(i32)]
    lib.ldc_packed_bytes.argtypes = [i32, i32, i32]
    lib.ldc_pack_codes.argtypes = [vp, vp, i32, i32, i32, i32, vp, C.c_int64, vp]
    lib.ldc_unpack_codes.argtypes = [vp, vp, C.c_int64, i32, i32, i32, i32, vp, vp]
    lib.ldc_ac_build_cdf.argtypes = [vp, vp, i32, i32, i32, C.c_float, i32, vp, vp]
    lib.ldc_ac_encode.argtypes = [vp, vp, vp, i32, i32, i32, i32, i32, vp, C.c_int64, vp, vp]
    lib.ldc_ac_decode.argtypes = [vp, vp, C.c_int64, vp, vp, i32, i32, i32, i32, i32, vp, vp, vp]
    lib.ldc_train_q_sample.argtypes = [vp, fp, vp, fp, i32, i32, i32, fp, vp]
    lib.ldc_train_l1_loss.argtypes = [vp, fp, fp, vp, i32, i32, i32, fp, fp, vp]
    lib.ldc_train_block_ws_floats.argtypes = [i32, i32, i32, i32, i32]
    lib.ldc_train_block_forward.argtypes = [vp, fp, fp, fp, fp, fp, fp, i32, i32, i32, i32, i32, fp, fp, vp]
    lib.ldc_train_block_backward.argtypes = [vp, fp, fp, fp, fp, fp, i32, i32, i32, i32, i32, fp, fp, fp, fp, fp, fp, fp, vp]
    lib.ldc_train_layernorm_forward.argtypes = [vp, fp, fp, i32, i32, i32, fp, fp, vp]
    lib.ldc_train_layernorm_backward.argtypes = [vp, fp, fp, fp, fp, i32, i32, i32, fp, fp, vp]
    lib.ldc_train_pointwise_forward.argtypes = [vp, fp, fp, fp, i32, i32, i32, i32, i32, fp, vp]
    lib.ldc_train_pointwise_backward.argtypes = [vp, fp, fp, fp, i32, i32, i32, i32, i32, fp, fp, fp, vp]
    lib.ldc_train_linattn_ws_floats.argtypes = [i32, i32, i32, i32]
    lib.ldc_train_linattn_ws_floats.restype = C.c_int64
    lib.ldc_train_linattn_forward.argtypes = [vp, fp, i32, i32, i32, i32, fp, fp, vp]
    lib.ldc_train_linattn_backward.argtypes = [vp, fp, fp, i32, i32, i32, i32, fp, fp, vp]
    lib.ldc_train_conv_forward.argtypes = [vp, fp, fp, fp, i32, i32, i32, i32, i32, i32, i32, fp, vp]
    lib.ldc_train_conv_backward.argtypes = [vp, fp, fp, fp, i32, i32, i32, i32, i32, i32, i32, fp, fp, fp, vp]
    lib.ldc_train_join.argtypes = [vp, vp]
    lib.ldc_train_side_stream.argtypes = [vp, C.POINTER(C.c_void_p)]
    lib.ldc_train_upsample2.argtypes = [vp, fp, C.c_int64, i32, i32, fp, vp]
    lib.ldc_train_activation.argtypes = [vp, fp, fp, C.c_int64, i32, fp, vp]
    lib.ldc_train_attn_ws_floats.argtypes = [i32, i32, i32]
    lib.ldc_train_attn_forward.argtypes = [vp, fp, i32, i32, i32, i32, fp, fp, vp]
    lib.ldc_train_attn_backward.argtypes = [vp, fp, fp, i32, i32, i32, i32, fp, fp, vp]
    lib.ldc_train_convtr_forward.argtypes = [vp, fp, fp, fp, i32, i32, i32, i32, i32, fp, vp]
    lib.ldc_train_convtr_backward.argtypes = [vp, fp, fp, fp, i32, i32, i32, i32, i32, fp, fp, fp, vp]
    lib.ldc_train_maxscale.argtypes = [vp, fp, fp, i32, C.c_int64, fp, vp]
    lib.ldc_train_adam_step.argtypes = [vp, fp, fp, fp, fp, C.c_int64, i32, C.c_float, C.c_float, C.c_float, C.c_float, vp]
    lib.ldc_train_adam_step_dev.argtypes = [vp, fp, fp, fp, fp, C.c_int64, vp, C.c_float, C.c_float, C.c_float, C.c_float, vp]
    lib.ldc_resample_out_len.argtypes = [C.c_int64, i32, i32]
    lib.ldc_resample.argtypes = [vp, fp, i32, C.c_int64, i32, i32, fp, vp]
    optional = {"ldc_debug_lean_launches"} if "LDC_LIB_PATH" in os.environ else set()
    if hasattr(lib, "ldc_debug_lean_launches"):
        lib.ldc_debug_lean_launches.argtypes = [i32]
    lib.ldc_gn_microbench.argtypes = [vp, i32, i32, i32, i32, i32, i32, C.POINTER(C.c_double)]
    for name in EXPORTS:
        if name in optional and not hasattr(lib, name):
            continue
        fn = getattr(lib, name)
        if name in ("ldc_debug_sync_count", "ldc_debug_lean_launches", "ldc_packed_bytes", "ldc_train_block_ws_floats", "ldc_train_linattn_ws_floats", "ldc_train_attn_ws_floats", "ldc_resample_out_len"):
            fn.restype = C.c_int64
        elif name == "ldc_quantize_e4m3":
            fn.restype = None
        elif name not in ("ldc_last_error", "ldc_version"):
            fn.restype = C.c_int
    _lib = lib
    return lib


def ddim_times(t_start: int, n_steps: int):
    out = (C.c_int * (int(n_steps) + 1))() if n_steps >= 0 else (C.c_int * 1)()
    check(load().ldc_ddim_times(int(t_start), int(n_steps), out))
    return list(out)


def window_layout(Ltot: int, Lw: int, overlap: int, up: int, max_windows: int = 32):
    import numpy as np
    lib = load()
    max_windows = int(max_windows)
    if max_windows == 32:
        def call(starts, weights):
            return lib.ldc_window_layout(int(Ltot), int(Lw), int(overlap), int(up), starts, weights)
    else:
        def call(starts, weights):
            return lib.ldc_window_layout_n(int(Ltot), int(Lw), int(overlap), int(up), max_windows, starts, weights)
    starts = (C.c_int * max(32, max_windows))()
    W = call(starts, None)
    if W < 0:
        check(W)
    lw = min(int(Lw), int(Ltot))
    weights = (C.c_float * (W * lw))()
    check(min(0, call(starts, weights)))
    return list(starts)[:W], np.array(weights, dtype=np.float32).reshape(W, lw)


def window_group_layout(Ltot, Lw: int, overlap: int, up: int):
    import numpy as np
    lib = load()
    lens = [int(v) for v in Ltot]
    R = len(lens)
    arr = (C.c_int * max(1, R))(*lens)
    w0 = (C.c_int * (R + 1))()
    starts = (C.c_int * 32)()
    W = lib.ldc_window_group_layout(R, arr, int(Lw), int(overlap), int(up), w0, starts, None)
    if W < 0:
        check(W)
    weights = (C.c_float * (W * int(Lw)))()
    check(min(0, lib.ldc_window_group_layout(R, arr, int(Lw), int(overlap), int(up), w0, starts, weights)))
    return list(w0), list(starts)[:W], np.array(weights, dtype=np.float32).reshape(W, int(Lw))


def window_parts(W: int, parts: int):
    first = (C.c_int * (max(1, int(parts)) + 1))()
    p_eff = load().ldc_window_parts(int(W), int(parts), first)
    if p_eff < 0:
        check(p_eff)
    return list(first)[:p_eff + 1]


def dpm_schedule(sqrt_recip, sqrt_recipm1, t_start: int, n_steps: int):
    import numpy as np
    R = np.ascontiguousarray(np.asarray(sqrt_recip, dtype=np.float32))
    M = np.ascontiguousarray(np.asarray(sqrt_recipm1, dtype=np.float32))
    if R.ndim != 1 or R.shape != M.shape:
        raise ValueError("the two tables must be one-dimensional and of one length")
    n = max(int(n_steps), 1)
    t_out, coef = (C.c_int * n)(), (C.c_float * (3 * n))()
    check(load().ldc_dpm_schedule(R.ctypes.data, M.ctypes.data, int(R.shape[0]), int(t_start), int(n_steps), t_out, coef))
    return np.array(t_out, dtype=np.int32), np.array(coef, dtype=np.float32).reshape(n, 3)


def stream_min_first(cfg: LdcConfig, which: int, side: int) -> int:
    n = load().ldc_stream_min_first(C.byref(cfg), int(which), int(side))
    if n < 0:
        check(n)
    return n


def check(rc: int) -> None:
    if rc != 0:
        raise LdcError(rc, load().ldc_last_error().decode("utf-8", "replace"))
```

Baseline: 692.4 audio-s/wall-s.

## Enable chunked two-layer LSTM wavefront pipelining by default, including cooperative kernel path

Splits the two stacked SEANet LSTM layers into time chunks so that layer 1's input projection and recurrence for chunk k run on an aux stream while layer 0 works on chunk k+1. The path is now on by default with 4 chunks, and the cooperative (large-H) LSTM kernel gains stride parameters and carried state so it can take part. Residency checks now count how many cooperative teams fit, requiring room for two concurrent teams. The aim is to hide the serial recurrence latency of the second layer, at the cost of extra launches, event syncs and the risk of two persistent cooperative kernels competing for CUs.

```diff
diff --git a/include/ladiffcodec.h b/include/ladiffcodec.h
--- a/include/ladiffcodec.h
+++ b/include/ladiffcodec.h
@@ -296,6 +296,7 @@
 int ldc_debug_raise_failure(ldc_ctx* ctx, int code);
 long long ldc_debug_sync_count(void);
 long long ldc_debug_lean_launches(int kind);
+long long ldc_debug_lstm_wavefronts(void);
 
 int ldc_host_stats(ldc_ctx* ctx, int reset, double* graph_launch_ms, double* lookahead_wait_ms, int64_t* graph_launches);
 int ldc_graph_schedule(int n_steps, int parts, int strided, int graph_steps_option, int* K_out, int* n_big_out, int* n_single_out);
diff --git a/ladiffcodec_amd/csrc/ldc_api.cpp b/ladiffcodec_amd/csrc/ldc_api.cpp
--- a/ladiffcodec_amd/csrc/ldc_api.cpp
+++ b/ladiffcodec_amd/csrc/ldc_api.cpp
@@ -675,8 +675,8 @@
   }
   c->xcd_resident[0] = lstm_xcd_resident(256);
   c->xcd_resident[1] = lstm_xcd_resident(512);
-  c->coop_resident[0] = lstm_coop_resident(256) ? 1 : 0;
-  c->coop_resident[1] = lstm_coop_resident(512) ? 1 : 0;
+  c->coop_resident[0] = lstm_coop_teams(256);
+  c->coop_resident[1] = lstm_coop_teams(512);
   c->plan_bytes_cap = (size_t)48 << 30;
   c->plan_count_cap = 24;
   if (const char* mp = getenv("LDC_AUX_FROM_SIDE")) {
@@ -839,6 +839,7 @@
   LDC_OPT("gn_nap0", c->tune.gn_nap0, true, 0, 4096)
   LDC_OPT("lstm_stream", c->lstm_stream_only, false, 0, 1)
   LDC_OPT("lstm_xcd", c->lstm_xcd, false, 0, 1)
+  LDC_OPT("lstm_wavefront", c->lstm_wavefront, false, 0, ldc_ctx::kLstmChunks)
   LDC_OPT("lstm_pipe", c->lstm_pipe, false, 0, 1)
   LDC_OPT("coop_launch", c->coop_launch, false, 0, 1)
   LDC_OPT("sea_splitk", c->sea_splitk, false, 0, 1)
@@ -875,6 +876,8 @@
 }
 
 extern "C" long long ldc_debug_sync_count(void) { return g_device_syncs; }
+static long long g_lstm_wavefronts = 0;
+extern "C" long long ldc_debug_lstm_wavefronts(void) { return g_lstm_wavefronts; }
 
 extern "C" int ldc_debug_raise_failure(ldc_ctx* c, int code) {
   if (!c || !c->dev_flag_host || (code != 1 && code != 2 && code != (int)kDevFailCtxRange)) return fail(LDC_E_INVALID, "bad arguments");
@@ -1075,27 +1078,52 @@
       case SeaOp::LSTM: {
         const int H = op.cout;
         const void* in = x;
-        const bool pipe = !R.st && R.c->lstm_pipe && R.side >= 0 && R.side < 2 && R.c->aux_stream[2 + R.side] && op.lstm.size() == 2 && lstm_seq_supported(H) && !op.lstm[0].w_rm && !op.lstm[1].w_rm &&
-                          L >= 64 * ldc_ctx::kLstmChunks;
-        if (pipe) {
-          constexpr int NCH = ldc_ctx::kLstmChunks;
+        const int hi = H == 512 ? 1 : 0;
+        const bool coop_all = op.lstm.size() == 2 && op.lstm[0].w_rm && op.lstm[1].w_rm && !R.c->lstm_stream_only && R.c->coop_resident[hi] >= 2 * R.teams &&
+                              R.c->coop_launch == 0;
+        const bool xcd_form = R.c->lstm_xcd && R.c->xcd_resident[hi] >= 2 * R.teams && (R.B % 32 == 1 || R.B % 32 == 2);
+        const bool reg_all = op.lstm.size() == 2 && lstm_seq_supported(H) && !op.lstm[0].w_rm && !op.lstm[1].w_rm;
+        const int want = R.c->lstm_wavefront ? R.c->lstm_wavefront : (R.c->lstm_pipe ? 4 : 0);
+        const int NCH = std::min(std::min(want, (int)ldc_ctx::kLstmChunks), L);
+        if (!R.st && NCH >= 2 && R.side >= 0 && R.side < 2 && R.c->aux_stream[2 + R.side] && (reg_all || (coop_all && !xcd_form))) {
           void* pre0 = R.ar->alloc((size_t)R.B * L * 4 * H * 4);
           void* o0 = R.ar->alloc((size_t)R.B * L * H * 4);
           void* pre1 = R.ar->alloc((size_t)R.B * L * 4 * H * 4);
           void* o1 = R.ar->alloc((size_t)R.B * L * H * 4);
           float* st0 = (float*)R.ar->alloc((size_t)R.B * 2 * H * 4);
           float* st1 = (float*)R.ar->alloc((size_t)R.B * 2 * H * 4);
+          int* fresh = (int*)R.ar->alloc((size_t)2 * R.B * 4);
+          void* lws0 = coop_all ? R.ar->alloc(lstm_coop_ws_bytes(H)) : nullptr;
+          void* lws1 = coop_all ? R.ar->alloc(lstm_coop_ws_bytes(H)) : nullptr;
           if (!R.dry) {
+            ++g_lstm_wavefronts;
             hipStream_t s2 = R.c->aux_stream[2 + R.side];
             hipEvent_t* ev = R.c->lstm_ev[R.side];
+            if (coop_all) {
+              HIPCHK(hipMemsetAsync(fresh, 1, (size_t)R.B * 4, R.s));
+              HIPCHK(hipMemsetAsync(fresh + R.B, 0, (size_t)R.B * 4, R.s));
+            }
             ConvCall cc;
             cc.B = R.B; cc.L_in = L; cc.L_rows = L; cc.x1 = in; cc.y = pre0; cc.y_ld = 4 * H; cc.tune = &R.c->tune;
             HIPCHK(launch_conv(op.lstm[0].in_proj, cc, R.s));
+            auto chunk = [&](int n, const void* pre, void* out, const void* skip, long long pre_bs, long long pre_ts, long long out_bs, long long out_ts,
+                             int t0, int t1, float* state, void* lws, hipStream_t s) -> hipError_t {
+              if (!coop_all) {
+                LstmSeq q;
+                q.t0 = t0; q.t1 = t1; q.pre_bs = pre_bs; q.pre_ts = pre_ts; q.out_bs = q.skip_bs = out_bs; q.out_ts = q.skip_ts = out_ts; q.state = state;
+                return launch_lstm_seq(DT_F32, pre, op.lstm[n].w_hh, out, skip, R.B, H, q, s);
+              }
+              LstmRows rw;
+              rw.pre_bs = pre_bs; rw.pre_ts = pre_ts; rw.out_bs = out_bs; rw.out_ts = out_ts;
+              LstmCarry carry;
+              carry.state = state; carry.fresh = t0 == 0 ? fresh : fresh + R.B;
+              const size_t po = (size_t)t0 * pre_ts * 4 * H * 4, oo = (size_t)t0 * out_ts * H * 4;
+              return launch_lstm_coop(DT_F32, (const char*)pre + po, op.lstm[n].w_rm, (char*)out + oo, skip ? (const char*)skip + oo : nullptr, R.B, t1 - t0, H, lws,
+                                      R.c->dev_flag_dev, 0, s, carry, &rw);
+            };
             for (int k = 0; k < NCH; ++k) {
               const int t0 = (int)((long long)L * k / NCH), t1 = (int)((long long)L * (k + 1) / NCH);
-              LstmSeq q0;
-              q0.t0 = t0; q0.t1 = t1; q0.pre_bs = L; q0.pre_ts = 1; q0.out_bs = 1; q0.out_ts = R.B; q0.state = st0;
-              HIPCHK(launch_lstm_seq(DT_F32, pre0, op.lstm[0].w_hh, o0, nullptr, R.B, H, q0, R.s));
+              HIPCHK(chunk(0, pre0, o0, nullptr, L, 1, 1, R.B, t0, t1, st0, lws0, R.s));
               HIPCHK(hipEventRecord(ev[k], R.s));
               HIPCHK(hipStreamWaitEvent(s2, ev[k], 0));
               ConvCall c1;
@@ -1103,9 +1131,7 @@
               c1.x1 = (const char*)o0 + (size_t)t0 * R.B * H * 4;
               c1.y = (char*)pre1 + (size_t)t0 * R.B * 4 * H * 4;
               HIPCHK(launch_conv(op.lstm[1].in_proj, c1, s2));
-              LstmSeq q1;
-              q1.t0 = t0; q1.t1 = t1; q1.pre_bs = 1; q1.pre_ts = R.B; q1.out_bs = L; q1.out_ts = 1; q1.skip_bs = L; q1.skip_ts = 1; q1.state = st1;
-              HIPCHK(launch_lstm_seq(DT_F32, pre1, op.lstm[1].w_hh, o1, x, R.B, H, q1, s2));
+              HIPCHK(chunk(1, pre1, o1, x, 1, R.B, L, 1, t0, t1, st1, lws1, s2));
             }
             HIPCHK(hipEventRecord(ev[NCH], s2));
             HIPCHK(hipStreamWaitEvent(R.s, ev[NCH], 0));
@@ -1173,6 +1199,7 @@
   const Codec& cd = c->codec[which];
   LDCCHK(with_scratch(c, s, [&](Arena& ar, bool dry) -> int {
     SeaRun R{c, &ar, s, dry, B};
+    R.side = 0;
     void* z = nullptr;
     int L = 0, C = 0;
     LDCCHK(run_seanet(R, cd.enc, wav, T, &z, &L, &C));
@@ -1257,10 +1284,11 @@
 }
 
 static int get_cond_rows(ldc_ctx* c, const float* wav, int B, int T, float bandwidth, Arena& ar, bool dry, hipStream_t s,
-                         float** q_rows, int* F_out, int64_t* codes_out, int teams = 1) {
+                         float** q_rows, int* F_out, int64_t* codes_out, int teams = 1, int side = -1) {
   const Codec& cd = c->codec[LDC_MODEL_COND];
   SeaRun R{c, &ar, s, dry, B};
   R.teams = teams;
+  R.side = side;
   void* z = nullptr;
   int F = 0, C = 0;
   LDCCHK(run_seanet(R, cd.enc, wav, T, &z, &F, &C));
@@ -1279,7 +1307,7 @@
   LDCCHK(with_scratch(c, s, [&](Arena& ar, bool dry) -> int {
     float* qr = nullptr;
     int F = 0;
-    LDCCHK(get_cond_rows(c, wav, B, T, bandwidth, ar, dry, s, &qr, &F, codes_out));
+    LDCCHK(get_cond_rows(c, wav, B, T, bandwidth, ar, dry, s, &qr, &F, codes_out, 1, 0));
     if (!dry) HIPCHK(launch_from_cl(DT_F32, qr, cond_out, B, c->cfg.rep_dims, F, nullptr, 0, 0.f, s));
     return LDC_OK;
   }));
@@ -1629,7 +1657,7 @@
       int Fq = 0;
       if (src.wav) {
         if (rag) LDCCHK(ragged_cond_rows(c, wav_in, B, b0, Bk, T, rag, flens_all, 0.f, ar, dry, sk, &qr, &Fq, codes_out, n_front));
-        else LDCCHK(get_cond_rows(c, wav_in + (size_t)b0 * T, Bk, T, 0.f, ar, dry, sk, &qr, &Fq, codes_out, n_front));
+        else LDCCHK(get_cond_rows(c, wav_in + (size_t)b0 * T, Bk, T, 0.f, ar, dry, sk, &qr, &Fq, codes_out, n_front, h.n <= 2 ? k : -1));
       } else {
         qr = (float*)ar.alloc((size_t)Bk * F * D * 4);
         Fq = F;
diff --git a/ladiffcodec_amd/csrc/ldc_internal.h b/ladiffcodec_amd/csrc/ldc_internal.h
--- a/ladiffcodec_amd/csrc/ldc_internal.h
+++ b/ladiffcodec_amd/csrc/ldc_internal.h
@@ -248,7 +248,7 @@
   Halves last_halves;
   hipStream_t aux_stream[kMaxParts] = {nullptr, nullptr, nullptr, nullptr};
   hipEvent_t ev_fork = nullptr, ev_join[kMaxParts] = {nullptr, nullptr, nullptr, nullptr};
-  static constexpr int kLstmChunks = 4;
+  static constexpr int kLstmChunks = 8;
   hipEvent_t lstm_ev[kMaxParts][kLstmChunks + 1] = {};
   hipStream_t calib_stream = nullptr; bool calibrated = false;
   int calib_good = -1, calib_cand = 0; double calib_one_ms = 0, calib_all_ms = 0;
@@ -256,6 +256,7 @@
   std::vector<CalibOrder> calib_cache;
   int calib = 1;
   int ends_join = 0;
+  int lstm_wavefront = 4;
   int lstm_pipe = 0;
   int split_batch = 2;
   int merge_advance = 1;
diff --git a/ladiffcodec_amd/csrc/ldc_kernels.h b/ladiffcodec_amd/csrc/ldc_kernels.h
--- a/ladiffcodec_amd/csrc/ldc_kernels.h
+++ b/ladiffcodec_amd/csrc/ldc_kernels.h
@@ -255,11 +255,15 @@
                              int H, hipStream_t s, LstmCarry carry = LstmCarry());
 bool lstm_coop_eligible(int H);
 size_t lstm_coop_ws_bytes(int H);
-bool lstm_coop_resident(int H);
+int lstm_coop_teams(int H);
 int conv_fused_gn_wgs_per_cu(int dt, bool w8);
 int lstm_xcd_resident(int H);
+struct LstmRows {
+  long long pre_bs = 0, pre_ts = 1, out_bs = 0, out_ts = 1;
+};
 hipError_t launch_lstm_coop(int dt, const void* pre, const float* w_rm, void* out, const void* skip, int B, int T, int H,
-                            void* ws, unsigned* host_flag, int coop_launch, hipStream_t s, LstmCarry carry = LstmCarry());
+                            void* ws, unsigned* host_flag, int coop_launch, hipStream_t s, LstmCarry carry = LstmCarry(),
+                            const LstmRows* rows = nullptr);
 
 hipError_t launch_rvq(const float* z_rows, int rows, int D, const float* codebooks, const float* cb_sqnorm, int bins,
                       int n_q, int64_t* codes, float* quantized_rows, hipStream_t s, int variant = 1);
diff --git a/ladiffcodec_amd/csrc/seanet.hip b/ladiffcodec_amd/csrc/seanet.hip
--- a/ladiffcodec_amd/csrc/seanet.hip
+++ b/ladiffcodec_amd/csrc/seanet.hip
@@ -282,7 +282,8 @@
 
 template <typename T, int H>
 __global__ __launch_bounds__(256) void lstm_coop_kernel(const void* pre, const float* w_hh, void* out, const void* skip,
-                                                        int B, int T_len, float* hbuf, unsigned* sync, unsigned* host_flag, const LstmCarry carry) {
+                                                        int B, int T_len, float* hbuf, unsigned* sync, unsigned* host_flag, const LstmCarry carry,
+                                                        const LstmRows rw) {
   constexpr int KW = H / 4;
   constexpr int NI = KW / 16;
   __shared__ float part[4][2][16][16];
@@ -305,8 +306,8 @@
   float sknext = 0.f;
   if (owner) {
 #pragma unroll
-    for (int g = 0; g < 4; ++g) pnext[g] = sld<T>(pre, ((size_t)ob * T_len) * (4 * H) + g * H + 4 * j + ou);
-    if (skip) sknext = sld<T>(skip, ((size_t)ob * T_len) * H + 4 * j + ou);
+    for (int g = 0; g < 4; ++g) pnext[g] = sld<T>(pre, ((size_t)ob * rw.pre_bs) * (4 * H) + g * H + 4 * j + ou);
+    if (skip) sknext = sld<T>(skip, ((size_t)ob * rw.out_bs) * H + 4 * j + ou);
     if (carry.state && !carry.fresh[ob]) c_state = carry.state[(size_t)ob * 2 * H + H + 4 * j + ou];
   }
   float h_last = 0.f;
@@ -384,12 +385,12 @@
       h_last = h;
       __hip_atomic_store(hbuf + (size_t)(t & 1) * 32 * H + (size_t)ob * H + 4 * j + ou, h, __ATOMIC_RELAXED, __HIP_MEMORY_SCOPE_AGENT);
       asm volatile("s_waitcnt vmcnt(0)" ::: "memory");
-      const size_t o = ((size_t)ob * T_len + t) * H + 4 * j + ou;
+      const size_t o = ((size_t)ob * rw.out_bs + (size_t)t * rw.out_ts) * H + 4 * j + ou;
       sst<T>(out, o, h + sknext);
       if (t + 1 < T_len) {
 #pragma unroll
-        for (int g = 0; g < 4; ++g) pnext[g] = sld<T>(pre, ((size_t)ob * T_len + t + 1) * (4 * H) + g * H + 4 * j + ou);
-        if (skip) sknext = sld<T>(skip, o + H);
+        for (int g = 0; g < 4; ++g) pnext[g] = sld<T>(pre, ((size_t)ob * rw.pre_bs + (size_t)(t + 1) * rw.pre_ts) * (4 * H) + g * H + 4 * j + ou);
+        if (skip) sknext = sld<T>(skip, o + (size_t)rw.out_ts * H);
       }
     }
     __syncthreads();
@@ -397,7 +398,7 @@
       __hip_atomic_fetch_add(sync + (j % LSTM_COOP_SHARDS) * LSTM_COOP_SHARD_STRIDE, 1u, __ATOMIC_RELAXED, __HIP_MEMORY_SCOPE_AGENT);
   }
   if (dead && owner) {
-    for (int tt = t; tt < T_len; ++tt) sst<T>(out, ((size_t)ob * T_len + tt) * H + 4 * j + ou, __builtin_nanf(""));
+    for (int tt = t; tt < T_len; ++tt) sst<T>(out, ((size_t)ob * rw.out_bs + (size_t)tt * rw.out_ts) * H + 4 * j + ou, __builtin_nanf(""));
   }
   if (carry.state && owner) {
     carry.state[(size_t)ob * 2 * H + 4 * j + ou] = dead ? __builtin_nanf("") : h_last;
@@ -576,17 +577,22 @@
 
 template <typename T>
 static hipError_t lstm_coop_launch(const void* pre, const float* w_rm, void* out, const void* skip, int B, int T_len, int H,
-                                   void* ws, unsigned* host_flag, int coop_launch, hipStream_t s, const LstmCarry carry_all) {
+                                   void* ws, unsigned* host_flag, int coop_launch, hipStream_t s, const LstmCarry carry_all,
+                                   const LstmRows* rows) {
   float* hbuf = reinterpret_cast<float*>(ws);
   unsigned* sync = reinterpret_cast<unsigned*>(hbuf + (size_t)2 * 32 * H);
   const size_t esz = sizeof(T);
+  LstmRows rw;
+  rw.pre_bs = rw.out_bs = T_len;
+  if (rows) rw = *rows;
   for (int b0 = 0; b0 < B; b0 += 32) {
     const int nb = std::min(32, B - b0);
+    if (rows && coop_launch == 2 && nb <= 2) return hipErrorInvalidValue;
     hipError_t e = hipMemsetAsync(sync, 0, 256 * sizeof(unsigned), s);
     if (e != hipSuccess) return e;
-    const char* p = reinterpret_cast<const char*>(pre) + (size_t)b0 * T_len * 4 * H * esz;
-    char* o = reinterpret_cast<char*>(out) + (size_t)b0 * T_len * H * esz;
-    const char* k = skip ? reinterpret_cast<const char*>(skip) + (size_t)b0 * T_len * H * esz : nullptr;
+    const char* p = reinterpret_cast<const char*>(pre) + (size_t)b0 * rw.pre_bs * 4 * H * esz;
+    char* o = reinterpret_cast<char*>(out) + (size_t)b0 * rw.out_bs * H * esz;
+    const char* k = skip ? reinterpret_cast<const char*>(skip) + (size_t)b0 * rw.out_bs * H * esz : nullptr;
     const void* pp = p; void* oo = o; const void* kk = k; int nbv = nb, tl = T_len;
     LstmCarry carry;
     if (carry_all.state) {
@@ -595,7 +601,7 @@
       hipLaunchKernelGGL(lstm_state_publish_kernel, dim3((nb * H + 255) / 256), dim3(256), 0, s, carry, hbuf + (size_t)32 * H, nb, H);
       if ((e = hipGetLastError()) != hipSuccess) return e;
     }
-    void* args[] = {&pp, &w_rm, &oo, &kk, &nbv, &tl, &hbuf, &sync, &host_flag, &carry};
+    void* args[] = {&pp, &w_rm, &oo, &kk, &nbv, &tl, &hbuf, &sync, &host_flag, &carry, &rw};
     const void* fn = H == 512 ? reinterpret_cast<const void*>(lstm_coop_kernel<T, 512>) : reinterpret_cast<const void*>(lstm_coop_kernel<T, 256>);
     if (coop_launch == 2 && nb <= 2) {
       const void* fx = H == 512 ? reinterpret_cast<const void*>(lstm_xcd_kernel<T, 512>) : reinterpret_cast<const void*>(lstm_xcd_kernel<T, 256>);
@@ -637,23 +643,24 @@
   return per_cu * (cus / 8) / 16;
 }
 
-bool lstm_coop_resident(int H) {
-  if (!lstm_coop_eligible(H)) return false;
+int lstm_coop_teams(int H) {
+  if (!lstm_coop_eligible(H)) return 0;
   const void* fn = H == 512 ? reinterpret_cast<const void*>(lstm_coop_kernel<float, 512>) : reinterpret_cast<const void*>(lstm_coop_kernel<float, 256>);
   int dev = 0, per_cu = 0, cus = 0;
   if (hipGetDevice(&dev) != hipSuccess || hipDeviceGetAttribute(&cus, hipDeviceAttributeMultiprocessorCount, dev) != hipSuccess ||
       hipOccupancyMaxActiveBlocksPerMultiprocessor(&per_cu, fn, 256, 0) != hipSuccess) {
     (void)hipGetLastError();
-    return false;
-  }
-  return (long long)std::max(0, per_cu - 1) * cus >= H / 4 || (long long)per_cu * cus >= 2 * (H / 4);
+    return 0;
+  }
+  const long long wgs = std::max((long long)std::max(0, per_cu - 1) * cus, (long long)per_cu * cus / 2);
+  return (int)(wgs / (H / 4));
 }
 
 hipError_t launch_lstm_coop(int dt, const void* pre, const float* w_rm, void* out, const void* skip, int B, int T, int H,
-                            void* ws, unsigned* host_flag, int coop_launch, hipStream_t s, LstmCarry carry) {
+                            void* ws, unsigned* host_flag, int coop_launch, hipStream_t s, LstmCarry carry, const LstmRows* rows) {
   if (!lstm_coop_eligible(H) || (carry.state && !carry.fresh)) return hipErrorInvalidValue;
-  return dt == DT_F32 ? lstm_coop_launch<float>(pre, w_rm, out, skip, B, T, H, ws, host_flag, coop_launch, s, carry)
-                      : lstm_coop_launch<__bf16>(pre, w_rm, out, skip, B, T, H, ws, host_flag, coop_launch, s, carry);
+  return dt == DT_F32 ? lstm_coop_launch<float>(pre, w_rm, out, skip, B, T, H, ws, host_flag, coop_launch, s, carry, rows)
+                      : lstm_coop_launch<__bf16>(pre, w_rm, out, skip, B, T, H, ws, host_flag, coop_launch, s, carry, rows);
 }
 
 bool lstm_seq_supported(int H) { return H == 64 || H == 128; }
diff --git a/ladiffcodec_amd/lib.py b/ladiffcodec_amd/lib.py
--- a/ladiffcodec_amd/lib.py
+++ b/ladiffcodec_amd/lib.py
@@ -28,7 +28,7 @@
     "ldc_unet_forward_items", "ldc_pool_create", "ldc_pool_destroy", "ldc_pool_admit", "ldc_pool_admit_ddim", "ldc_pool_step", "ldc_pool_remaining", "ldc_pool_take", "ldc_pool_peek", "ldc_pool_evict",
     "ldc_stream_min_first", "ldc_stream_create", "ldc_stream_reset", "ldc_stream_destroy", "ldc_seanet_encode_stream", "ldc_seanet_decode_stream", "ldc_get_cond_stream",
     "ldc_sconv1d", "ldc_sconvtr1d", "ldc_slstm", "ldc_unet_debug_tap", "ldc_unet_step_cost", "ldc_profile_enable",
-    "ldc_profile_read", "ldc_profile_read_classes", "ldc_conv_microbench", "ldc_conv_compare", "ldc_conv_compare_fp8", "ldc_ln_fold_compare", "ldc_gn_microbench", "ldc_host_stats", "ldc_graph_schedule", "ldc_stream_info", "ldc_clock_sample", "ldc_debug_raise_failure", "ldc_debug_attn_core", "ldc_debug_attention_block", "ldc_debug_resnet_block", "ldc_debug_sea_conv", "ldc_debug_sea_op", "ldc_debug_sync_count", "ldc_debug_lean_launches", "ldc_xcc_census", "ldc_timeline_enable", "ldc_timeline_read", "ldc_kstamps_enable", "ldc_kstamps_reset", "ldc_kstamps_read", "ldc_packed_bytes", "ldc_pack_codes", "ldc_unpack_codes",
+    "ldc_profile_read", "ldc_profile_read_classes", "ldc_conv_microbench", "ldc_conv_compare", "ldc_conv_compare_fp8", "ldc_ln_fold_compare", "ldc_gn_microbench", "ldc_host_stats", "ldc_graph_schedule", "ldc_stream_info", "ldc_clock_sample", "ldc_debug_raise_failure", "ldc_debug_attn_core", "ldc_debug_attention_block", "ldc_debug_resnet_block", "ldc_debug_sea_conv", "ldc_debug_sea_op", "ldc_debug_sync_count", "ldc_debug_lean_launches", "ldc_debug_lstm_wavefronts", "ldc_xcc_census", "ldc_timeline_enable", "ldc_timeline_read", "ldc_kstamps_enable", "ldc_kstamps_reset", "ldc_kstamps_read", "ldc_packed_bytes", "ldc_pack_codes", "ldc_unpack_codes",
     "ldc_ac_build_cdf", "ldc_ac_encode", "ldc_ac_decode", "ldc_train_q_sample", "ldc_train_num_timesteps", "ldc_train_predict_x_start", "ldc_train_neg_sdsdr", "ldc_train_l1_loss", "ldc_train_block_ws_floats",
     "ldc_train_block_forward", "ldc_train_block_backward", "ldc_train_layernorm_forward", "ldc_train_layernorm_backward", "ldc_train_adam_step", "ldc_train_adam_step_dev", "ldc_train_pointwise_forward", "ldc_train_pointwise_backward", "ldc_train_linattn_ws_floats", "ldc_train_linattn_forward", "ldc_train_linattn_backward", "ldc_train_conv_forward", "ldc_train_conv_backward", "ldc_train_join", "ldc_train_side_stream", "ldc_train_upsample2", "ldc_train_activation", "ldc_train_attn_ws_floats", "ldc_train_attn_forward", "ldc_train_attn_backward", "ldc_train_convtr_forward", "ldc_train_convtr_backward", "ldc_train_maxscale", "ldc_resample_out_len", "ldc_resample",
 ]
@@ -222,7 +222,7 @@
     lib.ldc_train_adam_step_dev.argtypes = [vp, fp, fp, fp, fp, C.c_int64, vp, C.c_float, C.c_float, C.c_float, C.c_float, vp]
     lib.ldc_resample_out_len.argtypes = [C.c_int64, i32, i32]
     lib.ldc_resample.argtypes = [vp, fp, i32, C.c_int64, i32, i32, fp, vp]
-    optional = {"ldc_debug_lean_launches"} if "LDC_LIB_PATH" in os.environ else set()
+    optional = {"ldc_debug_lean_launches", "ldc_debug_lstm_wavefronts"} if "LDC_LIB_PATH" in os.environ else set()
     if hasattr(lib, "ldc_debug_lean_launches"):
         lib.ldc_debug_lean_launches.argtypes = [i32]
     lib.ldc_gn_microbench.argtypes = [vp, i32, i32, i32, i32, i32, i32, C.POINTER(C.c_double)]
@@ -230,7 +230,7 @@
         if name in optional and not hasattr(lib, name):
             continue
         fn = getattr(lib, name)
-        if name in ("ldc_debug_sync_count", "ldc_debug_lean_launches", "ldc_packed_bytes", "ldc_train_block_ws_floats", "ldc_train_linattn_ws_floats", "ldc_train_attn_ws_floats", "ldc_resample_out_len"):
+        if name in ("ldc_debug_sync_count", "ldc_debug_lean_launches", "ldc_debug_lstm_wavefronts", "ldc_packed_bytes", "ldc_train_block_ws_floats", "ldc_train_linattn_ws_floats", "ldc_train_attn_ws_floats", "ldc_resample_out_len"):
             fn.restype = C.c_int64
         elif name == "ldc_quantize_e4m3":
             fn.restype = None
```

New measurement: 695.6 audio-s/wall-s (median of 6 runs). About the same (+0.5%).
